# IDEA-Research/MP-Former

Hardware: AMD Instinct MI355X
Metric: training images/sec COCO-instance R50 1024x1024 (higher is better)
Workload: dtype bf16 (backbone, decoder) + f32 (pixel decoder, losses), as the reference's AMP; 1 GPU; COCO-instance R50, 100 queries, 80 classes, 1024x1024: full train step = R50 backbone + MSDeformAttn pixel decoder (6 layers) + MP masked decoder (9 layers, NUM_DN 1) + Hungarian matching + 60 losses + backward + grad all-reduce + clip + AdamW; head_only_workload=False, global_batch=2, per_gpu_batch=2, parallelism=dp1, msda_offsets=init, full=False, autograd_threads=backward on the launch thread, miopen_find_db=shipped

## Files before the change

include/mpformer_hip.h:

```cpp
#ifndef MPFORMER_HIP_H
#define MPFORMER_HIP_H

#include <stddef.h>
#include <stdint.h>

#ifdef __cplusplus
extern "C" {
#endif

enum { MPF_F32 = 0, MPF_F64 = 1, MPF_BF16 = 2, MPF_U8 = 3, MPF_BITS = 4  };

enum {
    MPF_OK = 0,
    MPF_E_DTYPE = -1,
    MPF_E_SHAPE = -2,
    MPF_E_NULL = -3,
    MPF_E_TOO_LARGE = -4
};

int mpf_abi_version(void);
const char* mpf_last_error(void);

int mpf_msda_forward(const void* value, const int64_t* spatial_shapes,
                     const int64_t* level_start_index, const void* sampling_loc,
                     const void* attn_weight, void* output,
                     int batch, int spatial_size, int num_heads, int channels,
                     int num_levels, int num_query, int num_point,
                     int dtype, void* stream);

int mpf_msda_forward_hs(const void* value, const int64_t* spatial_shapes,
                        const int64_t* level_start_index, const int64_t* host_spatial_shapes,
                        const void* sampling_loc, const void* attn_weight, void* output,
                        int batch, int spatial_size, int num_heads, int channels,
                        int num_levels, int num_query, int num_point,
                        int dtype, void* stream);

int mpf_msda_backward(const void* value, const int64_t* spatial_shapes,
                      const int64_t* level_start_index, const void* sampling_loc,
                      const void* attn_weight, const void* grad_output,
                      void* grad_value, void* grad_sampling_loc, void* grad_attn_weight,
                      int batch, int spatial_size, int num_heads, int channels,
                      int num_levels, int num_query, int num_point,
                      int dtype, void* stream);

size_t mpf_msda_dev_workspace_bytes(int batch, int spatial_size, int num_heads, int num_levels, int num_query, int num_point,
                                    int backward);
int mpf_msda_forward_dev(const void* value, const int64_t* spatial_shapes, const int64_t* level_start_index, const void* sampling_loc,
                         const void* attn_weight, void* output, int batch, int spatial_size, int num_heads, int channels,
                         int num_levels, int num_query, int num_point, int dtype, void* workspace, size_t workspace_bytes,
                         void* stream);
int mpf_msda_backward_dev(const void* value, const int64_t* spatial_shapes, const int64_t* level_start_index, const void* sampling_loc,
                          const void* attn_weight, const void* grad_output, void* grad_value, void* grad_sampling_loc,
                          void* grad_attn_weight, int batch, int spatial_size, int num_heads, int channels, int num_levels,
                          int num_query, int num_point, int dtype, void* workspace, size_t workspace_bytes, void* stream);
int mpf_msda_dev_geometry(const void* workspace, int* out, int n);

size_t mpf_msda_backward_workspace_bytes(int batch, int num_heads, int num_levels, int num_query,
                                         int num_point, const int64_t* host_spatial_shapes);
int mpf_msda_backward_ws(const void* value, const int64_t* host_spatial_shapes,
                         const void* sampling_loc, const void* attn_weight, const void* grad_output,
                         void* grad_value, void* grad_sampling_loc, void* grad_attn_weight,
                         int batch, int spatial_size, int num_heads, int channels,
                         int num_levels, int num_query, int num_point, int dtype,
                         void* workspace, size_t workspace_bytes, void* stream);

int mpf_set_option(const char* key, int value);
const char* mpf_last_kernel(void);
int mpf_msda_stats(unsigned long long* out, int n, int reset);

int mpf_point_sample(const void* src, int src_dtype, int h, int w, const int64_t* rows,
                     const float* coords, const int32_t* coord_rows, float* out, int n, int P, void* stream);

int mpf_mask_loss_forward(const void* pred, int pred_dtype, int h, int w, const int64_t* pred_rows,
                          const void* gt, int gt_dtype, int H, int W, const int32_t* gt_rows,
                          const float* coords, float* partial, int n, int P, int chunks, void* stream);

int mpf_pack_mask_bits(const uint8_t* masks, void* bits, int64_t n_pixels, void* stream);

int mpf_mask_loss_backward(const void* pred, int pred_dtype, int h, int w, const int64_t* pred_rows,
                           const uint8_t* gt, int H, int W, const int32_t* gt_rows,
                           const float* coords, const float* grad_sums, float* grad_pred,
                           const int64_t* grad_offs, int n, int P, void* stream);

int mpf_select_uncertain(const float* vals, const float* coords_in, float* coords_out,
                         int n, int M, int k, int P_out, void* stream);

int mpf_sample_select_uncertain(const void* pred, int pred_dtype, int h, int w, const int64_t* pred_offs,
                                const float* coords_in, float* coords_out, int n, int M, int k, int P_out,
                                void* stream);

int mpf_match_cost(const void* pred, int pred_dtype, int h, int w, const int64_t* pred_offs,
                   const float* coords, const int32_t* coord_rows, const float* tsamp,
                   const int32_t* t_first, const int32_t* t_count, float* cost,
                   int n_rows, int Tmax, int P, float w_mask, float w_dice, int rows_per_group, void* stream);

int mpf_attn_mask(const void* masks, int dtype, int64_t stride_n, int64_t stride_q, int h, int w,
                  const uint8_t* mp_rows, int pad, uint8_t* out, int N, int Q, int hl, int wl, void* stream);

size_t mpf_attn_workspace_bytes(int Lq, int Lk, int N, int H);
int mpf_attn_forward(const void* q, const void* k, const void* vt, const uint8_t* mask, int mask_per_image,
                     void* out, float* lse, int Lq, int Lk, int N, int H, int head_dim, float scale,
                     void* workspace, size_t workspace_bytes, void* stream);

int mpf_attn_backward(const void* q, const void* k, const void* v, const void* kT, const void* qT,
                      const void* dout, const void* doutT, const uint8_t* mask, int mask_per_image,
                      const float* lse, const float* delta, void* dq, void* dk, void* dv,
                      int Lq, int LqP, int Lk, int N, int H, int head_dim, float scale,
                      void* workspace, size_t workspace_bytes, void* stream);

int mpf_attn_transpose2(const void* a, const void* b, void* aT, void* bT, int L, int LP, int N, int E, void* stream);
int mpf_attn_transpose2_strided(const void* a, const void* b, int64_t in_row_stride, int64_t in_img_stride, void* aT, void* bT, int L,
                                int LP, int N, int E, void* stream);
int mpf_attn_forward_kv(const void* q, const void* k, int64_t k_row_stride, int64_t k_img_stride, const void* vt, const uint8_t* mask,
                        int mask_per_image, void* out, float* lse, int Lq, int Lk, int N, int H, int head_dim, float scale,
                        void* workspace, size_t workspace_bytes, void* stream);
int mpf_attn_backward_kv(const void* q, const void* k, const void* v, int64_t kv_row_stride, int64_t kv_img_stride, const void* kT,
                         const void* qT, const void* dout, const void* doutT, const uint8_t* mask, int mask_per_image,
                         const float* lse, const float* delta, void* dq, void* dk, void* dv, int64_t dkv_row_stride,
                         int64_t dkv_img_stride, int Lq, int LqP, int Lk, int N, int H, int head_dim, float scale, void* workspace,
                         size_t workspace_bytes, void* stream);
size_t mpf_attn_bwd_aux_bytes(int Lq, int Lk, int N, int H, int mask_images);
int mpf_attn_bwd_prep_aux(const void* q, const void* dout, const void* out, const float* lse, const uint8_t* mask, int mask_per_image,
                          int Lk, void* qT, void* doT, float* delta, void* aux, size_t aux_bytes, int Lq, int LqP, int N, int H,
                          void* stream);
int mpf_attn_backward_kv_aux(const void* q, const void* k, const void* v, int64_t kv_row_stride, int64_t kv_img_stride, const void* kT,
                             const void* qT, const void* dout, const void* doutT, const uint8_t* mask, int mask_per_image,
                             const float* lse, const float* delta, void* dq, void* dk, void* dv, int64_t dkv_row_stride,
                             int64_t dkv_img_stride, int Lq, int LqP, int Lk, int N, int H, int head_dim, float scale, void* workspace,
                             size_t workspace_bytes, const void* aux, void* stream);
int mpf_attn_delta(const void* dout, const void* out, float* delta, int Lq, int N, int H, void* stream);
int mpf_attn_bwd_prep(const void* q, const void* dout, const void* out, void* qT, void* doT, float* delta, int Lq, int LqP, int N,
                      int H, void* stream);

int mpf_msda_forward_raw(const void* value, const int64_t* spatial_shapes, const int64_t* level_start_index,
                         const void* raw, const void* ref_points, void* loc_out, void* attn_out, void* output,
                         int batch, int spatial_size, int num_heads, int channels, int num_levels, int num_query,
                         int num_point, int dtype, void* stream);
int mpf_msda_forward_raw_hs(const void* value, const int64_t* spatial_shapes, const int64_t* level_start_index,
                            const int64_t* host_spatial_shapes,
                            const void* raw, const void* ref_points, void* loc_out, void* attn_out, void* output,
                            int batch, int spatial_size, int num_heads, int channels, int num_levels, int num_query,
                            int num_point, int dtype, void* stream);
int mpf_msda_backward_ws_raw(const void* value, const int64_t* host_spatial_shapes,
                             const void* sampling_loc, const void* attn_weight, const void* grad_output,
                             void* grad_value, void* grad_raw,
                             int batch, int spatial_size, int num_heads, int channels,
                             int num_levels, int num_query, int num_point, int dtype,
                             void* workspace, size_t workspace_bytes, void* stream);
int mpf_msda_backward_ws_raw_o(const void* value, const int64_t* host_spatial_shapes,
// ... 122 lines not shown
size_t mpf_next_attn_mask_scratch_bytes(int N, int Q);
int mpf_next_attn_mask(const MpfNextMask* m, void* stream);
int mpf_decoder_layer_backward(const MpfDecoderLayer* layer, const MpfDecoderLayerGrad* grad, void* stream);

typedef struct MpfScaleCastItem {
    const void* src;
    void* dst;
    const float* scale;
    int64_t numel, inner, first_block;
} MpfScaleCastItem;

int mpf_grouped_scale_cast(const MpfScaleCastItem* items_device, int n_items, int64_t total_blocks, int src_dtype, int dst_dtype,
                           void* stream);

#define MPF_AMAX_SLOT_FLOATS 512
int mpf_res_ln256_forward_b(const float* x, const void* t, int t_dtype, const float* gamma, const float* beta, float* s_out, float* y32,
                            void* y16, float* mean, float* rstd, int rows, float eps, const float* padd, int padd_rows, float* y_plus,
                            float* y_bound, const float* padd_amax, float* yplus_bound, void* stream);
int mpf_res_ln256_backward_ws_amax(const float* s, const float* mean, const float* rstd, const float* gamma, const float* gy32,
                                   const void* gy16, const float* gy_plus, float* ds32, void* ds16, float* dgamma, float* dbeta, int rows,
                                   void* workspace, size_t workspace_bytes, float* ds_amax, void* stream);
typedef struct MpfAmaxItem {
    const float* src;
    float* out;
    int64_t numel, first_block;
} MpfAmaxItem;
typedef struct MpfSplitItemH2 {
    const float* src;
    void* dst;
    const float* amax;
    int64_t rows, cols, transpose, dst_ld, plane_stride, first_block;
} MpfSplitItemH2;
int mpf_amax_f32(const float* x, int64_t n, float* amax, void* stream);
int mpf_amax_f32_grouped(const MpfAmaxItem* items_device, int n_items, int64_t total_blocks, void* stream);
int mpf_h2_range_stats(const float* a, int rows, int cols, int64_t lda, const float* amax_slot, int log2_below,
                       unsigned long long* counters_device, void* stream);
int mpf_gemm3_split_grouped_h2(const MpfSplitItemH2* items_device, int n_items, int64_t total_blocks, void* stream);
typedef struct MpfNtItemH2 {
    const float* a;
    int64_t lda;
    const float* a_amax;
    const float* b;
    int64_t ldb;
    const float* b_amax;
    float* c_part;
    float* csum_a;
    int64_t Mdim, Ndim;
} MpfNtItemH2;
int mpf_gemm3_nt_h2(const float* a, int64_t lda, const float* a_amax, const float* b, int64_t ldb, const float* b_amax,
                    float* c_part, float* csum_a, float* csum_b, int R, int Mdim, int Ndim, int rows_per_split,
                    int transpose_out, void* stream);
int mpf_gemm3_nt_grouped_h2(const MpfNtItemH2* items, int n_items, int R, int rows_per_split, int64_t split_stride, void* stream);
int mpf_gemm3_conv3x3_h2(const float* x, const float* x_amax, const void* w_planes_h2, const float* w_amax, const float* bias,
                         float* y, float* out_amax, int n_img, int H, int W, int Cin, int Cout, int transposed, void* stream);
int mpf_gemm3_conv3x3_wgrad_h2(const float* dy, const float* dy_amax, const float* x, const float* x_amax, float* c_part,
                               float* csum_dy, int n_img, int H, int W, int Cin, int Cout, int rows_per_split, void* stream);
int mpf_gemm3_tn_h2(const float* a, int64_t lda, const float* a_amax, const void* b_planes_h2, const float* b_amax,
                    const float* bias, const float* c_in, int64_t ldcin, const float* c_in2, int64_t ldcin2,
                    const float* gate, int64_t ldgate, float* c, int64_t ldc, float* out_amax, int M, int N, int K,
                    int relu, void* stream);
int mpf_gemm3_tn_h2_bits(const float* a, int64_t lda, const float* a_amax, const void* b_planes_h2, const float* b_amax,
                         const float* bias, const float* c_in, int64_t ldcin, const float* c_in2, int64_t ldcin2,
                         const unsigned char* gate_bits, int64_t ldgbits, float* c, int64_t ldc, float* out_amax,
                         unsigned char* gate_bits_out, int64_t ldgbits_out, int M, int N, int K, int relu, void* stream);

typedef struct MpfNtItem {
    const float* a;
    int64_t lda;
    const float* b;
    int64_t ldb;
    float* c_part;
    float* csum_a;
    int64_t Mdim, Ndim;
} MpfNtItem;
int mpf_gemm3_nt_grouped(const MpfNtItem* items, int n_items, int R, int rows_per_split, int64_t split_stride, void* stream);

int mpf_gemm3_conv3x3(const float* x, const void* w_planes, const float* bias, float* y, int n_img, int H, int W, int Cin,
                      int Cout, int transposed, void* stream);
int mpf_gemm3_conv3x3_wgrad(const float* dy, const float* x, float* c_part, float* csum_dy, int n_img, int H, int W, int Cin, int Cout,
                            int rows_per_split, void* stream);

int mpf_gemm3_tn_ex(const void* a, int a_dtype, int64_t lda, const void* b_planes, const float* bias, const float* c_in, int64_t ldcin,
                    void* c, int c_dtype, int64_t ldc, int M, int N, int K, int relu, void* stream);
int mpf_gemm3_nt_ex(const void* a, int a_dtype, int64_t lda, const void* b, int b_dtype, int64_t ldb, float* c_part, float* csum_a,
                    int R, int Mdim, int Ndim, int rows_per_split, void* stream);

typedef struct MpfSplitItem {
    const float* src;
    void* dst;
    int64_t rows, cols, transpose, dst_ld, plane_stride, first_block;
} MpfSplitItem;

int mpf_gemm3_split_grouped(const MpfSplitItem* items_device, int n_items, int64_t total_blocks, void* stream);

typedef struct MpfOptItem {
    float* param;
    const float* grad;
    float* exp_avg;
    float* exp_avg_sq;
    int64_t numel, first_block;
    float lr, weight_decay, bc1, bc2_sqrt;
} MpfOptItem;

int mpf_clip_adamw_step(const MpfOptItem* items_device, int n_items, int64_t total_blocks, float max_norm, double beta1,
                        double beta2, double eps, float* partial, float* norm_clip, void* stream);

int mpf_transpose_f32(const float* in, int64_t in_batch_stride, float* out, int64_t out_batch_stride, int B, int R, int C,
                      void* stream);

int mpf_gemm3_nt_reduce(const float* c_part, int64_t c_numel, const float* s_part, int64_t s_numel, int nsplit,
                        float* c_out, float* s_out, void* stream);
int mpf_gemm3_nt_reduce_levels(const float* c_part, int64_t c_numel, const float* s_part, int64_t s_numel, int nsplit,
                               const int64_t* level_of_split, int n_levels, float* c_out, float* lvl_out, float* s_out, void* stream);

int mpf_tall_gemm_bf16(const void* a, int64_t lda, const void* b, int64_t ldb, const void* bias, void* c, int64_t ldc, int M, int N,
                       int K, void* stream);
size_t mpf_gemm_nt_bf16_workspace_bytes(int R, int Mdim, int Ndim, int rows_per_split);
int mpf_gemm_nt_bf16(const void* a, int64_t lda, const void* b, int64_t ldb, void* c_out, void* csum_out, int R, int Mdim,
                     int Ndim, int rows_per_split, void* workspace, size_t workspace_bytes, void* stream);

int mpf_small_gemm_bf16_blocked(const void* a, int64_t a_rs, int64_t a_ks, int a_blk, int64_t a_bs, const void* gate, const void* b,
                                int64_t b_rs, int64_t b_ks, const void* bias, const void* c_in, int64_t ldcin, void* c, int64_t ldc,
                                int c_blk, int64_t c_bs, void* rowsum_a, int I, int J, int Kc, int relu, void* stream);

int mpf_class_loss_forward(const void* logits, int dtype, int64_t sl, int64_t sn, int64_t sq, const int64_t* target,
                           int target_per_output, const float* weight, int L, int N, int Q, int C, float* lse, float* ce,
                           float* wsum, void* stream);
int mpf_class_loss_backward(const void* logits, int dtype, int64_t sl, int64_t sn, int64_t sq, const int64_t* target,
                            int target_per_output, const float* weight, int L, int N, int Q, int C, const float* lse,
                            const float* wsum, const float* grad_ce, void* dlogits, void* stream);
int mpf_mask_loss_finalize(const float* sums, const int64_t* runs, const float* norm, int n, int G, int points, float* out,
                           void* stream);
int mpf_mask_loss_finalize_backward(const float* sums, const int64_t* runs, const float* norm, int n, int G, int points,
                                    const float* grad_out, float* dsums, void* stream);

typedef struct {
    const void* a;
    const void* gate;
    const void* b;
    void* c;
    void* rowsum_a;
    int64_t a_rs, a_ks, a_bs, b_rs, b_ks, ldc;
    int a_blk, I, J, Kc;
} MpfSmallGemmItem;
int mpf_small_gemm_bf16_group(const MpfSmallGemmItem* items, int n_items, void* stream);
typedef struct MpfTransposeItem {
    const void* src;
    const void* gate;
    void* dst;
    int64_t ld;
    int R, C;
} MpfTransposeItem;
int mpf_transpose_group_bf16(const MpfTransposeItem* items, int n_items, int Rp, void* stream);

int mpf_bias_act(const void* x, const float* bias, const void* res, void* y, int64_t numel, int C, int dtype,
                 int relu, void* stream);
int mpf_relu_bwd_add(const void* ga, const void* gb, const void* y, void* out, int64_t numel, int dtype, void* stream);
int mpf_maxpool3x3s2_forward(const void* x, void* y, void* code, int N, int H, int W, int C, void* stream);
int mpf_maxpool3x3s2_backward(const void* gy, const void* code, void* gx, int N, int H, int W, int C, void* stream);

int mpf_upload_small(const void* host_src, void* device_dst, int64_t nbytes, void* stream);

int mpf_res_ln256_forward(const float* x, const void* t, int t_dtype, const float* gamma, const float* beta,
                          float* s_out, float* y32, void* y16, float* mean, float* rstd, int rows, float eps,
                          const float* padd, int padd_rows, float* y_plus, void* stream);
int mpf_res_ln256_backward(const float* s, const float* mean, const float* rstd, const float* gamma, const float* gy32,
                           const void* gy16, const float* gy_plus, float* ds32, void* ds16, float* dgamma, float* dbeta,
                           int rows, void* stream);
int mpf_res_ln256_backward_partial(const float* s, const float* mean, const float* rstd, const float* gamma, const float* gy32,
                                   const void* gy16, const float* gy_plus, float* ds32, void* ds16, int rows, void* partials,
                                   size_t partials_bytes, void* stream);
int mpf_res_ln256_backward_partial_amax(const float* s, const float* mean, const float* rstd, const float* gamma, const float* gy32,
                                        const void* gy16, const float* gy_plus, float* ds32, void* ds16, int rows, void* partials,
                                        size_t partials_bytes, float* ds_amax, void* stream);
int mpf_ln_partial_reduce(const void* partials, size_t stride_bytes, int rows, int n_ln, float* out, void* stream);
size_t mpf_res_ln256_backward_det_workspace_bytes(int rows);
int mpf_res_ln256_backward_det(const float* s, const float* mean, const float* rstd, const float* gamma, const float* gy32,
                               const void* gy16, const float* gy_plus, float* ds32, void* ds16, float* dgamma_dbeta, int rows,
                               void* workspace, size_t workspace_bytes, void* stream);
size_t mpf_res_ln256_backward_workspace_bytes(int rows);
int mpf_res_ln256_backward_ws(const float* s, const float* mean, const float* rstd, const float* gamma, const float* gy32,
                              const void* gy16, const float* gy_plus, float* ds32, void* ds16, float* dgamma, float* dbeta, int rows,
                              void* workspace, size_t workspace_bytes, void* stream);

int mpf_mask_loss_backward_dense(const void* pred, int pred_dtype, int h, int w, const int64_t* pred_rows,
                                 const void* gt, int gt_dtype, int H, int W, const int32_t* gt_rows, const float* coords,
                                 const float* grad_sums, void* grad, int grad_dtype, const int64_t* grad_offs,
                                 int n, int P, void* stream);

size_t mpf_group_stats_workspace_bytes(int rows, int64_t row_len);
int mpf_group_stats(const float* x, int rows, int64_t row_len, float eps, float* mean, float* rstd,
                    void* workspace, size_t workspace_bytes, void* stream);

int mpf_gn_cl_supported(int HW, int C, int G);
size_t mpf_gn_cl_workspace_bytes(int N, int HW, int C, int G);
int mpf_gn_cl_forward(const float* x, int64_t x_bs, const float* gamma, const float* beta, int N, int HW, int C, int G,
                      float eps, int relu, const float* top, int64_t top_bs, int W, float* y, int64_t y_bs, float* mean,
                      float* rstd, void* workspace, size_t workspace_bytes, void* stream);
int mpf_gn_cl_backward(const float* gy, int64_t gy_bs, const float* x, int64_t x_bs, const float* gamma, const float* beta,
                       const float* mean, const float* rstd, int N, int HW, int C, int G, int relu, float* dx,
                       int64_t dx_bs, float* dgamma, float* dbeta, void* workspace, size_t workspace_bytes, void* stream);
int mpf_upsample2x_cl_backward(const float* gy, int64_t gy_bs, int N, int Ht, int Wt, int C, float* dtop, int64_t dtop_bs,
                               void* stream);

size_t mpf_match_cost_fused_workspace_bytes(int G, int Q, int Tmax, int P, int tsamp_rows);
int mpf_match_cost_fused(const void* embed, const int64_t* embed_first, int64_t embed_row_stride, const void* features,
                         int64_t feat_img_stride, const int32_t* group_image, int h, int w, int channels, const float* coords,
                         const float* tsamp, int tsamp_rows, const int32_t* t_first, const int32_t* t_count, float* cost, int G,
                         int Q, int Tmax, int P, float w_mask, float w_dice, void* workspace, size_t workspace_bytes, void* stream);
int mpf_pair_planes_forward(const void* embed, const int64_t* row_off, const int32_t* pair_of_slot, const int32_t* slot_first,
                            const int32_t* slot_count, const void* features, int64_t feat_img_stride, void* out, int N, int HW,
                            int channels, void* stream);
size_t mpf_pair_planes_backward_workspace_bytes(int N, int HW, int total_slots, int max_count);
int mpf_pair_planes_backward(const void* grad_planes, const void* embed, const int64_t* row_off, const int32_t* pair_of_slot,
                             const int32_t* slot_first, const int32_t* slot_count, const void* features, int64_t feat_img_stride,
                             void* d_features, int64_t dfeat_img_stride, void* d_embed, int d_embed_dtype, int N, int HW, int channels,
                             int total_slots, int max_count, void* workspace, size_t workspace_bytes, void* stream);

int mpf_profile_enable(int on);
int mpf_profile_get(const char* name_substr, int* count, double* total_ms, double* total_bytes);
int mpf_profile_get_flops(const char* name_substr, double* total_flops);

enum {
    MPF_ENC_PV, MPF_ENC_PV_AM, MPF_ENC_PO, MPF_ENC_PO_AM, MPF_ENC_P1, MPF_ENC_P1_AM, MPF_ENC_P2, MPF_ENC_P2_AM, MPF_ENC_P288, MPF_ENC_P288_AM,
    MPF_ENC_BV, MPF_ENC_BO, MPF_ENC_BB1, MPF_ENC_BB2, MPF_ENC_B288, MPF_ENC_G1, MPF_ENC_B1, MPF_ENC_G2, MPF_ENC_B2,
    MPF_ENC_VALUE, MPF_ENC_RAW, MPF_ENC_LOC, MPF_ENC_ATTN, MPF_ENC_AO, MPF_ENC_S1, MPF_ENC_MEAN1, MPF_ENC_RSTD1, MPF_ENC_X1, MPF_ENC_H,
    MPF_ENC_HBITS, MPF_ENC_S2, MPF_ENC_MEAN2, MPF_ENC_RSTD2, MPF_ENC_X2, MPF_ENC_QN,
    MPF_ENC_AO_AM, MPF_ENC_X1_AM, MPF_ENC_H_AM, MPF_ENC_XN_AM, MPF_ENC_QN_AM,
    MPF_ENC_FIELDS
};
typedef struct MpfEncoderCall {
    int32_t N, S, M, L, P, nl, F, reserved;
    float eps, pad_;
    const int64_t* host_shapes;
    const void* shapes_dev;
    const void* lsi_dev;
    const float* ref;
    const float* pos_full;
    const float* pos_am;
    const float* x0;
    const float* x0_am;
    const float* q0;
    const float* q0_am;
    const uint64_t* layers;
} MpfEncoderCall;
int mpf_encoder_fields(void);
int mpf_encoder_forward(const MpfEncoderCall* call, void* stream);

enum {
    MPF_ENCB_X, MPF_ENCB_Q, MPF_ENCB_VALUE, MPF_ENCB_LOC, MPF_ENCB_ATTN, MPF_ENCB_AO, MPF_ENCB_S1, MPF_ENCB_MEAN1, MPF_ENCB_RSTD1, MPF_ENCB_X1,
    MPF_ENCB_H, MPF_ENCB_HBITS, MPF_ENCB_S2, MPF_ENCB_MEAN2, MPF_ENCB_RSTD2,
    MPF_ENCB_X_AM, MPF_ENCB_Q_AM, MPF_ENCB_AO_AM, MPF_ENCB_X1_AM, MPF_ENCB_H_AM,
    MPF_ENCB_G1, MPF_ENCB_G2,
    MPF_ENCB_TV, MPF_ENCB_TV_AM, MPF_ENCB_TO, MPF_ENCB_TO_AM, MPF_ENCB_T1, MPF_ENCB_T1_AM, MPF_ENCB_T2, MPF_ENCB_T2_AM, MPF_ENCB_T288, MPF_ENCB_T288_AM,
    MPF_ENCB_DS2_AM, MPF_ENCB_DH_AM, MPF_ENCB_DS1_AM, MPF_ENCB_DRAW_AM, MPF_ENCB_GV_AM,
    MPF_ENCB_WGRAD, MPF_ENCB_DW288, MPF_ENCB_LVL, MPF_ENCB_DB288,
    MPF_ENCB_FIELDS
};
typedef struct MpfEncoderBwdCall {
    int32_t N, S, M, L, P, nl, F, rps288, rps_group, reserved;
    int64_t group_stride;
    const int64_t* host_shapes;
    const float* gout;
    const int64_t* split_level;
    float *ds2, *dh, *dx1, *ds1, *dao, *gv, *draw;
    float* dq[2];
    float* g[2];
    float *cpart288, *cs288, *part_group;
    void* ln_parts;
    uint64_t ln_stride;
    void* msda_ws;
    uint64_t msda_ws_bytes;
    float* dgb_out;
    const uint64_t* layers;
} MpfEncoderBwdCall;
int mpf_encoder_bwd_fields(void);
int mpf_encoder_backward(const MpfEncoderBwdCall* call, void* stream);

int mpf_seg_softmax(const float* cls, int Q, int K1, float object_mask_threshold, float* probs, float* max_score, int* max_label,
                    int* kept, float* kept_score, void* stream);
int mpf_seg_semantic(const void* masks, int64_t stride_q, int dtype, int Q, int h, int w, int Hp, int Wp, int hi, int wi, int H, int W,
                     const float* probs, int K, float* out, void* stream);
size_t mpf_seg_instance_workspace_bytes(int T, int H, int W);
int mpf_seg_instance_scores(const void* masks, int64_t stride_q, int dtype, int Q, int h, int w, int Hp, int Wp, int hi, int wi, int H,
                            int W, const int64_t* sel_q, const float* cls_score, int T, float* scores, void* workspace,
                            size_t workspace_bytes, void* stream);
// ... 32 lines not shown
```

mp_former_amd/_lib.py:

```python
import ctypes

import torch
import os

_HERE = os.path.dirname(os.path.abspath(__file__))
LIB_PATH = os.path.join(_HERE, "libmpformer_hip.so")
LIB_PATH = os.environ.get("MPF_LIB_PATH", LIB_PATH)
ABI_VERSION = 1

MPF_F32, MPF_F64, MPF_BF16, MPF_U8, MPF_BITS = 0, 1, 2, 3, 4
DTYPE = {torch.float32: MPF_F32, torch.float64: MPF_F64, torch.bfloat16: MPF_BF16, torch.uint8: MPF_U8, torch.bool: MPF_U8}

_lib = None
_status_fns = {}

_c_int = ctypes.c_int
_c_vp = ctypes.c_void_p

SIGNATURES = {
    "mpf_abi_version": (_c_int, []),
    "mpf_last_error": (ctypes.c_char_p, []),
    "mpf_last_kernel": (ctypes.c_char_p, []),
    "mpf_set_option": (_c_int, [ctypes.c_char_p, _c_int]),
    "mpf_match_cost_fused_workspace_bytes": (ctypes.c_size_t, [_c_int] * 5),
    "mpf_match_cost_fused": (_c_int, [_c_vp, _c_vp, ctypes.c_int64, _c_vp, ctypes.c_int64, _c_vp, _c_int, _c_int, _c_int, _c_vp, _c_vp, _c_int,
                                      _c_vp, _c_vp, _c_vp, _c_int, _c_int, _c_int, _c_int, ctypes.c_float, ctypes.c_float, _c_vp,
                                      ctypes.c_size_t, _c_vp]),
    "mpf_pair_planes_forward": (_c_int, [_c_vp] * 6 + [ctypes.c_int64, _c_vp, _c_int, _c_int, _c_int, _c_vp]),
    "mpf_pair_planes_backward_workspace_bytes": (ctypes.c_size_t, [_c_int] * 4),
    "mpf_pair_planes_backward": (_c_int, [_c_vp] * 7 + [ctypes.c_int64, _c_vp, ctypes.c_int64, _c_vp, _c_int, _c_int, _c_int, _c_int, _c_int,
                                          _c_int, _c_vp, ctypes.c_size_t, _c_vp]),
    "mpf_msda_dev_workspace_bytes": (ctypes.c_size_t, [_c_int] * 7),
    "mpf_msda_forward_dev": (_c_int, [_c_vp] * 6 + [_c_int] * 8 + [_c_vp, ctypes.c_size_t, _c_vp]),
    "mpf_msda_backward_dev": (_c_int, [_c_vp] * 9 + [_c_int] * 8 + [_c_vp, ctypes.c_size_t, _c_vp]),
    "mpf_msda_dev_geometry": (_c_int, [_c_vp, ctypes.POINTER(_c_int), _c_int]),
    "mpf_msda_stats": (_c_int, [ctypes.POINTER(ctypes.c_ulonglong), _c_int, _c_int]),
    "mpf_profile_enable": (_c_int, [_c_int]),
    "mpf_profile_get_flops": (_c_int, [ctypes.c_char_p, ctypes.POINTER(ctypes.c_double)]),
    "mpf_profile_get": (_c_int, [ctypes.c_char_p, ctypes.POINTER(_c_int), ctypes.POINTER(ctypes.c_double),
                                 ctypes.POINTER(ctypes.c_double)]),
    "mpf_point_sample": (_c_int, [_c_vp, _c_int, _c_int, _c_int, _c_vp, _c_vp, _c_vp, _c_vp, _c_int, _c_int, _c_vp]),
    "mpf_mask_loss_forward": (_c_int, [_c_vp, _c_int, _c_int, _c_int, _c_vp, _c_vp, _c_int, _c_int, _c_int, _c_vp, _c_vp,
                                       _c_vp, _c_int, _c_int, _c_int, _c_vp]),
    "mpf_pack_mask_bits": (_c_int, [_c_vp, _c_vp, ctypes.c_int64, _c_vp]),
    "mpf_mask_loss_backward": (_c_int, [_c_vp, _c_int, _c_int, _c_int, _c_vp, _c_vp, _c_int, _c_int, _c_vp, _c_vp,
                                        _c_vp, _c_vp, _c_vp, _c_int, _c_int, _c_vp]),
    "mpf_select_uncertain": (_c_int, [_c_vp, _c_vp, _c_vp, _c_int, _c_int, _c_int, _c_int, _c_vp]),
    "mpf_sample_select_uncertain": (_c_int, [_c_vp, _c_int, _c_int, _c_int, _c_vp, _c_vp, _c_vp, _c_int, _c_int, _c_int, _c_int, _c_vp]),
    "mpf_match_cost": (_c_int, [_c_vp, _c_int, _c_int, _c_int, _c_vp, _c_vp, _c_vp, _c_vp, _c_vp, _c_vp, _c_vp,
                                _c_int, _c_int, _c_int, ctypes.c_float, ctypes.c_float, _c_int, _c_vp]),
    "mpf_attn_mask": (_c_int, [_c_vp, _c_int, ctypes.c_int64, ctypes.c_int64, _c_int, _c_int, _c_vp, _c_int, _c_vp,
                               _c_int, _c_int, _c_int, _c_int, _c_vp]),
    "mpf_attn_workspace_bytes": (ctypes.c_size_t, [_c_int] * 4),
    "mpf_attn_forward": (_c_int, [_c_vp, _c_vp, _c_vp, _c_vp, _c_int, _c_vp, _c_vp, _c_int, _c_int, _c_int, _c_int, _c_int,
                                  ctypes.c_float, _c_vp, ctypes.c_size_t, _c_vp]),
    "mpf_attn_backward": (_c_int, [_c_vp] * 8 + [_c_int] + [_c_vp] * 5 + [_c_int] * 6 + [ctypes.c_float, _c_vp, ctypes.c_size_t, _c_vp]),
    "mpf_attn_transpose2": (_c_int, [_c_vp] * 4 + [_c_int] * 4 + [_c_vp]),
    "mpf_attn_transpose2_strided": (_c_int, [_c_vp] * 2 + [ctypes.c_int64] * 2 + [_c_vp] * 2 + [_c_int] * 4 + [_c_vp]),
    "mpf_attn_forward_kv": (_c_int, [_c_vp, _c_vp, ctypes.c_int64, ctypes.c_int64, _c_vp, _c_vp, _c_int, _c_vp, _c_vp, _c_int, _c_int,
                                     _c_int, _c_int, _c_int, ctypes.c_float, _c_vp, ctypes.c_size_t, _c_vp]),
    "mpf_attn_backward_kv": (_c_int, [_c_vp] * 3 + [ctypes.c_int64] * 2 + [_c_vp] * 5 + [_c_int] + [_c_vp] * 5 + [ctypes.c_int64] * 2
                             + [_c_int] * 6 + [ctypes.c_float, _c_vp, ctypes.c_size_t, _c_vp]),
    "mpf_attn_backward_kv_aux": (_c_int, [_c_vp] * 3 + [ctypes.c_int64] * 2 + [_c_vp] * 5 + [_c_int] + [_c_vp] * 5 + [ctypes.c_int64] * 2
                                 + [_c_int] * 6 + [ctypes.c_float, _c_vp, ctypes.c_size_t, _c_vp, _c_vp]),
    "mpf_attn_bwd_aux_bytes": (ctypes.c_size_t, [_c_int] * 5),
    "mpf_attn_bwd_prep_aux": (_c_int, [_c_vp] * 5 + [_c_int] * 2 + [_c_vp] * 4 + [ctypes.c_size_t] + [_c_int] * 4 + [_c_vp]),
    "mpf_attn_delta": (_c_int, [_c_vp] * 3 + [_c_int] * 3 + [_c_vp]),
    "mpf_attn_bwd_prep": (_c_int, [_c_vp] * 6 + [_c_int] * 4 + [_c_vp]),
    "mpf_gemm3_split": (_c_int, [_c_vp, _c_int, _c_int, _c_int, _c_vp, _c_vp]),
    "mpf_gemm3_tn": (_c_int, [_c_vp, ctypes.c_int64, _c_vp, _c_int, _c_vp, _c_vp, _c_vp, ctypes.c_int64, _c_vp, ctypes.c_int64,
                           _c_vp, ctypes.c_int64, _c_vp, ctypes.c_int64, _c_int, _c_int, _c_int, _c_int, _c_vp]),
    "mpf_gemm3_nt": (_c_int, [_c_vp, ctypes.c_int64, _c_vp, ctypes.c_int64, _c_vp, ctypes.c_int64, _c_int, _c_vp, _c_vp, _c_vp,
                           _c_int, _c_int, _c_int, _c_int, _c_int, _c_vp]),
    "mpf_amax_f32": (_c_int, [_c_vp, ctypes.c_int64, _c_vp, _c_vp]),
    "mpf_amax_f32_grouped": (_c_int, [_c_vp, _c_int, ctypes.c_int64, _c_vp]),
    "mpf_h2_range_stats": (_c_int, [_c_vp, _c_int, _c_int, ctypes.c_int64, _c_vp, _c_int, _c_vp, _c_vp]),
    "mpf_gemm3_split_grouped_h2": (_c_int, [_c_vp, _c_int, ctypes.c_int64, _c_vp]),
    "mpf_gemm3_tn_h2": (_c_int, [_c_vp, ctypes.c_int64, _c_vp, _c_vp, _c_vp, _c_vp, _c_vp, ctypes.c_int64, _c_vp, ctypes.c_int64,
                              _c_vp, ctypes.c_int64, _c_vp, ctypes.c_int64, _c_vp, _c_int, _c_int, _c_int, _c_int, _c_vp]),
    "mpf_gemm3_tn_h2_bits": (_c_int, [_c_vp, ctypes.c_int64, _c_vp, _c_vp, _c_vp, _c_vp, _c_vp, ctypes.c_int64, _c_vp, ctypes.c_int64,
                                   _c_vp, ctypes.c_int64, _c_vp, ctypes.c_int64, _c_vp, _c_vp, ctypes.c_int64,
                                   _c_int, _c_int, _c_int, _c_int, _c_vp]),
    "mpf_gemm3_nt_h2": (_c_int, [_c_vp, ctypes.c_int64, _c_vp, _c_vp, ctypes.c_int64, _c_vp, _c_vp, _c_vp, _c_vp,
                              _c_int, _c_int, _c_int, _c_int, _c_int, _c_vp]),
    "mpf_gemm3_nt_grouped_h2": (_c_int, [_c_vp, _c_int, _c_int, _c_int, ctypes.c_int64, _c_vp]),
    "mpf_gemm3_conv3x3_h2": (_c_int, [_c_vp] * 7 + [_c_int] * 6 + [_c_vp]),
    "mpf_gemm3_conv3x3_wgrad_h2": (_c_int, [_c_vp, _c_vp, _c_vp, _c_vp, _c_vp, _c_vp, _c_int, _c_int, _c_int, _c_int, _c_int, _c_int, _c_vp]),
    "mpf_gemm3_nt_grouped": (_c_int, [_c_vp, _c_int, _c_int, _c_int, ctypes.c_int64, _c_vp]),
    "mpf_small_gemm_bf16": (_c_int, [_c_vp, ctypes.c_int64, ctypes.c_int64, _c_vp, _c_vp, ctypes.c_int64, ctypes.c_int64, _c_vp, _c_vp,
                                     ctypes.c_int64, _c_vp, ctypes.c_int64, _c_vp, _c_int, _c_int, _c_int, _c_int, _c_vp]),
    "mpf_encoder_fields": (_c_int, []),
    "mpf_encoder_forward": (_c_int, [_c_vp, _c_vp]),
    "mpf_encoder_bwd_fields": (_c_int, []),
    "mpf_encoder_backward": (_c_int, [_c_vp, _c_vp]),
    "mpf_decoder_layer_struct_bytes": (ctypes.c_uint64, [_c_int]),
    "mpf_decoder_layer_scratch_bytes": (ctypes.c_uint64, [_c_int] * 6),
    "mpf_decoder_layer_forward": (_c_int, [_c_vp, _c_vp]),
    "mpf_next_attn_mask_scratch_bytes": (ctypes.c_size_t, [_c_int, _c_int]),
    "mpf_next_attn_mask": (_c_int, [_c_vp, _c_vp]),
    "mpf_lin256_res_ln_forward": (_c_int, [_c_vp] * 11 + [_c_int, ctypes.c_float, _c_vp]),
    "mpf_ln256_mlp3_forward": (_c_int, [_c_vp] * 10 + [_c_int, ctypes.c_float, _c_vp]),
    "mpf_decoder_layer_backward": (_c_int, [_c_vp, _c_vp, _c_vp]),
    "mpf_pool_features": (_c_int, [_c_vp, _c_int, _c_vp] + [_c_int] * 6 + [_c_vp]),
    "mpf_pool_features_cl": (_c_int, [_c_vp, ctypes.c_int64, _c_int, _c_vp, _c_int, _c_int, _c_int, _c_int, _c_int, _c_int, _c_vp]),
    "mpf_mask_head_bits": (_c_int, [_c_vp, ctypes.c_int64, ctypes.c_int64, _c_vp, _c_vp, _c_int, _c_vp, _c_vp] + [_c_int] * 3 + [_c_vp]),
    "mpf_lsa_assign": (_c_int, [_c_vp, _c_vp, _c_int, _c_int, ctypes.c_int64] + [_c_vp] * 7),
    "mpf_lsa_assign_status": (_c_int, [_c_vp, _c_vp, _c_int, _c_int, ctypes.c_int64] + [_c_vp] * 8),
    "mpf_mask_block_empty": (_c_int, [_c_vp, _c_vp] + [_c_int] * 5 + [_c_vp]),
    "mpf_mp_open_counts": (_c_int, [_c_vp, _c_int, _c_int, _c_vp, _c_vp]),
    "mpf_mp_noise_rows": (_c_int, [_c_vp] * 3 + [_c_int] * 4 + [ctypes.c_double, ctypes.c_uint64, ctypes.c_uint64, _c_vp, _c_vp]),
    "mpf_gemm_nt_bf16_workspace_bytes": (ctypes.c_size_t, [_c_int] * 4),
    "mpf_gemm_nt_bf16": (_c_int, [_c_vp, ctypes.c_int64, _c_vp, ctypes.c_int64, _c_vp, _c_vp, _c_int, _c_int, _c_int, _c_int, _c_vp,
                                  ctypes.c_size_t, _c_vp]),
    "mpf_gemm3_nt_reduce": (_c_int, [_c_vp, ctypes.c_int64, _c_vp, ctypes.c_int64, _c_int, _c_vp, _c_vp, _c_vp]),
    "mpf_grouped_scale_cast": (_c_int, [_c_vp, _c_int, ctypes.c_int64, _c_int, _c_int, _c_vp]),
    "mpf_gemm3_split_grouped": (_c_int, [_c_vp, _c_int, ctypes.c_int64, _c_vp]),
    "mpf_decoder_inputs_forward": (_c_int, [_c_vp, ctypes.c_int64, ctypes.c_int64, _c_vp, _c_vp, _c_vp, _c_vp, _c_int, _c_int, _c_int, _c_int,
                                            _c_vp]),
    "mpf_decoder_inputs_backward": (_c_int, [_c_vp, _c_vp, _c_int, _c_vp, ctypes.c_int64, ctypes.c_int64, _c_int, _c_int, _c_int, _c_vp]),
    "mpf_clip_adamw_step": (_c_int, [_c_vp, _c_int, ctypes.c_int64, ctypes.c_float, ctypes.c_double, ctypes.c_double, ctypes.c_double,
                                     _c_vp, _c_vp, _c_vp]),
    "mpf_transpose_f32": (_c_int, [_c_vp, ctypes.c_int64, _c_vp, ctypes.c_int64, _c_int, _c_int, _c_int, _c_vp]),
    "mpf_small_gemm_bf16_blocked": (_c_int, [_c_vp, ctypes.c_int64, ctypes.c_int64, _c_int, ctypes.c_int64, _c_vp, _c_vp, ctypes.c_int64,
                                             ctypes.c_int64, _c_vp, _c_vp, ctypes.c_int64, _c_vp, ctypes.c_int64, _c_int, ctypes.c_int64,
                                             _c_vp, _c_int, _c_int, _c_int, _c_int, _c_vp]),
    "mpf_small_gemm_bf16_group": (_c_int, [_c_vp, _c_int, _c_vp]),
    "mpf_transpose_group_bf16": (_c_int, [_c_vp, _c_int, _c_int, _c_vp]),
    "mpf_class_loss_forward": (_c_int, [_c_vp, _c_int, ctypes.c_int64, ctypes.c_int64, ctypes.c_int64, _c_vp, _c_int, _c_vp, _c_int, _c_int,
                                        _c_int, _c_int, _c_vp, _c_vp, _c_vp, _c_vp]),
    "mpf_class_loss_backward": (_c_int, [_c_vp, _c_int, ctypes.c_int64, ctypes.c_int64, ctypes.c_int64, _c_vp, _c_int, _c_vp, _c_int, _c_int,
                                         _c_int, _c_int, _c_vp, _c_vp, _c_vp, _c_vp, _c_vp]),
    "mpf_mask_loss_finalize": (_c_int, [_c_vp, _c_vp, _c_vp, _c_int, _c_int, _c_int, _c_vp, _c_vp]),
    "mpf_mask_loss_finalize_backward": (_c_int, [_c_vp, _c_vp, _c_vp, _c_int, _c_int, _c_int, _c_vp, _c_vp, _c_vp]),
    "mpf_bias_act": (_c_int, [_c_vp, _c_vp, _c_vp, _c_vp, ctypes.c_int64, _c_int, _c_int, _c_int, _c_vp]),
    "mpf_relu_bwd_add": (_c_int, [_c_vp, _c_vp, _c_vp, _c_vp, ctypes.c_int64, _c_int, _c_vp]),
    "mpf_maxpool3x3s2_forward": (_c_int, [_c_vp] * 3 + [_c_int] * 4 + [_c_vp]),
    "mpf_maxpool3x3s2_backward": (_c_int, [_c_vp] * 3 + [_c_int] * 4 + [_c_vp]),
    "mpf_upload_small": (_c_int, [_c_vp, _c_vp, ctypes.c_int64, _c_vp]),
    "mpf_tall_gemm_bf16": (_c_int, [_c_vp, ctypes.c_int64, _c_vp, ctypes.c_int64, _c_vp, _c_vp, ctypes.c_int64, _c_int, _c_int, _c_int, _c_vp]),
    "mpf_res_ln256_forward": (_c_int, [_c_vp, _c_vp, _c_int, _c_vp, _c_vp, _c_vp, _c_vp, _c_vp, _c_vp, _c_vp, _c_int, ctypes.c_float,
                                       _c_vp, _c_int, _c_vp, _c_vp]),
    "mpf_res_ln256_forward_b": (_c_int, [_c_vp, _c_vp, _c_int, _c_vp, _c_vp, _c_vp, _c_vp, _c_vp, _c_vp, _c_vp, _c_int, ctypes.c_float,
                                         _c_vp, _c_int, _c_vp, _c_vp, _c_vp, _c_vp, _c_vp]),
    "mpf_res_ln256_backward_ws_amax": (_c_int, [_c_vp] * 11 + [_c_int, _c_vp, ctypes.c_size_t, _c_vp, _c_vp]),
    "mpf_res_ln256_backward": (_c_int, [_c_vp] * 11 + [_c_int, _c_vp]),
    "mpf_mask_loss_backward_dense": (_c_int, [_c_vp, _c_int, _c_int, _c_int, _c_vp, _c_vp, _c_int, _c_int, _c_int, _c_vp, _c_vp, _c_vp,
                                              _c_vp, _c_int, _c_vp, _c_int, _c_int, _c_vp]),
    "mpf_gn_cl_supported": (_c_int, [_c_int, _c_int, _c_int]),
    "mpf_gn_cl_workspace_bytes": (ctypes.c_size_t, [_c_int, _c_int, _c_int, _c_int]),
    "mpf_gn_cl_forward": (_c_int, [_c_vp, ctypes.c_int64, _c_vp, _c_vp, _c_int, _c_int, _c_int, _c_int, ctypes.c_float, _c_int,
                                   _c_vp, ctypes.c_int64, _c_int, _c_vp, ctypes.c_int64, _c_vp, _c_vp, _c_vp, ctypes.c_size_t, _c_vp]),
    "mpf_gn_cl_backward": (_c_int, [_c_vp, ctypes.c_int64, _c_vp, ctypes.c_int64, _c_vp, _c_vp, _c_vp, _c_vp, _c_int, _c_int, _c_int,
                                    _c_int, _c_int, _c_vp, ctypes.c_int64, _c_vp, _c_vp, _c_vp, ctypes.c_size_t, _c_vp]),
    "mpf_upsample2x_cl_backward": (_c_int, [_c_vp, ctypes.c_int64, _c_int, _c_int, _c_int, _c_int, _c_vp, ctypes.c_int64, _c_vp]),
    "mpf_gemm3_conv3x3": (_c_int, [_c_vp, _c_vp, _c_vp, _c_vp, _c_int, _c_int, _c_int, _c_int, _c_int, _c_int, _c_vp]),
    "mpf_gemm3_conv3x3_wgrad": (_c_int, [_c_vp, _c_vp, _c_vp, _c_vp, _c_int, _c_int, _c_int, _c_int, _c_int, _c_int, _c_vp]),
    "mpf_gemm3_nt_reduce_levels": (_c_int, [_c_vp, ctypes.c_int64, _c_vp, ctypes.c_int64, _c_int, _c_vp, _c_int, _c_vp, _c_vp, _c_vp, _c_vp]),
    "mpf_gemm3_tn_ex": (_c_int, [_c_vp, _c_int, ctypes.c_int64, _c_vp, _c_vp, _c_vp, ctypes.c_int64, _c_vp, _c_int, ctypes.c_int64,
                                 _c_int, _c_int, _c_int, _c_int, _c_vp]),
    "mpf_gemm3_nt_ex": (_c_int, [_c_vp, _c_int, ctypes.c_int64, _c_vp, _c_int, ctypes.c_int64, _c_vp, _c_vp, _c_int, _c_int, _c_int, _c_int, _c_vp]),
    "mpf_res_ln256_backward_workspace_bytes": (ctypes.c_size_t, [_c_int]),
    "mpf_res_ln256_backward_partial": (_c_int, [_c_vp] * 9 + [_c_int, _c_vp, ctypes.c_size_t, _c_vp]),
    "mpf_res_ln256_backward_partial_amax": (_c_int, [_c_vp] * 9 + [_c_int, _c_vp, ctypes.c_size_t, _c_vp, _c_vp]),
    "mpf_ln_partial_reduce": (_c_int, [_c_vp, ctypes.c_size_t, _c_int, _c_int, _c_vp, _c_vp]),
    "mpf_res_ln256_backward_det_workspace_bytes": (ctypes.c_size_t, [_c_int]),
    "mpf_res_ln256_backward_det": (_c_int, [_c_vp] * 10 + [_c_int, _c_vp, ctypes.c_size_t, _c_vp]),
    "mpf_res_ln256_backward_ws": (_c_int, [_c_vp] * 11 + [_c_int, _c_vp, ctypes.c_size_t, _c_vp]),
    "mpf_group_stats_workspace_bytes": (ctypes.c_size_t, [_c_int, ctypes.c_int64]),
    "mpf_group_stats": (_c_int, [_c_vp, _c_int, ctypes.c_int64, ctypes.c_float, _c_vp, _c_vp, _c_vp, ctypes.c_size_t, _c_vp]),
    "mpf_msda_forward": (_c_int, [_c_vp] * 6 + [_c_int] * 8 + [_c_vp]),
    "mpf_msda_backward": (_c_int, [_c_vp] * 9 + [_c_int] * 8 + [_c_vp]),
    "mpf_msda_forward_hs": (_c_int, [_c_vp] * 7 + [_c_int] * 8 + [_c_vp]),
    "mpf_msda_forward_raw_hs": (_c_int, [_c_vp] * 9 + [_c_int] * 8 + [_c_vp]),
    "mpf_msda_forward_raw": (_c_int, [_c_vp] * 8 + [_c_int] * 8 + [_c_vp]),
    "mpf_msda_backward_ws_raw": (_c_int, [_c_vp] * 7 + [_c_int] * 8 + [_c_vp, ctypes.c_size_t, _c_vp]),
    "mpf_msda_backward_ws_raw_o": (_c_int, [_c_vp] * 8 + [_c_int] * 8 + [_c_vp, ctypes.c_size_t, _c_vp, _c_vp, _c_vp]),
    "mpf_msda_backward_workspace_bytes": (ctypes.c_size_t, [_c_int] * 5 + [_c_vp]),
    "mpf_msda_backward_ws": (_c_int, [_c_vp] * 8 + [_c_int] * 8 + [_c_vp, ctypes.c_size_t, _c_vp]),
    "mpf_seg_softmax": (_c_int, [_c_vp, _c_int, _c_int, ctypes.c_float] + [_c_vp] * 6),
    "mpf_seg_semantic": (_c_int, [_c_vp, ctypes.c_int64] + [_c_int] * 10 + [_c_vp, _c_int, _c_vp, _c_vp]),
    "mpf_seg_instance_workspace_bytes": (ctypes.c_size_t, [_c_int] * 3),
    "mpf_seg_instance_scores": (_c_int, [_c_vp, ctypes.c_int64] + [_c_int] * 10 + [_c_vp, _c_vp, _c_int, _c_vp, _c_vp, ctypes.c_size_t,
                                                                                   _c_vp]),
    "mpf_seg_instance_masks": (_c_int, [_c_vp, ctypes.c_int64] + [_c_int] * 10 + [_c_vp, _c_int, _c_vp, _c_vp]),
    "mpf_seg_panoptic_areas": (_c_int, [_c_vp, ctypes.c_int64] + [_c_int] * 10 + [_c_vp] * 5),
    "mpf_seg_panoptic_paint": (_c_int, [_c_vp, _c_int, _c_int, _c_vp, _c_vp, _c_vp]),
    "mpf_seg_semantic_labels": (_c_int, [_c_vp, ctypes.c_int64] + [_c_int] * 10 + [_c_vp, _c_int, _c_vp, _c_vp]),
    "mpf_seg_labels_resize": (_c_int, [_c_vp] + [_c_int] * 5 + [_c_vp, _c_vp]),
    "mpf_seg_confusion_add": (_c_int, [_c_vp, _c_vp, ctypes.c_int64, _c_int, _c_int, _c_vp, _c_vp]),
    "mpf_seg_instance_rle_workspace_bytes": (ctypes.c_size_t, [_c_int] * 3),
    "mpf_seg_instance_rle_count": (_c_int, [_c_vp, ctypes.c_int64] + [_c_int] * 10 + [_c_vp, _c_int, _c_vp, _c_vp, ctypes.c_size_t, _c_vp]),
    "mpf_seg_instance_rle_write": (_c_int, [_c_vp, ctypes.c_size_t, _c_int, _c_int, _c_int, _c_vp, ctypes.c_int64, _c_vp, _c_vp, _c_vp]),
    "mpf_seg_tta_accumulate": (_c_int, [_c_vp, ctypes.c_int64] + [_c_int] * 10 + [_c_vp, _c_int, _c_int, _c_vp, _c_vp]),
    "mpf_seg_tta_resize_add": (_c_int, [_c_vp] + [_c_int] * 6 + [_c_vp, _c_vp]),
    "mpf_seg_tta_finish": (_c_int, [_c_vp] + [_c_int] * 4 + [_c_vp, _c_vp]),
    "mpf_seg_pq_workspace_bytes": (ctypes.c_size_t, [_c_int] * 2),
    "mpf_seg_pq_pairs": (_c_int, [_c_vp, _c_vp, _c_int, ctypes.c_int64, _c_vp, _c_int, _c_int, _c_vp, _c_int, _c_int, _c_int, _c_vp,
                                  ctypes.c_size_t, _c_vp]),
    "mpf_seg_pq_match": (_c_int, [_c_vp, ctypes.c_size_t, _c_int, _c_int, _c_int, _c_vp, _c_vp, _c_vp, _c_int] + [_c_vp] * 6),
}


class NativeLibraryError(RuntimeError):
    pass


def lib():
    global _lib
    if _lib is None:
        if not os.path.exists(LIB_PATH):
            raise NativeLibraryError(
                f"{LIB_PATH} not found: build it with `python -c 'import __graft_entry__ as g; g.build()'` "
                "or `make -C mp_former_amd/csrc`.  mp_former_amd has no CPU / eager fallback.")
        l = ctypes.CDLL(LIB_PATH)
        for name, (res, args) in SIGNATURES.items():
            try:
                fn = getattr(l, name)
            except AttributeError as e:
                raise NativeLibraryError(f"{LIB_PATH} does not export {name}") from e
            fn.restype = res
            fn.argtypes = args
            if res is _c_int:
                _status_fns[name] = fn
        v = l.mpf_abi_version()
        if v != ABI_VERSION:
            raise NativeLibraryError(f"ABI mismatch: library {v}, binding {ABI_VERSION}")
        _lib = l
        for kv in filter(None, os.environ.get("MPF_OPTIONS", "").split(",")):
            k, _, v = kv.partition("=")
            set_option(k.strip(), int(v))
    return _lib


def check(code, what):
    if code != 0:
        msg = lib().mpf_last_error().decode()
        raise RuntimeError(f"{what} failed with code {code}: {msg}")


def _status_fn(name):
    lib()
    fn = _status_fns.get(name)
    if fn is None:
        raise TypeError(f"{name} does not return a status: call() is for the int-returning entry points, sizes go through lib()")
    return fn


def call(name, device, *args):
    fn = _status_fns.get(name) or _status_fn(name)
    idx = device.index
    if idx is None or idx == torch.cuda.current_device():
        code = fn(*args)
    else:
        with torch.cuda.device(device):
            code = fn(*args)
    if code != 0:
        check(code, name)


def ptr(t):
    return None if t is None else t.data_ptr()


_option_gen = 0


def option_generation():
    return _option_gen


def set_option(key, value):
    global _option_gen
    check(lib().mpf_set_option(key.encode(), int(value)), f"mpf_set_option({key})")
    _option_gen += 1


def msda_stats(reset=True):
    out = (ctypes.c_ulonglong * 9)()
    check(lib().mpf_msda_stats(out, 9, 1 if reset else 0), "mpf_msda_stats")
    keys = ("fwd_lds", "fwd_gather", "push_lds", "push_gather", "push_direct", "push_hash", "spill_entries", "pull_split", "pull_single")
    return dict(zip(keys, (int(v) for v in out)))


def last_kernel():
    return lib().mpf_last_kernel().decode()


def profile_enable(on=True):
    check(lib().mpf_profile_enable(1 if on else 0), "mpf_profile_enable")


def profile_get_flops(name_substr):
    fl = ctypes.c_double(0)
    check(lib().mpf_profile_get_flops(name_substr.encode(), ctypes.byref(fl)), "mpf_profile_get_flops")
    return fl.value


def profile_get(name_substr):
    n, ms, by = _c_int(0), ctypes.c_double(0), ctypes.c_double(0)
    check(lib().mpf_profile_get(name_substr.encode(), ctypes.byref(n), ctypes.byref(ms), ctypes.byref(by)),
          "mpf_profile_get")
    return n.value, ms.value, by.value


_scratch = {}


def scratch(owner, device, stream, nbytes, zeroed=False):
    key = (owner, device, stream)
    w = _scratch.get(key)
    if w is None or w.numel() < nbytes:
        n = int(nbytes * 1.25) + 1024
        w = _scratch[key] = (torch.zeros if zeroed else torch.empty)(n, dtype=torch.uint8, device=device)
    return w


def stream_ptr(device):
    idx = device.index
    return torch._C._cuda_getCurrentRawStream(torch.cuda.current_device() if idx is None else idx)


class _NullGuard:
    def __enter__(self):
        return None

    def __exit__(self, *exc):
        return False


_NULL_GUARD = _NullGuard()


def device_guard(device):
    idx = device.index
    if idx is None or idx == torch.cuda.current_device():
        return _NULL_GUARD
    return torch.cuda.device(device)
```

mp_former_amd/conv3x3.py:

```python

import torch
from torch.autograd import Function

from . import _lib
from .gemm3 import amax, split_weights_grouped, split_weights_grouped_h2
from .groupnorm import is_cl_plane


def enabled():
    return True


def supported(x, weight):
    if not (enabled() and is_cl_plane(x) and weight.dtype == torch.float32 and weight.dim() == 4):
        return False
    N, C, H, W = x.shape
    Cout, Cin, kh, kw = weight.shape
    return (kh == 3 and kw == 3 and Cin == C and C % 32 == 0 and Cout % 32 == 0 and x.stride(0) == H * W * C
            and N * H * W * max(C, Cout) < 2 ** 31 and H >= 2 and W >= 2)


def _planes(N, C, H, W, device):
    return torch.empty((N, H, W, C), dtype=torch.float32, device=device).permute(0, 3, 1, 2)


class _Conv3x3Fn(Function):
    @staticmethod
    def forward(ctx, x, weight, bias):
        N, Cin, H, W = x.shape
        Cout = weight.shape[0]
        w2 = weight.permute(0, 2, 3, 1).reshape(Cout, 9 * Cin)
        w2t = weight.permute(1, 2, 3, 0).reshape(Cin, 9 * Cout)
        y = _planes(N, Cout, H, W, x.device)
        st = _lib.stream_ptr(x.device)
        h2 = Cout % 256 == 0 and Cin % 256 == 0
        if h2:
            (pf, pf_am), (pb, pb_am) = split_weights_grouped_h2([([w2.contiguous()], False), ([w2t.contiguous()], False)])
            x_am = amax(x.permute(0, 2, 3, 1))
            _lib.call("mpf_gemm3_conv3x3_h2", x.device, x.data_ptr(), x_am.data_ptr(), pf.data_ptr(), pf_am.data_ptr(), _lib.ptr(bias),
                      y.data_ptr(), None, N, H, W, Cin, Cout, 0, st)
            ctx.save_for_backward(x, weight, pb, pb_am, x_am)
        else:
            pf, pb = split_weights_grouped([([w2.contiguous()], False), ([w2t.contiguous()], False)])
            _lib.call("mpf_gemm3_conv3x3", x.device, x.data_ptr(), pf.data_ptr(), _lib.ptr(bias), y.data_ptr(), N, H, W, Cin, Cout, 0, st)
            ctx.save_for_backward(x, weight, pb)
        ctx.has_bias, ctx.h2 = bias is not None, h2
        return y

    @staticmethod
    def backward(ctx, gy):
        if ctx.h2:
            x, weight, pb, pb_am, x_am = ctx.saved_tensors
        else:
            x, weight, pb = ctx.saved_tensors
        N, Cin, H, W = x.shape
        Cout = weight.shape[0]
        if not (is_cl_plane(gy) and gy.stride(0) == H * W * Cout):
            gy = gy.permute(0, 2, 3, 1).contiguous().permute(0, 3, 1, 2)
        dx = dw = db = None
        st = _lib.stream_ptr(x.device)
        gy_am = amax(gy.permute(0, 2, 3, 1)) if ctx.h2 else None
        if ctx.needs_input_grad[0]:
            dx = _planes(N, Cin, H, W, x.device)
            if ctx.h2:
                _lib.call("mpf_gemm3_conv3x3_h2", x.device, gy.data_ptr(), gy_am.data_ptr(), pb.data_ptr(), pb_am.data_ptr(), None,
                          dx.data_ptr(), None, N, H, W, Cout, Cin, 1, st)
            else:
                _lib.call("mpf_gemm3_conv3x3", x.device, gy.data_ptr(), pb.data_ptr(), None, dx.data_ptr(), N, H, W, Cout, Cin, 1, st)
        if ctx.needs_input_grad[1] or (ctx.has_bias and ctx.needs_input_grad[2]):
            if W % 8 == 0 and Cin % 128 == 0:
                dw, db = _wgrad_native(gy, x, N, H, W, Cin, Cout, ctx.has_bias, (gy_am, x_am) if ctx.h2 else None)
            else:
                _, dw, db = torch.ops.aten.convolution_backward(
                    gy, x, weight, [Cout] if ctx.has_bias else None, [1, 1], [1, 1], [1, 1], False, [0, 0], 1,
                    [False, bool(ctx.needs_input_grad[1]), bool(ctx.has_bias and ctx.needs_input_grad[2])])
        return dx, dw, db


def _wgrad_native(gy, x, N, H, W, Cin, Cout, has_bias, amax_ab=None):
    from .gemm3 import nt_reduce
    R = N * H * W
    tiles = ((Cout + 127) // 128) * (9 * Cin // 128)
    slots = 2 * torch.cuda.get_device_properties(x.device).multi_processor_count
    ns = max(1, (3 * slots) // tiles)
    if amax_ab is not None and Cout % 256 == 0 and Cin % 256 == 0:
        ns = max(1, (slots // 2) // ((Cout // 256) * (9 * Cin // 256)))
    rps = max(128, ((-(-R // ns)) + 31) // 32 * 32)
    ns = -(-R // rps)
    c = torch.empty((ns, Cout, 9 * Cin), dtype=torch.float32, device=x.device)
    ca = torch.empty((ns, Cout), dtype=torch.float32, device=x.device) if has_bias else None
    if amax_ab is not None:
        _lib.call("mpf_gemm3_conv3x3_wgrad_h2", x.device, gy.data_ptr(), amax_ab[0].data_ptr(), x.data_ptr(), amax_ab[1].data_ptr(),
                  c.data_ptr(), _lib.ptr(ca), N, H, W, Cin, Cout, rps, _lib.stream_ptr(x.device))
    else:
        _lib.call("mpf_gemm3_conv3x3_wgrad", x.device, gy.data_ptr(), x.data_ptr(), c.data_ptr(), _lib.ptr(ca), N, H, W, Cin, Cout, rps,
                  _lib.stream_ptr(x.device))
    dw2, db = nt_reduce(c, ca)
    return dw2.view(Cout, 3, 3, Cin).permute(0, 3, 1, 2), db


def conv3x3(x, weight, bias=None):
    return _Conv3x3Fn.apply(x, weight, bias)


def _planes_any(x):
    if not (x.dim() == 4 and x.is_cuda and x.dtype in (torch.float32, torch.bfloat16)):
        return False
    N, C, H, W = x.shape
    return (x.stride(1) == 1 and x.stride(3) == C and x.stride(2) == W * C and x.stride(0) == H * W * C
            and x.data_ptr() % 16 == 0 and (C * x.element_size()) % 16 == 0)


def supported_1x1(x, weight):
    if not (_planes_any(x) and weight.dtype == torch.float32 and weight.dim() == 4):
        return False
    N, C, H, W = x.shape
    Cout, Cin, kh, kw = weight.shape
    return kh == 1 and kw == 1 and Cin == C and C % 32 == 0 and Cout % 32 == 0


class _Conv1x1Fn(Function):

    @staticmethod
    def forward(ctx, x, weight, bias, out_dtype):
        from .gemm3 import gemm3, gemm3_ex
        N, Cin, H, W = x.shape
        Cout = weight.shape[0]
        w2 = weight.view(Cout, Cin)
        pf, pb = split_weights_grouped([([w2], False), ([w2], True)])
        x2 = x.permute(0, 2, 3, 1).reshape(N * H * W, Cin)
        if x.dtype == torch.float32 and out_dtype == torch.float32:
            y2 = gemm3(x2, pf, bias)
        else:
            y2 = gemm3_ex(x2, pf, bias, out_dtype=out_dtype)
        ctx.save_for_backward(x2, pb)
        ctx.dims, ctx.has_bias = (N, Cin, Cout, H, W), bias is not None
        return y2.view(N, H, W, Cout).permute(0, 3, 1, 2)

    @staticmethod
    def backward(ctx, gy):
        from .gemm3 import balanced_rps, gemm3, gemm3_ex, gemm3_nt, gemm3_nt_ex, nt_reduce
        x2, pb = ctx.saved_tensors
        N, Cin, Cout, H, W = ctx.dims
        g2 = gy.permute(0, 2, 3, 1).reshape(N * H * W, Cout)
        if g2.stride(1) != 1 or g2.stride(0) != Cout:
            g2 = g2.contiguous()
        if g2.dtype == torch.bfloat16 and x2.dtype == torch.bfloat16:
            g2 = g2.float()
        dx = dw = db = None
        if ctx.needs_input_grad[0]:
            if g2.dtype == torch.float32 and x2.dtype == torch.float32:
                dx2 = gemm3(g2, pb)
            else:
                dx2 = gemm3_ex(g2, pb, out_dtype=x2.dtype)
            dx = dx2.view(N, H, W, Cin).permute(0, 3, 1, 2)
        if ctx.needs_input_grad[1] or (ctx.has_bias and ctx.needs_input_grad[2]):
            rps = balanced_rps(g2.shape[0], Cout, Cin, g2.device)
            mixed = g2.dtype != x2.dtype
            if mixed and Cin % 128 == 0:
                c, ca = gemm3_nt_ex(g2, x2, rps, want_csum_a=True)
            else:
                c, ca, _ = gemm3_nt(g2.float() if mixed else g2, x2.float() if mixed else x2, rps, want_csum_a=True)
            dw, db = nt_reduce(c, ca)
            dw = dw.view(Cout, Cin, 1, 1)
            if not ctx.has_bias:
                db = None
        return dx, dw, db, None


def conv1x1(x, weight, bias=None, out_dtype=torch.float32):
    return _Conv1x1Fn.apply(x, weight, bias, out_dtype)
```

mp_former_amd/csrc/common.hip:

```cpp
#include "mpf_common.h"

#include <stdio.h>

#include <atomic>
#include <mutex>
#include <string>
#include <vector>

namespace {
thread_local char t_err[256] = "";
std::atomic<const char*> g_kernel{""};
}

namespace mpf {
int fail(int code, const char* msg)
{
    snprintf(t_err, sizeof(t_err), "%s", msg);
    return code;
}

int check(hipError_t err, const char* where)
{
    if (err == hipSuccess) return 0;
    snprintf(t_err, sizeof(t_err), "%s: %s (%d)", where, hipGetErrorString(err), (int)err);
// ... 37 lines not shown
{
    std::lock_guard<std::mutex> lk(mpf::g_prof_mu);
    for (auto& r : mpf::g_prof) { (void)hipEventDestroy(r.e0); (void)hipEventDestroy(r.e1); }
    mpf::g_prof.clear();
    mpf::g_prof_on.store(on ? 1 : 0);
    return 0;
}

extern "C" int mpf_profile_get(const char* name_substr, int* count, double* total_ms, double* total_bytes)
{
    if (!name_substr || !count || !total_ms || !total_bytes) return MPF_E_NULL;
    std::lock_guard<std::mutex> lk(mpf::g_prof_mu);
    int n = 0; double ms = 0, by = 0;
    for (auto& r : mpf::g_prof) {
        if (!strstr(r.name, name_substr)) continue;
        if (hipEventSynchronize(r.e1) != hipSuccess) continue;
        float t = 0.f;
        if (hipEventElapsedTime(&t, r.e0, r.e1) != hipSuccess) continue;
        ms += t; by += r.bytes; ++n;
    }
    *count = n; *total_ms = ms; *total_bytes = by;
    return 0;
}

extern "C" int mpf_profile_get_flops(const char* name_substr, double* total_flops)
{
    if (!name_substr || !total_flops) return MPF_E_NULL;
    std::lock_guard<std::mutex> lk(mpf::g_prof_mu);
    double fl = 0;
    for (auto& r : mpf::g_prof)
        if (strstr(r.name, name_substr)) fl += r.flops;
    *total_flops = fl;
    return 0;
}

namespace {
constexpr int kUpPayload = 3968;
struct UpPayload { uint32_t w[kUpPayload / 4]; };
__global__ __launch_bounds__(256) void upload_small_kernel(UpPayload p, uint32_t* __restrict__ dst, int nwords)
{
    for (int i = threadIdx.x; i < nwords; i += 256) dst[i] = p.w[i];
}
}

extern "C" int mpf_upload_small(const void* host_src, void* device_dst, int64_t nbytes, void* stream)
{
    if (nbytes == 0) return 0;
    if (!host_src || !device_dst) return mpf::fail(MPF_E_NULL, "upload_small: NULL buffer");
    if (nbytes < 0 || (nbytes & 3) || ((uintptr_t)device_dst & 3)) return mpf::fail(MPF_E_SHAPE, "upload_small: size / destination must be multiples of 4 bytes");
    const unsigned char* src = static_cast<const unsigned char*>(host_src);
    unsigned char* dst = static_cast<unsigned char*>(device_dst);
    for (int64_t off = 0; off < nbytes; off += kUpPayload) {
        const int n = (int)((nbytes - off) < kUpPayload ? (nbytes - off) : kUpPayload);
        UpPayload p;
        memcpy(p.w, src + off, (size_t)n);
        hipLaunchKernelGGL(upload_small_kernel, dim3(1), dim3(256), 0, (hipStream_t)stream, p, reinterpret_cast<uint32_t*>(dst + off), n / 4);
    }
    return mpf::check(hipGetLastError(), "mpf_upload_small");
}

extern "C" int mpf_abi_version(void) { return 1; }
extern "C" const char* mpf_last_error(void) { return t_err; }
extern "C" const char* mpf_last_kernel(void) { return g_kernel.load(std::memory_order_relaxed); }

extern "C" int mpf_set_option(const char* key, int value)
{
    if (!key) return MPF_E_NULL;
    int r = mpf::set_msda_option(key, value);
    if (r <= 0) return r;
    r = mpf::set_binned_option(key, value);
    if (r <= 0) return r;
    r = mpf::set_gemm3_option(key, value);
    if (r <= 0) return r;
    r = mpf::set_decoder_option(key, value);
    if (r <= 0) return r;
    r = mpf::set_block_option(key, value);
    if (r <= 0) return r;
    r = mpf::set_attn_option(key, value);
    if (r <= 0) return r;
    r = mpf::set_small_gemm_option(key, value);
    if (r <= 0) return r;
    return mpf::fail(MPF_E_SHAPE, "mpf_set_option: unknown key");
}
```

mp_former_amd/csrc/gemm3.hip:

```cpp
#include <hip/hip_runtime.h>

#include <algorithm>
#include <atomic>
#include <stdint.h>

#include "mpf_common.h"
#include "amax.h"
#ifndef G3_PRIO
#define G3_PRIO 1
#endif

namespace {

typedef __attribute__((ext_vector_type(8))) __bf16 bf16x8;
typedef __attribute__((ext_vector_type(4))) float f32x4;

constexpr int kBM = 128;
constexpr int kBK = 32;
constexpr int kThreads = 256;
constexpr int kAKc = kBM * 16;

struct G3 {
    const float* a;
    const float* a2;
    const unsigned short* bp;
    const float* bias;
    const float* cin;
    const float* cin2;
    const float* gate;
    float* c;
    int64_t lda, ldc, ldcin, ldcin2, ldgate, plane;
    int M, N, K, a2_rows, relu, tiles_n, ntiles;
    int bias_cm, cin_cm, cin2_cm, gate_cm;
    unsigned short* c16;
    int cv_H, cv_W, cv_cin, cv_sign;
    int tm0, ntiles2, tiles_n2;
    const float* a_amax;
    const float* b_amax;
    float* out_amax;
    const unsigned char* gbits;
    unsigned char* gbits_out;
    int64_t ldgbits, ldgbits_out;
    int gbits_cm;
    int t3_bm;
};

int g_ablate = 0;
int g_mixed = 1;
int g_two_pass = 256;
int g_two_pass_rows = 0;
int g_nt2 = 1;
int g_tn3 = 1;
int g_tn3_176 = 1;
int g_ws = 512;


__device__ __forceinline__ unsigned pack_hi16(unsigned a, unsigned b)
{
    return __builtin_amdgcn_perm(b, a, 0x07060302u);
}

__device__ __forceinline__ void split8(const float4 u, const float4 v, uint4* h, uint4* m, uint4* l)
{
    const float x[8] = {u.x, u.y, u.z, u.w, v.x, v.y, v.z, v.w};
    unsigned hb[8], mb[8], lb[8];
#pragma unroll
    for (int i = 0; i < 8; ++i) {
        const unsigned xb = __float_as_uint(x[i]);
        hb[i] = xb;
        const float r1 = x[i] - __uint_as_float(xb & 0xFFFF0000u);
        const unsigned rb = __float_as_uint(r1);
        mb[i] = rb;
        const float r2 = r1 - __uint_as_float(rb & 0xFFFF0000u);
        lb[i] = __float_as_uint(r2) + 0x8000u;
    }
    *h = make_uint4(pack_hi16(hb[0], hb[1]), pack_hi16(hb[2], hb[3]), pack_hi16(hb[4], hb[5]), pack_hi16(hb[6], hb[7]));
    *m = make_uint4(pack_hi16(mb[0], mb[1]), pack_hi16(mb[2], mb[3]), pack_hi16(mb[4], mb[5]), pack_hi16(mb[6], mb[7]));
    *l = make_uint4(pack_hi16(lb[0], lb[1]), pack_hi16(lb[2], lb[3]), pack_hi16(lb[4], lb[5]), pack_hi16(lb[6], lb[7]));
}

typedef __attribute__((ext_vector_type(8))) _Float16 f16x8;
typedef __attribute__((ext_vector_type(2))) _Float16 f16x2;
typedef __attribute__((ext_vector_type(2))) float f32x2;

__device__ __forceinline__ void split8h(const float4 u, const float4 v, const float scale, uint4* h, uint4* l)
{
    const float x[8] = {u.x, u.y, u.z, u.w, v.x, v.y, v.z, v.w};
    unsigned hb[4], lb[4];
#pragma unroll
    for (int i = 0; i < 4; ++i) {
        const f32x2 s = {x[2 * i] * scale, x[2 * i + 1] * scale};
        const f16x2 hh = __builtin_convertvector(s, f16x2);
        const f32x2 back = __builtin_convertvector(hh, f32x2);
        const f32x2 r = {s[0] - back[0], s[1] - back[1]};
        const f16x2 ll = __builtin_convertvector(r, f16x2);
        union { f16x2 f; unsigned u; } ch, cl;
        ch.f = hh; cl.f = ll;
        hb[i] = ch.u; lb[i] = cl.u;
    }
    *h = make_uint4(hb[0], hb[1], hb[2], hb[3]);
    *l = make_uint4(lb[0], lb[1], lb[2], lb[3]);
}

__device__ __forceinline__ void h2_scale(const unsigned amax_bits, float* scale, float* inv)
{
    int e = (int)((amax_bits >> 23) & 0xffu);
    e = max(e, 30);
    *scale = __uint_as_float((unsigned)(268 - e) << 23);
    *inv = __uint_as_float((unsigned)(e - 14) << 23);
}

__device__ __forceinline__ f16x8 as_fragh(const uint4 v)
{
    union { uint4 u; f16x8 f; } c;
    c.u = v;
    return c.f;
}

__device__ __forceinline__ float4 add4(float4 x, float4 y) { return make_float4(x.x + y.x, x.y + y.y, x.z + y.z, x.w + y.w); }

__device__ __forceinline__ bf16x8 as_frag(const uint4 v)
{
    union { uint4 u; bf16x8 f; } c;
    c.u = v;
    return c.f;
}

typedef __attribute__((ext_vector_type(16))) float f32x16;

template <int NJ, bool W32 = false>
struct Acc {
    f32x4 v[4][NJ];

    __device__ __forceinline__ void zero()
    {
#pragma unroll
// ... 1164 lines not shown
        out[o] = (unsigned short)(xb >> 16);
        out[it.plane_stride + o] = (unsigned short)(rb >> 16);
        out[2 * it.plane_stride + o] = (unsigned short)(lb >> 16);
    }
}

__global__ __launch_bounds__(256) void amax_grouped_kernel(const MpfAmaxItem* __restrict__ items, int n_items)
{
    int lo = 0, hi = n_items - 1;
    const int64_t blk = blockIdx.x;
    while (lo < hi) {
        const int mid = (lo + hi + 1) >> 1;
        if (items[mid].first_block <= blk) lo = mid; else hi = mid - 1;
    }
    const MpfAmaxItem it = items[lo];
    const int64_t base = (blk - it.first_block) * 4096;
    float m = 0.f;
    if (((uintptr_t)it.src & 15) == 0 && base + 4096 <= it.numel) {
        const float4* __restrict__ s4 = reinterpret_cast<const float4*>(it.src + base);
        float4 v[4];
#pragma unroll
        for (int k = 0; k < 4; ++k) v[k] = s4[k * 256 + threadIdx.x];
#pragma unroll
        for (int k = 0; k < 4; ++k) m = fmaxf(fmaxf(m, fmaxf(fabsf(v[k].x), fabsf(v[k].y))), fmaxf(fabsf(v[k].z), fabsf(v[k].w)));
    } else {
        for (int64_t i = base + threadIdx.x; i < min(base + 4096, it.numel); i += 256) m = fmaxf(m, fabsf(it.src[i]));
    }
    __shared__ float red[4];
    amax_commit(it.out, m, red);
}

__global__ __launch_bounds__(256) void amax_kernel(const float* __restrict__ x, int64_t n4, int64_t n, float* __restrict__ out)
{
    const float4* __restrict__ x4 = reinterpret_cast<const float4*>(x);
    float m = 0.f;
    const int64_t stride = (int64_t)gridDim.x * 256;
    int64_t i = (int64_t)blockIdx.x * 256 + threadIdx.x;
    for (; i + 3 * stride < n4; i += 4 * stride) {
        float4 v[4];
#pragma unroll
        for (int k = 0; k < 4; ++k) v[k] = x4[i + k * stride];
#pragma unroll
        for (int k = 0; k < 4; ++k) m = fmaxf(fmaxf(m, fmaxf(fabsf(v[k].x), fabsf(v[k].y))), fmaxf(fabsf(v[k].z), fabsf(v[k].w)));
    }
    for (; i < n4; i += stride) {
        const float4 v = x4[i];
        m = fmaxf(fmaxf(m, fmaxf(fabsf(v.x), fabsf(v.y))), fmaxf(fabsf(v.z), fabsf(v.w)));
    }
    for (int64_t j = 4 * n4 + (int64_t)blockIdx.x * 256 + threadIdx.x; j < n; j += stride) m = fmaxf(m, fabsf(x[j]));
    __shared__ float red[4];
    amax_commit(out, m, red);
}

__global__ __launch_bounds__(256) void gemm3_split_grouped_h2_kernel(const MpfSplitItemH2* __restrict__ items, int n_items)
{
    int lo = 0, hi = n_items - 1;
    const int64_t blk = blockIdx.x;
    while (lo < hi) {
        const int mid = (lo + hi + 1) >> 1;
        if (items[mid].first_block <= blk) lo = mid; else hi = mid - 1;
    }
    const MpfSplitItemH2 it = items[lo];
    const float* __restrict__ w = it.src;
    _Float16* __restrict__ out = static_cast<_Float16*>(it.dst);
    float scale, inv;
    h2_scale(amax_read(it.amax), &scale, &inv);
    const int R = (int)it.rows, C = (int)it.cols;
    const int64_t total = (int64_t)R * C, base = (blk - it.first_block) * 1024;
#pragma unroll
    for (int k = 0; k < 4; ++k) {
        const int64_t i = base + k * 256 + threadIdx.x;
        if (i >= total) continue;
        int r, c;
        int64_t o;
        if (it.transpose) { c = (int)(i / R); r = (int)(i - (int64_t)c * R); o = (int64_t)c * it.dst_ld + r; }
        else { r = (int)(i / C); c = (int)(i - (int64_t)r * C); o = (int64_t)r * it.dst_ld + c; }
        const float x = w[(int64_t)r * C + c] * scale;
        const _Float16 h = (_Float16)x;
        out[o] = h;
        out[it.plane_stride + o] = (_Float16)(x - (float)h);
    }
}

}

extern "C" int mpf_amax_f32(const float* x, int64_t n, float* amax, void* stream)
{
    if (!x || !amax) return mpf::fail(MPF_E_NULL, "amax_f32: NULL buffer");
    if (n <= 0) return 0;
    if ((uintptr_t)x & 15) return mpf::fail(MPF_E_SHAPE, "amax_f32: x must be 16-byte aligned");
    const int64_t n4 = n / 4;
    const int blocks = (int)std::min<int64_t>(1024, std::max<int64_t>(1, (n4 + 1023) / 1024));
    mpf::prof_begin((hipStream_t)stream);
    mpf::set_kernel("amax_kernel");
    hipLaunchKernelGGL(amax_kernel, dim3(blocks), dim3(256), 0, (hipStream_t)stream, x, n4, n, amax);
    mpf::prof_end("amax_kernel", (hipStream_t)stream, 4.0 * (double)n);
    return mpf::check(hipGetLastError(), "mpf_amax_f32");
}

__global__ __launch_bounds__(256) void h2_range_stats_kernel(const float* __restrict__ a, int rows, int cols, int64_t lda,
                                                             const float* __restrict__ amax_slot, int log2_below,
                                                             unsigned long long* __restrict__ counters)
{
    const int lane = threadIdx.x & 63, wave = threadIdx.x >> 6;
    const float ref = __uint_as_float(amax_read(amax_slot));
    const float thr = ldexpf(ref, -log2_below);
    unsigned nz = 0, below = 0;
    for (int r = blockIdx.x * 4 + wave; r < rows; r += gridDim.x * 4) {
        const float4* __restrict__ row = reinterpret_cast<const float4*>(a + (int64_t)r * lda);
        float m = 0.f;
        for (int c = lane; c < cols / 4; c += 64) {
            const float4 v = row[c];
            m = fmaxf(fmaxf(m, fmaxf(fabsf(v.x), fabsf(v.y))), fmaxf(fabsf(v.z), fabsf(v.w)));
        }
#pragma unroll
        for (int o = 32; o >= 1; o >>= 1) m = fmaxf(m, __shfl_xor(m, o));
        nz += m > 0.f;
        below += (m > 0.f && m < thr);
    }
    __shared__ unsigned red[8];
    if (lane == 0) { red[wave * 2] = nz; red[wave * 2 + 1] = below; }
    __syncthreads();
    if (threadIdx.x < 2) {
        const unsigned v = red[threadIdx.x] + red[2 + threadIdx.x] + red[4 + threadIdx.x] + red[6 + threadIdx.x];
        if (v) atomicAdd(counters + threadIdx.x, (unsigned long long)v);
    }
}

extern "C" int mpf_h2_range_stats(const float* a, int rows, int cols, int64_t lda, const float* amax_slot, int log2_below,
                                  unsigned long long* counters_device, void* stream)
{
    if (!a || !amax_slot || !counters_device) return mpf::fail(MPF_E_NULL, "h2_range_stats: NULL buffer");
    if (rows <= 0 || cols <= 0 || cols % 4 || lda < cols || lda % 4 || ((uintptr_t)a & 15) || log2_below < 0 || log2_below > 120)
        return mpf::fail(MPF_E_SHAPE, "h2_range_stats: cols and lda must be multiples of 4, a 16-byte aligned, 0 <= log2_below <= 120");
    const int blocks = std::min(2048, (rows + 3) / 4);
    mpf::set_kernel("h2_range_stats_kernel");
    hipLaunchKernelGGL(h2_range_stats_kernel, dim3(blocks), dim3(256), 0, (hipStream_t)stream, a, rows, cols, lda, amax_slot, log2_below,
                       counters_device);
    return mpf::check(hipGetLastError(), "mpf_h2_range_stats");
}

extern "C" int mpf_amax_f32_grouped(const MpfAmaxItem* items_device, int n_items, int64_t total_blocks, void* stream)
{
    if (n_items == 0 || total_blocks == 0) return 0;
    if (!items_device) return mpf::fail(MPF_E_NULL, "amax_f32_grouped: NULL table");
    if (n_items < 0 || total_blocks < 0 || total_blocks > 0x7fffffffLL) return mpf::fail(MPF_E_SHAPE, "amax_f32_grouped: bad sizes");
    mpf::set_kernel("amax_grouped_kernel");
    hipLaunchKernelGGL(amax_grouped_kernel, dim3((unsigned)total_blocks), dim3(256), 0, (hipStream_t)stream, items_device, n_items);
    return mpf::check(hipGetLastError(), "mpf_amax_f32_grouped");
}

extern "C" int mpf_gemm3_split_grouped_h2(const MpfSplitItemH2* items_device, int n_items, int64_t total_blocks, void* stream)
{
    if (n_items == 0 || total_blocks == 0) return 0;
    if (!items_device) return mpf::fail(MPF_E_NULL, "gemm3_split_grouped_h2: NULL table");
    if (n_items < 0 || total_blocks < 0 || total_blocks > 0x7fffffffLL) return mpf::fail(MPF_E_SHAPE, "gemm3_split_grouped_h2: bad sizes");
    mpf::set_kernel("gemm3_split_grouped_h2_kernel");
    hipLaunchKernelGGL(gemm3_split_grouped_h2_kernel, dim3((unsigned)total_blocks), dim3(256), 0, (hipStream_t)stream, items_device,
                       n_items);
    return mpf::check(hipGetLastError(), "mpf_gemm3_split_grouped_h2");
}

int mpf::set_gemm3_option(const char* key, int v)
{
    if (!strcmp(key, "gemm3_mixed_tiles")) { g_mixed = v; return 0; }
    if (!strcmp(key, "gemm3_two_pass")) { g_two_pass = v; return 0; }
    if (!strcmp(key, "gemm3_two_pass_rows")) { g_two_pass_rows = v; return 0; }
    if (!strcmp(key, "gemm3_ws")) { g_ws = v; return 0; }
    if (!strcmp(key, "gemm3_tn3")) { g_tn3 = v; return 0; }
    if (!strcmp(key, "gemm3_tn3_176")) { g_tn3_176 = v; return 0; }
    if (!strcmp(key, "gemm3_nt2")) { g_nt2 = v; return 0; }
    if (strcmp(key, "gemm3_ablate") != 0) return 1;
    g_ablate = v;
    return 0;
}

extern "C" int mpf_gemm3_split(const float* w, int rows, int cols, int transpose, void* planes, void* stream)
{
    hipStream_t st = (hipStream_t)stream;
    if (!w || !planes) return mpf::fail(MPF_E_NULL, "gemm3_split: NULL buffer");
    if (rows <= 0 || cols <= 0) return mpf::fail(MPF_E_SHAPE, "gemm3_split: bad sizes");
    const int64_t total = (int64_t)rows * cols;
    const int blocks = (int)((total + 255) / 256 < 2048 ? (total + 255) / 256 : 2048);
    mpf::set_kernel("gemm3_split_kernel");
    hipLaunchKernelGGL(gemm3_split_kernel, dim3(blocks), dim3(256), 0, st, w, (unsigned short*)planes, rows, cols, transpose);
    return mpf::check(hipGetLastError(), "mpf_gemm3_split");
}

extern "C" int mpf_gemm3_split_grouped(const MpfSplitItem* items_device, int n_items, int64_t total_blocks, void* stream)
{
    if (n_items == 0 || total_blocks == 0) return 0;
    if (!items_device) return mpf::fail(MPF_E_NULL, "gemm3_split_grouped: NULL table");
    if (n_items < 0 || total_blocks < 0 || total_blocks > 0x7fffffffLL) return mpf::fail(MPF_E_SHAPE, "gemm3_split_grouped: bad sizes");
    mpf::set_kernel("gemm3_split_grouped_kernel");
    hipLaunchKernelGGL(gemm3_split_grouped_kernel, dim3((unsigned)total_blocks), dim3(256), 0, (hipStream_t)stream, items_device,
                       n_items);
    return mpf::check(hipGetLastError(), "mpf_gemm3_split_grouped");
}

static bool g3_launch_two_pass(G3& p, hipStream_t st)
{
    if (g_two_pass <= 0 || p.N % 256 != 0 || p.N < g_two_pass) return false;
    static int slots2 = 0;
    if (!slots2) {
        int dev = 0, cus = 0;
        slots2 = (hipGetDevice(&dev) == hipSuccess && hipDeviceGetAttribute(&cus, hipDeviceAttributeMultiprocessorCount, dev) == hipSuccess && cus > 0) ? 2 * cus : 512;
    }
    p.tiles_n = p.N / 256;
    const int t128 = ((p.M + 127) / 128) * p.tiles_n, t96 = ((p.M + 95) / 96) * p.tiles_n;
    const double c128 = (double)((t128 + slots2 - 1) / slots2) * 128.0, c96 = (double)((t96 + slots2 - 1) / slots2) * 96.0;
    const bool use96r = g_two_pass_rows == 96 || (g_two_pass_rows == 0 && c96 < c128);
    p.ntiles = use96r ? t96 : t128;
    p.tm0 = 0; p.ntiles2 = 0; p.tiles_n2 = 0;
    mpf::prof_begin(st);
    mpf::set_kernel(use96r ? "gemm3_tn_kernel<96x256>" : "gemm3_tn_kernel<128x256>");
    if (p.a_amax) {
        mpf::set_kernel(use96r ? "gemm3_tn_kernel<h2 96x256>" : "gemm3_tn_kernel<h2 128x256>");
        if (use96r) hipLaunchKernelGGL((gemm3_tn2_kernel<96, false, true>), dim3(((p.ntiles + 7) / 8) * 8), dim3(kThreads), 0, st, p);
        else hipLaunchKernelGGL((gemm3_tn2_kernel<128, false, true>), dim3(((p.ntiles + 7) / 8) * 8), dim3(kThreads), 0, st, p);
        return true;
    }
    if (use96r) hipLaunchKernelGGL(gemm3_tn2_kernel<96>, dim3(((p.ntiles + 7) / 8) * 8), dim3(kThreads), 0, st, p);
    else hipLaunchKernelGGL(gemm3_tn2_kernel<128>, dim3(((p.ntiles + 7) / 8) * 8), dim3(kThreads), 0, st, p);
    return true;
}

static int g3_tn_impl(const float* a, int64_t lda, const float* a2, int a2_rows, const void* b_planes,
                      const float* bias, const float* c_in, int64_t ldcin, const float* c_in2, int64_t ldcin2,
                      const float* gate, int64_t ldgate, float* c, int64_t ldc, int M, int N, int K,
                      int relu, void* stream, const float* a_amax, const float* b_amax, float* out_amax,
                      const unsigned char* gbits = nullptr, int64_t ldgbits = 0, unsigned char* gbits_out = nullptr,
                      int64_t ldgbits_out = 0);

static int g3_launch_ws(G3& p, hipStream_t st)
{
    const int ncg = p.N / 256;
    const int cus = mpf::cu_count();
    int per_xcd = cus / 8 / ncg * ncg;
    if (per_xcd < ncg) per_xcd = ncg;
    int workers = per_xcd / ncg * 8;
    const int tiles16 = (p.M + 15) / 16;
    if (workers > tiles16) workers = ((tiles16 + 7) / 8) * 8;
    const int rpw = ((p.M + workers - 1) / workers + 15) / 16 * 16;
    const int grid = workers * ncg;
    const int key = (p.cin_cm ? 8 : 0) | (p.gbits_cm ? 4 : 0) | (p.relu ? 2 : 0) | (p.gbits_out ? 1 : 0);
    const void* fn = nullptr;
    int slot = 0;
#define WS_CASE(K_, I_, E_, G_, R_, B_) case K_: fn = (const void*)gemm3_ws_kernel<E_, G_, R_, B_>; slot = I_; break;
    switch (key) {
        WS_CASE(0, 0, 0, false, false, false) WS_CASE(8, 1, 1, false, false, false) WS_CASE(2, 2, 0, false, true, false)
        WS_CASE(10, 3, 1, false, true, false) WS_CASE(3, 4, 0, false, true, true) WS_CASE(4, 5, 0, true, false, false)
        WS_CASE(12, 6, 1, true, false, false)
        default: return -1000;
    }
#undef WS_CASE
    static mpf::LdsAttr attr[7];
    if (int e = mpf::ensure_dynamic_lds(fn, kWsLds, attr[slot])) return e;
    mpf::prof_begin(st);
    mpf::set_kernel("gemm3_tn_kernel<h2 ws>");
    {
        void* args[] = {(void*)&p, (void*)&rpw, (void*)&ncg};
        if (hipError_t e = hipLaunchKernel(fn, dim3(grid), dim3(kWsThreads), args, kWsLds, st); e != hipSuccess) return mpf::check(e, "gemm3_ws_kernel");
    }
    mpf::prof_end(mpf_last_kernel(), st, 4.0 * ((double)p.M * p.K + (double)p.M * p.N) + 4.0 * (double)p.N * p.K, 2.0 * p.M * (double)p.N * p.K);
    return mpf::check(hipGetLastError(), "mpf_gemm3_tn_h2(ws)");
}

extern "C" int mpf_gemm3_tn(const float* a, int64_t lda, const float* a2, int a2_rows, const void* b_planes,
                            const float* bias, const float* c_in, int64_t ldcin, const float* c_in2, int64_t ldcin2,
                            const float* gate, int64_t ldgate, float* c, int64_t ldc, int M, int N, int K,
                            int relu, void* stream)
{
    return g3_tn_impl(a, lda, a2, a2_rows, b_planes, bias, c_in, ldcin, c_in2, ldcin2, gate, ldgate, c, ldc, M, N, K, relu, stream,
                      nullptr, nullptr, nullptr);
}

extern "C" int mpf_gemm3_tn_h2(const float* a, int64_t lda, const float* a_amax, const void* b_planes_h2, const float* b_amax,
                               const float* bias, const float* c_in, int64_t ldcin, const float* c_in2, int64_t ldcin2,
                               const float* gate, int64_t ldgate, float* c, int64_t ldc, float* out_amax, int M, int N, int K,
                               int relu, void* stream)
{
    if (!a_amax || !b_amax) return mpf::fail(MPF_E_NULL, "gemm3_tn_h2: NULL amax");
    return g3_tn_impl(a, lda, nullptr, 0, b_planes_h2, bias, c_in, ldcin, c_in2, ldcin2, gate, ldgate, c, ldc, M, N, K, relu, stream,
                      a_amax, b_amax, out_amax);
}

extern "C" int mpf_gemm3_tn_h2_bits(const float* a, int64_t lda, const float* a_amax, const void* b_planes_h2, const float* b_amax,
                                    const float* bias, const float* c_in, int64_t ldcin, const float* c_in2, int64_t ldcin2,
                                    const unsigned char* gate_bits, int64_t ldgbits, float* c, int64_t ldc, float* out_amax,
                                    unsigned char* gate_bits_out, int64_t ldgbits_out, int M, int N, int K, int relu, void* stream)
{
    if (!a_amax || !b_amax) return mpf::fail(MPF_E_NULL, "gemm3_tn_h2_bits: NULL amax");
    if (N % 128 != 0 || (gate_bits && (ldgbits < N / 8 || ldgbits % 8 != 0 || ((uintptr_t)gate_bits & 7))) ||
        (gate_bits_out && (ldgbits_out < N / 8 || ldgbits_out % 8 != 0 || ((uintptr_t)gate_bits_out & 7))))
        return mpf::fail(MPF_E_SHAPE, "gemm3_tn_h2_bits: N must be a multiple of 128; mask rows of >= N / 8 bytes, 8-byte aligned");
    return g3_tn_impl(a, lda, nullptr, 0, b_planes_h2, bias, c_in, ldcin, c_in2, ldcin2, nullptr, 0, c, ldc, M, N, K, relu, stream,
                      a_amax, b_amax, out_amax, gate_bits, ldgbits, gate_bits_out, ldgbits_out);
}

static int g3_tn_impl(const float* a, int64_t lda, const float* a2, int a2_rows, const void* b_planes,
                      const float* bias, const float* c_in, int64_t ldcin, const float* c_in2, int64_t ldcin2,
                      const float* gate, int64_t ldgate, float* c, int64_t ldc, int M, int N, int K,
                      int relu, void* stream, const float* a_amax, const float* b_amax, float* out_amax,
                      const unsigned char* gbits, int64_t ldgbits, unsigned char* gbits_out, int64_t ldgbits_out)
{
    hipStream_t st = (hipStream_t)stream;
    if (!a || !b_planes || !c) return mpf::fail(MPF_E_NULL, "gemm3_tn: NULL buffer");
    if (M <= 0 || N <= 0 || K <= 0) return mpf::fail(MPF_E_SHAPE, "gemm3_tn: bad sizes");
    if (K % kBK != 0 || N % 4 != 0 || lda % 4 != 0 || ldc % 4 != 0 || (c_in && ldcin % 4 != 0) || (c_in2 && ldcin2 % 4 != 0) ||
        (gate && ldgate % 4 != 0))
        return mpf::fail(MPF_E_SHAPE, "gemm3_tn: K must be a multiple of 32; N, lda, ldc multiples of 4");
    if (a2 && a2_rows <= 0) return mpf::fail(MPF_E_SHAPE, "gemm3_tn: a2_rows must be positive");
    G3 p;
    p.a_amax = nullptr; p.b_amax = nullptr; p.out_amax = nullptr;
    p.a = a; p.a2 = a2; p.bp = (const unsigned short*)b_planes; p.bias = bias; p.cin = c_in; p.c = c;
    p.cin2 = c_in2; p.gate = gate; p.ldcin2 = ldcin2; p.ldgate = ldgate;
    p.lda = lda; p.ldc = ldc; p.ldcin = ldcin; p.plane = (int64_t)N * K;
    p.M = M; p.N = N; p.K = K; p.a2_rows = a2_rows; p.relu = relu; p.c16 = nullptr;
    p.a_amax = a_amax; p.b_amax = b_amax; p.out_amax = out_amax;
    {
        const float* consts = nullptr;
        if (int rc = g3_consts(&consts, "gemm3_tn: constants")) return rc;
        p.bias_cm = bias ? 1 : 0; p.cin_cm = c_in ? 1 : 0; p.cin2_cm = c_in2 ? 1 : 0; p.gate_cm = gate ? 1 : 0;
        if (!bias) p.bias = consts;
        if (!c_in) { p.cin = consts; p.ldcin = 0; }
        if (!c_in2) { p.cin2 = consts; p.ldcin2 = 0; }
        if (!gate) { p.gate = consts + 4; p.ldgate = 0; }
        g3_no_bits(p, consts);
        if (gbits) { p.gbits = gbits; p.ldgbits = ldgbits; p.gbits_cm = 1; }
        p.gbits_out = gbits_out; p.ldgbits_out = ldgbits_out;
    }
    const int tiles_m = (M + kBM - 1) / kBM;
    const int waste128 = ((N + 127) / 128) * 128 - N, waste96 = ((N + 95) / 96) * 96 - N;
    const bool use96 = waste96 < waste128;
    p.tiles_n = use96 ? (N + 95) / 96 : (N + 127) / 128;
    p.ntiles = tiles_m * p.tiles_n;
    p.tm0 = 0; p.ntiles2 = 0; p.tiles_n2 = 0;
    if (a_amax && !a2 && !gate && !c_in2 && g_ws > 0 && N >= g_ws && K == kWsK && N % 256 == 0 && ((uintptr_t)a & 15) == 0) {
        const int r = g3_launch_ws(p, st);
        if (r != -1000) return r;
    }
    bool tn3 = a_amax && !a2 && g_tn3 && N % 256 == 0 && M >= 2048 && ((uintptr_t)a & 15) == 0 && lda % 4 == 0;
    int t3_bm = kT3BM;
    if (tn3) {
        const int cus = mpf::cu_count(), nt3 = ((M + kT3BM - 1) / kT3BM) * (N / 256), rem = nt3 % cus;
        tn3 = g_tn3 == 2 || (nt3 >= cus * 3 / 4 && (rem == 0 || 4 * rem >= 3 * cus || nt3 >= 4 * cus));
        const int nt176 = ((M + 175) / 176) * (N / 256);
        if (g_tn3_176 && (nt176 + cus - 1) / cus <= (nt3 + cus - 1) / cus) t3_bm = 176;
    }
    if (tn3) {
        static mpf::LdsAttr attr;
        if (int e = mpf::ensure_dynamic_lds((const void*)gemm3_tn3_kernel, kT3Lds, attr)) return e;
        p.tiles_n = N / 256;
        p.t3_bm = t3_bm;
        p.ntiles = ((M + t3_bm - 1) / t3_bm) * p.tiles_n;
        mpf::prof_begin(st);
        mpf::set_kernel(t3_bm == kT3BM ? "gemm3_tn_kernel<h2 192x256>" : "gemm3_tn_kernel<h2 192x256:176>");
        {
            void* args[] = {(void*)&p};
            if (hipError_t e = hipLaunchKernel((const void*)gemm3_tn3_kernel, dim3(((p.ntiles + 7) / 8) * 8), dim3(kT3T), args, kT3Lds, st); e != hipSuccess)
                return mpf::check(e, "gemm3_tn3_kernel");
        }
        mpf::prof_end(mpf_last_kernel(), st, 4.0 * ((double)M * K + (double)M * N) + 4.0 * (double)N * K, 2.0 * M * (double)N * K);
        return mpf::check(hipGetLastError(), "mpf_gemm3_tn_h2(192x256)");
    }
    if (!a2 && g3_launch_two_pass(p, st)) {
        mpf::prof_end(mpf_last_kernel(), st, 4.0 * ((double)M * K + (double)M * N) + (a_amax ? 4.0 : 6.0) * (double)N * K, 2.0 * M * (double)N * K);
        return mpf::check(hipGetLastError(), "mpf_gemm3_tn");
    }
    if (a_amax) {
        const int grid_h = ((p.ntiles + 7) / 8) * 8;
        mpf::prof_begin(st);
        if (use96) {
            mpf::set_kernel("gemm3_tn_kernel<h2 96>");
            hipLaunchKernelGGL((gemm3_tn_kernel<96, false, true>), dim3(grid_h), dim3(kThreads), 0, st, p);
        } else {
            mpf::set_kernel("gemm3_tn_kernel<h2 128>");
            hipLaunchKernelGGL((gemm3_tn_kernel<128, false, true>), dim3(grid_h), dim3(kThreads), 0, st, p);
        }
        mpf::prof_end(mpf_last_kernel(), st, 4.0 * ((double)M * K + (double)M * N) + 4.0 * (double)N * K, 2.0 * M * (double)N * K);
        return mpf::check(hipGetLastError(), "mpf_gemm3_tn_h2");
    }
    if (!use96 && N % 64 == 0 && g_mixed) {
        static int slots = 0;
        if (!slots) {
            int dev = 0, cus = 0;
            if (hipGetDevice(&dev) == hipSuccess && hipDeviceGetAttribute(&cus, hipDeviceAttributeMultiprocessorCount, dev) == hipSuccess && cus > 0)
                slots = 2 * cus;
            else
                slots = 512;
        }
        const int rounds = p.ntiles / slots, rem = p.ntiles - rounds * slots;
        if (rounds >= 1 && rem > 0 && 2 * rem <= slots && slots % p.tiles_n == 0) {
            const int main_blocks = rounds * (slots / p.tiles_n);
            p.tm0 = main_blocks;
            p.tiles_n2 = N / 64;
            p.ntiles2 = (tiles_m - main_blocks) * p.tiles_n2;
            p.ntiles = main_blocks * p.tiles_n;
            const int grid_mixed = ((p.ntiles + 7) / 8) * 8 + ((p.ntiles2 + 7) / 8) * 8;
            mpf::prof_begin(st);
            mpf::set_kernel("gemm3_tn_kernel<128+64>");
            if (a2) hipLaunchKernelGGL(gemm3_tn_mixed_kernel<true>, dim3(grid_mixed), dim3(kThreads), 0, st, p);
            else hipLaunchKernelGGL(gemm3_tn_mixed_kernel<false>, dim3(grid_mixed), dim3(kThreads), 0, st, p);
            mpf::prof_end(mpf_last_kernel(), st, 4.0 * ((double)M * K + (double)M * N) + 6.0 * (double)N * K, 2.0 * M * (double)N * K);
            return mpf::check(hipGetLastError(), "mpf_gemm3_tn");
        }
    }
    const int grid = ((p.ntiles + 7) / 8) * 8;
    mpf::prof_begin(st);
    if (use96) {
        mpf::set_kernel("gemm3_tn_kernel<96>");
        if (a2) hipLaunchKernelGGL((gemm3_tn_kernel<96, true>), dim3(grid), dim3(kThreads), 0, st, p);
        else hipLaunchKernelGGL((gemm3_tn_kernel<96, false>), dim3(grid), dim3(kThreads), 0, st, p);
    } else {
        mpf::set_kernel("gemm3_tn_kernel<128>");
        if (a2) hipLaunchKernelGGL((gemm3_tn_kernel<128, true>), dim3(grid), dim3(kThreads), 0, st, p);
        else hipLaunchKernelGGL((gemm3_tn_kernel<128, false>), dim3(grid), dim3(kThreads), 0, st, p);
    }
    mpf::prof_end(mpf_last_kernel(), st, 4.0 * ((double)M * K + (double)M * N) + 6.0 * (double)N * K, 2.0 * M * (double)N * K);
    return mpf::check(hipGetLastError(), "mpf_gemm3_tn");
}

extern "C" int mpf_gemm3_tn_ex(const void* a, int a_dtype, int64_t lda, const void* b_planes, const float* bias, const float* c_in,
                               int64_t ldcin, void* c, int c_dtype, int64_t ldc, int M, int N, int K, int relu, void* stream)
{
    hipStream_t st = (hipStream_t)stream;
    if (!a || !b_planes || !c) return mpf::fail(MPF_E_NULL, "gemm3_tn_ex: NULL buffer");
    if ((a_dtype != MPF_F32 && a_dtype != MPF_BF16) || (c_dtype != MPF_F32 && c_dtype != MPF_BF16))
        return mpf::fail(MPF_E_DTYPE, "gemm3_tn_ex: a / c must be MPF_F32 or MPF_BF16");
    const int aal = a_dtype == MPF_BF16 ? 8 : 4;
    if (M <= 0 || N <= 0 || K <= 0 || K % kBK != 0 || N % 4 != 0 || lda % aal != 0 || ldc % 4 != 0 || (c_in && ldcin % 4 != 0) ||
        ((uintptr_t)a & 15))
        return mpf::fail(MPF_E_SHAPE, "gemm3_tn_ex: K must be a multiple of 32, N / ldc of 4, 16-byte aligned A rows");
    if (a_dtype == MPF_F32 && c_dtype == MPF_F32)
        return mpf_gemm3_tn((const float*)a, lda, nullptr, 0, b_planes, bias, c_in, ldcin, nullptr, 0, nullptr, 0, (float*)c, ldc, M, N, K, relu, stream);
    const float* consts = nullptr;
    if (int rc = g3_consts(&consts, "gemm3_tn_ex: constants")) return rc;
    G3 p;
    p.a_amax = nullptr; p.b_amax = nullptr; p.out_amax = nullptr;
    p.a = (const float*)a; p.a2 = nullptr; p.bp = (const unsigned short*)b_planes;
    p.bias = bias ? bias : consts; p.bias_cm = bias ? 1 : 0;
    p.cin = c_in ? c_in : consts; p.ldcin = c_in ? ldcin : 0; p.cin_cm = c_in ? 1 : 0;
    p.cin2 = consts; p.ldcin2 = 0; p.cin2_cm = 0; p.gate = consts + 4; p.ldgate = 0; p.gate_cm = 0;
    g3_no_bits(p, consts);
    p.c = c_dtype == MPF_F32 ? (float*)c : nullptr; p.c16 = c_dtype == MPF_BF16 ? (unsigned short*)c : nullptr;
    p.lda = lda; p.ldc = ldc; p.plane = (int64_t)N * K;
    p.M = M; p.N = N; p.K = K; p.a2_rows = 0; p.relu = relu;
    p.cv_H = p.cv_W = p.cv_cin = 0; p.cv_sign = 1;
    p.tm0 = 0; p.ntiles2 = 0; p.tiles_n2 = 0;
    const int tiles_m = (M + kBM - 1) / kBM;
    const int waste128 = ((N + 127) / 128) * 128 - N, waste96 = ((N + 95) / 96) * 96 - N;
    const bool use96 = waste96 < waste128;
    p.tiles_n = use96 ? (N + 95) / 96 : (N + 127) / 128;
    p.ntiles = tiles_m * p.tiles_n;
    if (a_dtype == MPF_F32 && g3_launch_two_pass(p, st)) {
        mpf::prof_end(mpf_last_kernel(), st, 4.0 * (double)M * K + 2.0 * (double)M * N + 6.0 * (double)N * K, 2.0 * M * (double)N * K);
        return mpf::check(hipGetLastError(), "mpf_gemm3_tn_ex");
    }
    const dim3 grid(((p.ntiles + 7) / 8) * 8);
    mpf::prof_begin(st);
    if (a_dtype == MPF_BF16) {
        mpf::set_kernel("gemm3_tn_kernel<a16>");
        if (use96) hipLaunchKernelGGL(gemm3_tn_abf_kernel<96>, grid, dim3(kThreads), 0, st, p);
        else hipLaunchKernelGGL(gemm3_tn_abf_kernel<128>, grid, dim3(kThreads), 0, st, p);
    } else {
        mpf::set_kernel("gemm3_tn_kernel<c16>");
        if (use96) hipLaunchKernelGGL((gemm3_tn_kernel<96, false>), grid, dim3(kThreads), 0, st, p);
        else hipLaunchKernelGGL((gemm3_tn_kernel<128, false>), grid, dim3(kThreads), 0, st, p);
    }
    mpf::prof_end(mpf_last_kernel(), st, (a_dtype == MPF_BF16 ? 2.0 : 4.0) * (double)M * K + (c_dtype == MPF_BF16 ? 2.0 : 4.0) * (double)M * N + 6.0 * (double)N * K,
                  2.0 * M * (double)N * K);
    return mpf::check(hipGetLastError(), "mpf_gemm3_tn_ex");
}

static int g3_conv_impl(const float* x, const void* w_planes, const float* bias, float* y, int n_img, int H, int W, int Cin,
                        int Cout, int transposed, void* stream, const float* x_amax, const float* w_amax, float* out_amax);

extern "C" int mpf_gemm3_conv3x3(const float* x, const void* w_planes, const float* bias, float* y, int n_img, int H, int W, int Cin,
                                 int Cout, int transposed, void* stream)
{
    return g3_conv_impl(x, w_planes, bias, y, n_img, H, W, Cin, Cout, transposed, stream, nullptr, nullptr, nullptr);
}

extern "C" int mpf_gemm3_conv3x3_h2(const float* x, const float* x_amax, const void* w_planes_h2, const float* w_amax, const float* bias,
                                    float* y, float* out_amax, int n_img, int H, int W, int Cin, int Cout, int transposed, void* stream)
{
    if (!x_amax || !w_amax) return mpf::fail(MPF_E_NULL, "gemm3_conv3x3_h2: NULL amax");
    if (Cout % 256 != 0) return mpf::fail(MPF_E_SHAPE, "gemm3_conv3x3_h2: Cout must be a multiple of 256");
    return g3_conv_impl(x, w_planes_h2, bias, y, n_img, H, W, Cin, Cout, transposed, stream, x_amax, w_amax, out_amax);
}

static int g3_conv_impl(const float* x, const void* w_planes, const float* bias, float* y, int n_img, int H, int W, int Cin,
                        int Cout, int transposed, void* stream, const float* x_amax, const float* w_amax, float* out_amax)
{
    hipStream_t st = (hipStream_t)stream;
    if (!x || !w_planes || !y) return mpf::fail(MPF_E_NULL, "gemm3_conv3x3: NULL buffer");
    if (n_img <= 0 || H <= 0 || W <= 0 || Cin <= 0 || Cout <= 0 || Cin % 32 != 0 || Cout % 4 != 0)
        return mpf::fail(MPF_E_SHAPE, "gemm3_conv3x3: Cin must be a multiple of 32, Cout of 4");
    const int64_t M64 = (int64_t)n_img * H * W;
    if (M64 >= (1ll << 31) / 4 || M64 * Cin >= (1ll << 40)) return mpf::fail(MPF_E_TOO_LARGE, "gemm3_conv3x3: image too large");
    G3 p;
    p.a_amax = nullptr; p.b_amax = nullptr; p.out_amax = nullptr;
    const float* consts = nullptr;
    if (int rc = g3_consts(&consts, "gemm3_conv3x3: constants")) return rc;
    p.a = x; p.a2 = nullptr; p.bp = (const unsigned short*)w_planes; p.c = y;
    p.bias = bias ? bias : consts; p.bias_cm = bias ? 1 : 0;
    p.cin = consts; p.ldcin = 0; p.cin_cm = 0; p.cin2 = consts; p.ldcin2 = 0; p.cin2_cm = 0; p.gate = consts + 4; p.ldgate = 0; p.gate_cm = 0;
    g3_no_bits(p, consts);
    p.M = (int)M64; p.N = Cout; p.K = 9 * Cin; p.lda = Cin; p.ldc = Cout; p.plane = (int64_t)Cout * p.K;
    p.a2_rows = 0; p.relu = 0; p.c16 = nullptr;
    p.cv_H = H; p.cv_W = W; p.cv_cin = Cin; p.cv_sign = transposed ? -1 : 1;
    p.tiles_n = (Cout + 127) / 128;
    p.ntiles = ((p.M + kBM - 1) / kBM) * p.tiles_n;
    p.tm0 = 0; p.ntiles2 = 0; p.tiles_n2 = 0;
    mpf::prof_begin(st);
    mpf::set_kernel("gemm3_conv_kernel");
    p.a_amax = x_amax; p.b_amax = w_amax; p.out_amax = out_amax;
    if (x_amax) mpf::set_kernel("gemm3_conv_kernel<h2>");
    if (x_amax) {
        p.tiles_n = Cout / 256;
        p.ntiles = ((p.M + kBM - 1) / kBM) * p.tiles_n;
        hipLaunchKernelGGL((gemm3_tn2_kernel<128, true, true>), dim3(((p.ntiles + 7) / 8) * 8), dim3(kThreads), 0, st, p);
    } else if (g_two_pass > 0 && Cout % 256 == 0) {
        p.tiles_n = Cout / 256;
        p.ntiles = ((p.M + kBM - 1) / kBM) * p.tiles_n;
        hipLaunchKernelGGL((gemm3_tn2_kernel<128, true>), dim3(((p.ntiles + 7) / 8) * 8), dim3(kThreads), 0, st, p);
    } else
    hipLaunchKernelGGL(gemm3_conv_kernel, dim3(((p.ntiles + 7) / 8) * 8), dim3(kThreads), 0, st, p);
    mpf::prof_end(mpf_last_kernel(), st, 4.0 * ((double)p.M * Cin + (double)p.M * Cout) + (x_amax ? 4.0 : 6.0) * (double)Cout * p.K,
                  2.0 * p.M * (double)Cout * p.K);
    return mpf::check(hipGetLastError(), "mpf_gemm3_conv3x3");
}

static int g3_nt_impl(const float* a, int64_t lda, const float* b, int64_t ldb, const float* b2, int64_t ldb2, int b2_rows,
                      float* c_part, float* csum_a, float* csum_b, int R, int Mdim, int Ndim, int rows_per_split,
                      int transpose_out, void* stream, const float* a_amax, const float* b_amax);

extern "C" int mpf_gemm3_nt(const float* a, int64_t lda, const float* b, int64_t ldb, const float* b2, int64_t ldb2, int b2_rows,
                            float* c_part, float* csum_a, float* csum_b, int R, int Mdim, int Ndim, int rows_per_split,
                            int transpose_out, void* stream)
{
    return g3_nt_impl(a, lda, b, ldb, b2, ldb2, b2_rows, c_part, csum_a, csum_b, R, Mdim, Ndim, rows_per_split, transpose_out, stream,
                      nullptr, nullptr);
}

extern "C" int mpf_gemm3_nt_h2(const float* a, int64_t lda, const float* a_amax, const float* b, int64_t ldb, const float* b_amax,
                               float* c_part, float* csum_a, float* csum_b, int R, int Mdim, int Ndim, int rows_per_split,
                               int transpose_out, void* stream)
{
    if (!a_amax || !b_amax) return mpf::fail(MPF_E_NULL, "gemm3_nt_h2: NULL amax");
    return g3_nt_impl(a, lda, b, ldb, nullptr, 0, 0, c_part, csum_a, csum_b, R, Mdim, Ndim, rows_per_split, transpose_out, stream,
                      a_amax, b_amax);
}

static int g3_nt_impl(const float* a, int64_t lda, const float* b, int64_t ldb, const float* b2, int64_t ldb2, int b2_rows,
// ... 409 lines not shown
```

mp_former_amd/csrc/groupnorm_cl.hip:

```cpp
#include <hip/hip_runtime.h>
#include <math.h>
#include <stdint.h>

#include "mpf_common.h"

namespace {

constexpr int kT = 256;
constexpr int kStatPix = 128;
constexpr int kApplyPix = 64;
constexpr int kSub = 8;

struct Plane {
    int HW, C, G, chunks;
    int tpc;
    int pr;
};

__device__ __forceinline__ void chan_merge(float& n, float& mu, float& m2, float nb, float mb, float qb)
{
    if (nb == 0.f) return;
    const float nn = n + nb, d = mb - mu;
    mu += d * (nb / nn);
    m2 += qb + d * d * (n * nb / nn);
    n = nn;
}

__global__ __launch_bounds__(kT) void gn_cl_stats_kernel(const float* __restrict__ x, int64_t x_bs, float* __restrict__ part,
                                                         const Plane P)
{
    __shared__ float s_st[kT * 3];
    const int n = blockIdx.y, ch = blockIdx.x;
    const int c4 = threadIdx.x % P.tpc, prow = threadIdx.x / P.tpc;
    const int p0 = ch * kStatPix, p1 = min(P.HW, p0 + kStatPix);
    const float* xb = x + (int64_t)n * x_bs + c4 * 4;
    float cn = 0.f, mu = 0.f, m2 = 0.f;
    for (int base = p0 + prow; base < p1; base += P.pr * kSub) {
        float4 v[kSub];
        int cnt = 0;
#pragma unroll
        for (int j = 0; j < kSub; ++j) {
            const int p = base + j * P.pr;
            v[j] = make_float4(0.f, 0.f, 0.f, 0.f);
            if (p < p1) { v[j] = *reinterpret_cast<const float4*>(xb + (int64_t)p * P.C); ++cnt; }
        }
        float s = 0.f;
#pragma unroll
        for (int j = 0; j < kSub; ++j) s += (v[j].x + v[j].y) + (v[j].z + v[j].w);
        const float nb = 4.f * cnt, mb = s / nb;
        float q = 0.f;
#pragma unroll
        for (int j = 0; j < kSub; ++j)
            if (j < cnt) {
                const float a = v[j].x - mb, b = v[j].y - mb, c = v[j].z - mb, d = v[j].w - mb;
                q += (a * a + b * b) + (c * c + d * d);
            }
        chan_merge(cn, mu, m2, nb, mb, q);
    }
    s_st[threadIdx.x * 3] = cn; s_st[threadIdx.x * 3 + 1] = mu; s_st[threadIdx.x * 3 + 2] = m2;
    __syncthreads();
    if (threadIdx.x < P.G) {
        const int g = threadIdx.x, tpg = P.tpc / P.G;
        float an = 0.f, am = 0.f, aq = 0.f;
        for (int r = 0; r < P.pr; ++r)
            for (int k = 0; k < tpg; ++k) {
                const int t = r * P.tpc + g * tpg + k;
                chan_merge(an, am, aq, s_st[t * 3], s_st[t * 3 + 1], s_st[t * 3 + 2]);
            }
        float* o = part + (((int64_t)n * P.G + g) * P.chunks + ch) * 3;
        o[0] = an; o[1] = am; o[2] = aq;
    }
}

__global__ __launch_bounds__(kT) void gn_cl_merge_kernel(const float* __restrict__ part, float* __restrict__ mean,
                                                         float* __restrict__ rstd, int rows, int chunks, float eps)
{
    const int row = blockIdx.x * (kT / 64) + (threadIdx.x >> 6), lane = threadIdx.x & 63;
    if (row >= rows) return;
    double n = 0.0, mu = 0.0, m2 = 0.0;
    for (int c = lane; c < chunks; c += 64) {
        const float* o = part + ((int64_t)row * chunks + c) * 3;
        const double nb = o[0], mb = o[1], qb = o[2];
        if (nb == 0.0) continue;
        const double d = mb - mu, nn = n + nb;
        mu += d * nb / nn;
        m2 += qb + d * d * n * nb / nn;
        n = nn;
    }
#pragma unroll
    for (int o = 1; o < 64; o <<= 1) {
        const double nb = __shfl_xor(n, o, 64), mb = __shfl_xor(mu, o, 64), qb = __shfl_xor(m2, o, 64);
        const double nn = n + nb;
        if (nn > 0.0) {
            const double d = mb - mu;
            const double mu_new = (n * mu + nb * mb) / nn;
            m2 = m2 + qb + d * d * n * nb / nn;
            mu = mu_new;
            n = nn;
        }
    }
    if (lane == 0) {
        mean[row] = (float)mu;
        rstd[row] = (float)(1.0 / sqrt(m2 / n + (double)eps));
    }
}

__device__ __forceinline__ void up2_taps(int o, int in, int& i0, int& i1, float& w0, float& w1)
{
    const float src = fmaxf(0.5f * (o + 0.5f) - 0.5f, 0.f);
    i0 = (int)src;
    i1 = i0 + (i0 < in - 1 ? 1 : 0);
    w1 = src - (float)i0;
    w0 = 1.f - w1;
}

struct ApplyArgs {
    const float* x; int64_t x_bs;
    const float* gamma; const float* beta; const float* mean; const float* rstd;
    const float* top; int64_t top_bs; int W;
    float* y; int64_t y_bs;
};

template <bool RELU, bool TOP>
__global__ __launch_bounds__(kT) void gn_cl_apply_kernel(const ApplyArgs A, const Plane P)
{
    const int n = blockIdx.y;
    const int c4 = threadIdx.x % P.tpc, prow = threadIdx.x / P.tpc;
    const int c = c4 * 4, g = c / (P.C / P.G);
    const float rs = A.rstd[n * P.G + g], mu = A.mean[n * P.G + g];
    const float4 gm = *reinterpret_cast<const float4*>(A.gamma + c), bt = *reinterpret_cast<const float4*>(A.beta + c);
    const float4 a = make_float4(rs * gm.x, rs * gm.y, rs * gm.z, rs * gm.w);
    const float4 b = make_float4(bt.x - mu * a.x, bt.y - mu * a.y, bt.z - mu * a.z, bt.w - mu * a.w);
    const float* xb = A.x + (int64_t)n * A.x_bs + c;
    float* yb = A.y + (int64_t)n * A.y_bs + c;
    const float* tb = TOP ? A.top + (int64_t)n * A.top_bs + c : nullptr;
    const int p0 = blockIdx.x * kApplyPix, p1 = min(P.HW, p0 + kApplyPix);
    const int Wt = A.W >> 1, Ht = (P.HW / A.W) >> 1;
#pragma unroll 4
    for (int p = p0 + prow; p < p1; p += P.pr) {
        const float4 v = *reinterpret_cast<const float4*>(xb + (int64_t)p * P.C);
        float4 r = make_float4(fmaf(v.x, a.x, b.x), fmaf(v.y, a.y, b.y), fmaf(v.z, a.z, b.z), fmaf(v.w, a.w, b.w));
        if (TOP) {
            const int oy = p / A.W, ox = p - oy * A.W;
            int y0, y1, x0, x1;
            float wy0, wy1, wx0, wx1;
            up2_taps(oy, Ht, y0, y1, wy0, wy1);
            up2_taps(ox, Wt, x0, x1, wx0, wx1);
            const float4 t00 = *reinterpret_cast<const float4*>(tb + ((int64_t)y0 * Wt + x0) * P.C);
            const float4 t01 = *reinterpret_cast<const float4*>(tb + ((int64_t)y0 * Wt + x1) * P.C);
            const float4 t10 = *reinterpret_cast<const float4*>(tb + ((int64_t)y1 * Wt + x0) * P.C);
            const float4 t11 = *reinterpret_cast<const float4*>(tb + ((int64_t)y1 * Wt + x1) * P.C);
            r.x += wy0 * (wx0 * t00.x + wx1 * t01.x) + wy1 * (wx0 * t10.x + wx1 * t11.x);
            r.y += wy0 * (wx0 * t00.y + wx1 * t01.y) + wy1 * (wx0 * t10.y + wx1 * t11.y);
            r.z += wy0 * (wx0 * t00.z + wx1 * t01.z) + wy1 * (wx0 * t10.z + wx1 * t11.z);
            r.w += wy0 * (wx0 * t00.w + wx1 * t01.w) + wy1 * (wx0 * t10.w + wx1 * t11.w);
        }
        if (RELU) r = make_float4(fmaxf(r.x, 0.f), fmaxf(r.y, 0.f), fmaxf(r.z, 0.f), fmaxf(r.w, 0.f));
        *reinterpret_cast<float4*>(yb + (int64_t)p * P.C) = r;
    }
}

struct BwdArgs {
    const float* gy; int64_t gy_bs;
    const float* x; int64_t x_bs;
    const float* gamma; const float* beta; const float* mean; const float* rstd;
    float* part;
    float* coef;
    float* dx; int64_t dx_bs;
    float* dgamma; float* dbeta;
    int N;
};

template <bool RELU>
__global__ __launch_bounds__(kT) void gn_cl_bwd_stats_kernel(const BwdArgs A, const Plane P)
{
    __shared__ float4 s_a[kT], s_b[kT];
    const int n = blockIdx.y, ch = blockIdx.x;
    const int c4 = threadIdx.x % P.tpc, prow = threadIdx.x / P.tpc;
    const int c = c4 * 4, g = c / (P.C / P.G);
    float4 a = make_float4(0.f, 0.f, 0.f, 0.f), b = a;
    if (RELU) {
        const float rs = A.rstd[n * P.G + g], mu = A.mean[n * P.G + g];
        const float4 gm = *reinterpret_cast<const float4*>(A.gamma + c), bt = *reinterpret_cast<const float4*>(A.beta + c);
        a = make_float4(rs * gm.x, rs * gm.y, rs * gm.z, rs * gm.w);
        b = make_float4(bt.x - mu * a.x, bt.y - mu * a.y, bt.z - mu * a.z, bt.w - mu * a.w);
    }
    const float* xb = A.x + (int64_t)n * A.x_bs + c;
    const float* gb = A.gy + (int64_t)n * A.gy_bs + c;
    const int p0 = ch * kStatPix, p1 = min(P.HW, p0 + kStatPix);
    float4 sg = make_float4(0.f, 0.f, 0.f, 0.f), sx = sg;
#pragma unroll 4
    for (int p = p0 + prow; p < p1; p += P.pr) {
        const float4 v = *reinterpret_cast<const float4*>(xb + (int64_t)p * P.C);
        float4 q = *reinterpret_cast<const float4*>(gb + (int64_t)p * P.C);
        if (RELU) {
            q.x = fmaf(v.x, a.x, b.x) > 0.f ? q.x : 0.f;
            q.y = fmaf(v.y, a.y, b.y) > 0.f ? q.y : 0.f;
            q.z = fmaf(v.z, a.z, b.z) > 0.f ? q.z : 0.f;
            q.w = fmaf(v.w, a.w, b.w) > 0.f ? q.w : 0.f;
        }
        sg.x += q.x; sg.y += q.y; sg.z += q.z; sg.w += q.w;
        sx.x = fmaf(q.x, v.x, sx.x); sx.y = fmaf(q.y, v.y, sx.y); sx.z = fmaf(q.z, v.z, sx.z); sx.w = fmaf(q.w, v.w, sx.w);
    }
    s_a[threadIdx.x] = sg; s_b[threadIdx.x] = sx;
    __syncthreads();
    if (prow == 0) {
        for (int r = 1; r < P.pr; ++r) {
            const float4 u = s_a[r * P.tpc + c4], w = s_b[r * P.tpc + c4];
            sg.x += u.x; sg.y += u.y; sg.z += u.z; sg.w += u.w;
            sx.x += w.x; sx.y += w.y; sx.z += w.z; sx.w += w.w;
        }
        float* o = A.part + ((int64_t)n * P.chunks + ch) * 2 * P.C;
        *reinterpret_cast<float4*>(o + c) = sg;
        *reinterpret_cast<float4*>(o + P.C + c) = sx;
    }
}

constexpr int kRedCh = 32;
__global__ __launch_bounds__(1024) void gn_cl_bwd_reduce_kernel(const BwdArgs A, const Plane P, float* __restrict__ dgb)
{
    __shared__ double s_1[1024], s_2[1024];
    const int n = blockIdx.y;
    const int cl = threadIdx.x % kRedCh, sl = threadIdx.x / kRedCh;
    const int c = blockIdx.x * kRedCh + cl;
    const int cpg = P.C / P.G, g = c / cpg;
    double sgy = 0.0, sgx = 0.0;
    for (int ch = sl; ch < P.chunks; ch += 1024 / kRedCh) {
        const float* o = A.part + ((int64_t)n * P.chunks + ch) * 2 * P.C;
        sgy += (double)o[c];
        sgx += (double)o[P.C + c];
    }
    s_1[threadIdx.x] = sgy; s_2[threadIdx.x] = sgx;
    __syncthreads();
    for (int h = 512; h >= kRedCh; h >>= 1) {
        if (threadIdx.x < h) { s_1[threadIdx.x] += s_1[threadIdx.x + h]; s_2[threadIdx.x] += s_2[threadIdx.x + h]; }
        __syncthreads();
    }
    if (sl != 0) return;
    sgy = s_1[cl]; sgx = s_2[cl];
    const float gm = A.gamma[c];
    const double mu = A.mean[n * P.G + g], rs = A.rstd[n * P.G + g];
    const double t2 = (sgx - mu * sgy) * rs;
    double s1 = (double)gm * sgy, s2 = (double)gm * t2;
    for (int o = 1; o < cpg; o <<= 1) { s1 += __shfl_xor(s1, o, 64); s2 += __shfl_xor(s2, o, 64); }
    const double m = (double)cpg * (double)P.HW;
    const double Bc = -rs * rs * s2 / m;
    float* o = A.coef + (int64_t)n * 3 * P.C;
    o[c] = (float)(rs * (double)gm);
    o[P.C + c] = (float)Bc;
    o[2 * P.C + c] = (float)(-rs * s1 / m - Bc * mu);
    dgb[((int64_t)n * 2) * P.C + c] = (float)t2;
    dgb[((int64_t)n * 2 + 1) * P.C + c] = (float)sgy;
}

template <bool RELU>
__global__ __launch_bounds__(kT) void gn_cl_bwd_apply_kernel(const BwdArgs A, const Plane P, const float* __restrict__ dgb)
{
    const int n = blockIdx.y;
    if (blockIdx.x == 0 && blockIdx.y == 0)
        for (int c = threadIdx.x; c < P.C; c += kT) {
            float dg = 0.f, db = 0.f;
            for (int i = 0; i < A.N; ++i) { dg += dgb[((int64_t)i * 2) * P.C + c]; db += dgb[((int64_t)i * 2 + 1) * P.C + c]; }
            if (A.dgamma) A.dgamma[c] = dg;
            if (A.dbeta) A.dbeta[c] = db;
        }
    const int c4 = threadIdx.x % P.tpc, prow = threadIdx.x / P.tpc;
    const int c = c4 * 4, g = c / (P.C / P.G);
    const float* co = A.coef + (int64_t)n * 3 * P.C + c;
    const float4 ca = *reinterpret_cast<const float4*>(co), cb = *reinterpret_cast<const float4*>(co + P.C),
                 cd = *reinterpret_cast<const float4*>(co + 2 * P.C);
    float4 a = make_float4(0.f, 0.f, 0.f, 0.f), b = a;
    if (RELU) {
        const float rs = A.rstd[n * P.G + g], mu = A.mean[n * P.G + g];
        const float4 gm = *reinterpret_cast<const float4*>(A.gamma + c), bt = *reinterpret_cast<const float4*>(A.beta + c);
        a = make_float4(rs * gm.x, rs * gm.y, rs * gm.z, rs * gm.w);
        b = make_float4(bt.x - mu * a.x, bt.y - mu * a.y, bt.z - mu * a.z, bt.w - mu * a.w);
    }
    const float* xb = A.x + (int64_t)n * A.x_bs + c;
    const float* gb = A.gy + (int64_t)n * A.gy_bs + c;
    float* db = A.dx + (int64_t)n * A.dx_bs + c;
    const int p0 = blockIdx.x * kApplyPix, p1 = min(P.HW, p0 + kApplyPix);
#pragma unroll 4
    for (int p = p0 + prow; p < p1; p += P.pr) {
        const float4 v = *reinterpret_cast<const float4*>(xb + (int64_t)p * P.C);
        float4 q = *reinterpret_cast<const float4*>(gb + (int64_t)p * P.C);
        if (RELU) {
            q.x = fmaf(v.x, a.x, b.x) > 0.f ? q.x : 0.f;
            q.y = fmaf(v.y, a.y, b.y) > 0.f ? q.y : 0.f;
            q.z = fmaf(v.z, a.z, b.z) > 0.f ? q.z : 0.f;
            q.w = fmaf(v.w, a.w, b.w) > 0.f ? q.w : 0.f;
        }
        float4 r;
        r.x = fmaf(ca.x, q.x, fmaf(cb.x, v.x, cd.x));
        r.y = fmaf(ca.y, q.y, fmaf(cb.y, v.y, cd.y));
        r.z = fmaf(ca.z, q.z, fmaf(cb.z, v.z, cd.z));
        r.w = fmaf(ca.w, q.w, fmaf(cb.w, v.w, cd.w));
        *reinterpret_cast<float4*>(db + (int64_t)p * P.C) = r;
    }
}

__device__ __forceinline__ void up2_adj(int k, int in, int o[4], float w[4])
{
    o[0] = 2 * k - 1; o[1] = 2 * k; o[2] = 2 * k + 1; o[3] = 2 * k + 2;
    w[0] = k > 0 ? 0.25f : 0.f;
    w[1] = k > 0 ? 0.75f : 1.f;
    w[2] = k < in - 1 ? 0.75f : 1.f;
    w[3] = k < in - 1 ? 0.25f : 0.f;
    if (k == 0) o[0] = 0;
    if (k == in - 1) o[3] = 2 * k + 1;
}

__global__ __launch_bounds__(kT) void upsample2x_cl_bwd_kernel(const float* __restrict__ gy, int64_t gy_bs, float* __restrict__ dt,
                                                               int64_t dt_bs, int Ht, int Wt, int C, int tpc, int pr)
{
    const int n = blockIdx.y;
    const int c4 = threadIdx.x % tpc, prow = threadIdx.x / tpc;
    const int p = blockIdx.x * pr + prow;
    if (p >= Ht * Wt) return;
    const int ky = p / Wt, kx = p - ky * Wt;
    int oy[4], ox[4];
    float wy[4], wx[4];
    up2_adj(ky, Ht, oy, wy);
    up2_adj(kx, Wt, ox, wx);
    const float* gb = gy + (int64_t)n * gy_bs + c4 * 4;
    const int W = 2 * Wt;
    float4 acc = make_float4(0.f, 0.f, 0.f, 0.f);
#pragma unroll
    for (int i = 0; i < 4; ++i) {
        float4 row = make_float4(0.f, 0.f, 0.f, 0.f);
#pragma unroll
        for (int j = 0; j < 4; ++j) {
            const float4 q = *reinterpret_cast<const float4*>(gb + ((int64_t)oy[i] * W + ox[j]) * C);
            row.x = fmaf(wx[j], q.x, row.x); row.y = fmaf(wx[j], q.y, row.y);
            row.z = fmaf(wx[j], q.z, row.z); row.w = fmaf(wx[j], q.w, row.w);
        }
        acc.x = fmaf(wy[i], row.x, acc.x); acc.y = fmaf(wy[i], row.y, acc.y);
        acc.z = fmaf(wy[i], row.z, acc.z); acc.w = fmaf(wy[i], row.w, acc.w);
    }
    *reinterpret_cast<float4*>(dt + (int64_t)n * dt_bs + (int64_t)p * C + c4 * 4) = acc;
}

bool make_plane(int HW, int C, int G, Plane& P)
{
    if (HW <= 0 || C <= 0 || G <= 0 || C % G != 0 || C % 4 != 0 || C > 1024) return false;
    const int cpg = C / G, tpc = C / 4;
    if (cpg % 4 != 0 || kT % tpc != 0 || G > kT || C % 32 != 0 || cpg > 32 || (cpg & (cpg - 1)) != 0) return false;
    P.HW = HW; P.C = C; P.G = G; P.tpc = tpc; P.pr = kT / tpc;
    P.chunks = (HW + kStatPix - 1) / kStatPix;
    return true;
}

size_t fwd_ws(int N, const Plane& P) { return (size_t)N * P.G * P.chunks * 3 * sizeof(float); }
size_t bwd_ws(int N, const Plane& P) { return ((size_t)N * P.chunks * 2 * P.C + (size_t)N * 5 * P.C) * sizeof(float); }

}

extern "C" int mpf_gn_cl_supported(int HW, int C, int G)
{
    Plane P;
    return make_plane(HW, C, G, P) ? 1 : 0;
}

extern "C" size_t mpf_gn_cl_workspace_bytes(int N, int HW, int C, int G)
{
    Plane P;
    if (N <= 0 || !make_plane(HW, C, G, P)) return 0;
    const size_t a = fwd_ws(N, P), b = bwd_ws(N, P);
    return a > b ? a : b;
}

extern "C" int mpf_gn_cl_forward(const float* x, int64_t x_bs, const float* gamma, const float* beta, int N, int HW, int C, int G,
                                 float eps, int relu, const float* top, int64_t top_bs, int W, float* y, int64_t y_bs, float* mean,
                                 float* rstd, void* workspace, size_t workspace_bytes, void* stream)
{
    hipStream_t st = (hipStream_t)stream;
    if (!x || !gamma || !beta || !y || !mean || !rstd || !workspace) return mpf::fail(MPF_E_NULL, "gn_cl_forward: NULL buffer");
    Plane P;
    if (N <= 0 || !make_plane(HW, C, G, P))
        return mpf::fail(MPF_E_SHAPE, "gn_cl_forward: needs C % 32 == 0, C/G a power of two in 4..32, 256 % (C/4) == 0");
    if (x_bs % 4 != 0 || y_bs % 4 != 0 || top_bs % 4 != 0) return mpf::fail(MPF_E_SHAPE, "gn_cl_forward: batch strides must be multiples of 4");
    if (top && (W <= 0 || W % 2 != 0 || HW % W != 0 || (HW / W) % 2 != 0))
        return mpf::fail(MPF_E_SHAPE, "gn_cl_forward: the fused top-down sum needs an exact 2x upsampling (even H and W)");
    if (top && relu) return mpf::fail(MPF_E_SHAPE, "gn_cl_forward: relu and top are exclusive");
    if (workspace_bytes < fwd_ws(N, P)) return mpf::fail(MPF_E_SHAPE, "gn_cl_forward: workspace too small");
    float* part = (float*)workspace;
    mpf::prof_begin(st);
    mpf::set_kernel("gn_cl_stats_kernel");
    hipLaunchKernelGGL(gn_cl_stats_kernel, dim3(P.chunks, N), dim3(kT), 0, st, x, x_bs, part, P);
    mpf::prof_end("gn_cl_stats_kernel", st, 4.0 * (double)N * HW * C);
    hipLaunchKernelGGL(gn_cl_merge_kernel, dim3((N * G + kT / 64 - 1) / (kT / 64)), dim3(kT), 0, st, (const float*)part, mean, rstd, N * G, P.chunks, eps);
    ApplyArgs A{x, x_bs, gamma, beta, mean, rstd, top, top_bs, W, y, y_bs};
    const dim3 grid((HW + kApplyPix - 1) / kApplyPix, N);
    mpf::prof_begin(st);
    mpf::set_kernel("gn_cl_apply_kernel");
    if (top) hipLaunchKernelGGL((gn_cl_apply_kernel<false, true>), grid, dim3(kT), 0, st, A, P);
    else if (relu) hipLaunchKernelGGL((gn_cl_apply_kernel<true, false>), grid, dim3(kT), 0, st, A, P);
    else hipLaunchKernelGGL((gn_cl_apply_kernel<false, false>), grid, dim3(kT), 0, st, A, P);
    mpf::prof_end("gn_cl_apply_kernel", st, (top ? 9.0 : 8.0) * (double)N * HW * C);
    return mpf::check(hipGetLastError(), "mpf_gn_cl_forward");
}

extern "C" int mpf_gn_cl_backward(const float* gy, int64_t gy_bs, const float* x, int64_t x_bs, const float* gamma, const float* beta,
                                  const float* mean, const float* rstd, int N, int HW, int C, int G, int relu, float* dx,
                                  int64_t dx_bs, float* dgamma, float* dbeta, void* workspace, size_t workspace_bytes, void* stream)
{
    hipStream_t st = (hipStream_t)stream;
    if (!gy || !x || !gamma || !beta || !mean || !rstd || !dx || !workspace) return mpf::fail(MPF_E_NULL, "gn_cl_backward: NULL buffer");
    Plane P;
    if (N <= 0 || !make_plane(HW, C, G, P))
        return mpf::fail(MPF_E_SHAPE, "gn_cl_backward: needs C % 32 == 0, C/G a power of two in 4..32, 256 % (C/4) == 0");
    if (x_bs % 4 != 0 || gy_bs % 4 != 0 || dx_bs % 4 != 0) return mpf::fail(MPF_E_SHAPE, "gn_cl_backward: batch strides must be multiples of 4");
    if (workspace_bytes < bwd_ws(N, P)) return mpf::fail(MPF_E_SHAPE, "gn_cl_backward: workspace too small");
    float* part = (float*)workspace;
    BwdArgs A{gy, gy_bs, x, x_bs, gamma, beta, mean, rstd, part, part + (size_t)N * P.chunks * 2 * C, dx, dx_bs, dgamma, dbeta, N};
    mpf::prof_begin(st);
    mpf::set_kernel("gn_cl_bwd_stats_kernel");
    if (relu) hipLaunchKernelGGL(gn_cl_bwd_stats_kernel<true>, dim3(P.chunks, N), dim3(kT), 0, st, A, P);
    else hipLaunchKernelGGL(gn_cl_bwd_stats_kernel<false>, dim3(P.chunks, N), dim3(kT), 0, st, A, P);
    mpf::prof_end("gn_cl_bwd_stats_kernel", st, 8.0 * (double)N * HW * C);
    float* dgb = A.coef + (size_t)N * 3 * C;
    hipLaunchKernelGGL(gn_cl_bwd_reduce_kernel, dim3(C / kRedCh, N), dim3(1024), 0, st, A, P, dgb);
    const dim3 grid((HW + kApplyPix - 1) / kApplyPix, N);
    mpf::prof_begin(st);
    mpf::set_kernel("gn_cl_bwd_apply_kernel");
    if (relu) hipLaunchKernelGGL(gn_cl_bwd_apply_kernel<true>, grid, dim3(kT), 0, st, A, P, (const float*)dgb);
    else hipLaunchKernelGGL(gn_cl_bwd_apply_kernel<false>, grid, dim3(kT), 0, st, A, P, (const float*)dgb);
    mpf::prof_end("gn_cl_bwd_apply_kernel", st, 12.0 * (double)N * HW * C);
    return mpf::check(hipGetLastError(), "mpf_gn_cl_backward");
}

extern "C" int mpf_upsample2x_cl_backward(const float* gy, int64_t gy_bs, int N, int Ht, int Wt, int C, float* dtop, int64_t dtop_bs,
                                          void* stream)
{
    hipStream_t st = (hipStream_t)stream;
    if (!gy || !dtop) return mpf::fail(MPF_E_NULL, "upsample2x_cl_backward: NULL buffer");
    if (N <= 0 || Ht <= 0 || Wt <= 0 || C <= 0 || C % 4 != 0 || C > 1024 || kT % (C / 4) != 0 || gy_bs % 4 != 0 || dtop_bs % 4 != 0)
        return mpf::fail(MPF_E_SHAPE, "upsample2x_cl_backward: needs C % 4 == 0 and 256 % (C/4) == 0");
    const int tpc = C / 4, pr = kT / tpc;
    mpf::prof_begin(st);
    mpf::set_kernel("upsample2x_cl_bwd_kernel");
    hipLaunchKernelGGL(upsample2x_cl_bwd_kernel, dim3((Ht * Wt + pr - 1) / pr, N), dim3(kT), 0, st, gy, gy_bs, dtop, dtop_bs, Ht, Wt, C,
                       tpc, pr);
    mpf::prof_end("upsample2x_cl_bwd_kernel", st, 20.0 * (double)N * Ht * Wt * C);
    return mpf::check(hipGetLastError(), "mpf_upsample2x_cl_backward");
}
```

mp_former_amd/csrc/mpf_common.h:

```cpp
#pragma once
#include <hip/hip_runtime.h>
#include <string.h>

#include <atomic>

#include "../../include/mpformer_hip.h"

namespace mpf {
int fail(int code, const char* msg);
int check(hipError_t err, const char* where);
void set_kernel(const char* name);
void prof_begin(hipStream_t st);
void prof_end(const char* name, hipStream_t st, double algorithmic_bytes, double flops = 0.0);
constexpr int kMaxDevices = 32;
struct LdsAttr { std::atomic<int> bytes[kMaxDevices] = {}; };
inline int ensure_dynamic_lds(const void* fn, size_t bytes, LdsAttr& slots)
{
    int dev = 0;
    if (hipGetDevice(&dev) != hipSuccess || dev < 0 || dev >= kMaxDevices) dev = -1;
    if (dev >= 0 && slots.bytes[dev].load(std::memory_order_relaxed) >= (int)bytes) return 0;
    if (int e = check(hipFuncSetAttribute(fn, hipFuncAttributeMaxDynamicSharedMemorySize, (int)bytes), "hipFuncSetAttribute")) return e;
    if (dev >= 0) slots.bytes[dev].store((int)bytes, std::memory_order_relaxed);
    return 0;
}
inline int cu_count()
{
    static std::atomic<int> cache[kMaxDevices];
    int dev = 0, cus = 0;
    if (hipGetDevice(&dev) != hipSuccess || dev < 0 || dev >= kMaxDevices) return 256;
    cus = cache[dev].load(std::memory_order_relaxed);
    if (cus > 0) return cus;
    if (hipDeviceGetAttribute(&cus, hipDeviceAttributeMultiprocessorCount, dev) != hipSuccess || cus <= 0) cus = 256;
    cache[dev].store(cus, std::memory_order_relaxed);
    return cus;
}
int set_msda_option(const char* key, int v);
int set_binned_option(const char* key, int v);
int set_gemm3_option(const char* key, int v);
int set_block_option(const char* key, int v);
int set_decoder_option(const char* key, int v);
int set_attn_option(const char* key, int v);
int set_small_gemm_option(const char* key, int v);
int msda_block_forward(const void* value, const int64_t* host_shapes, const void* loc, const void* attn, void* out, int N, int S, int M,
                       int D, int L, int Lq, int P, int dtype, hipStream_t st, const void* raw = nullptr, const void* ref = nullptr);
size_t msda_block_workspace_bytes(const int64_t* host_shapes, int N, int M, int L, int Lq, int P);
int msda_block_backward(const void* value, const int64_t* host_shapes, const void* loc, const void* attn, const void* go, void* gv,
                        void* gl, void* ga, void* graw, int N, int S, int M, int D, int L, int Lq, int P, int dtype, void* workspace,
                        size_t workspace_bytes, hipStream_t st, const void* fwd_out = nullptr, float* graw_amax = nullptr,
                        float* gv_amax = nullptr, bool* amax_recorded = nullptr);
}
```

mp_former_amd/gemm3.py:

```python
import functools

import torch

from . import _lib


def split_weight(w, transpose=False):
    assert w.is_cuda and w.dtype == torch.float32 and w.dim() == 2 and w.is_contiguous()
    r, c = w.shape
    out = torch.empty((3, c, r) if transpose else (3, r, c), dtype=torch.bfloat16, device=w.device)
    _lib.call("mpf_gemm3_split", w.device, w.data_ptr(), r, c, 1 if transpose else 0, out.data_ptr(), _lib.stream_ptr(w.device))
    return out


def split_weights_grouped(groups):
    import numpy as np
    from ._h2d import upload
    dev = groups[0][0][0].device
    sizes, tot = [], 0
    for srcs, _ in groups:
        n = sum(t.numel() for t in srcs)
        sizes.append((tot, n))
        tot += 3 * n
    buf = torch.empty(tot, dtype=torch.bfloat16, device=dev)
    base = buf.data_ptr()
    rows_tab, blk, outs = [], 0, []
    for (srcs, tr), (off, n) in zip(groups, sizes):
        K = srcs[0].shape[1]
        R = sum(t.shape[0] for t in srcs)
        r0 = 0
        for t in srcs:
            assert t.dtype == torch.float32 and t.is_contiguous() and t.shape[1] == K
            dst = base + 2 * (off + (r0 if tr else r0 * K))
            rows_tab.append((t.data_ptr(), dst, t.shape[0], K, 1 if tr else 0, R if tr else K, n, blk))
            blk += (t.numel() + 1023) // 1024
            r0 += t.shape[0]
        outs.append(buf[off:off + 3 * n].view((3, K, R) if tr else (3, R, K)))
    items = upload(np.asarray(rows_tab, dtype=np.int64).reshape(-1), dev)
    _lib.call("mpf_gemm3_split_grouped", dev, items.data_ptr(), len(rows_tab), blk, _lib.stream_ptr(dev))
    return outs


AMAX_SLOT = 512


def amax_slots(n, device):
    return torch.zeros((n, AMAX_SLOT), dtype=torch.float32, device=device)


def amax_value(slot):
    return slot.view(-1)[::32][:16].max()


def amax(t, out=None):
    assert t.is_cuda and t.dtype == torch.float32 and t.is_contiguous()
    if out is None:
        out = torch.zeros(AMAX_SLOT, dtype=torch.float32, device=t.device)
    _lib.call("mpf_amax_f32", t.device, t.data_ptr(), t.numel(), out.data_ptr(), _lib.stream_ptr(t.device))
    return out


def split_weights_grouped_h2(groups):
    import numpy as np
    from ._h2d import upload
    dev = groups[0][0][0].device
    sizes, tot = [], 0
    for srcs, _ in groups:
        n = sum(t.numel() for t in srcs)
        sizes.append((tot, n))
        tot += 2 * n
    buf = torch.empty(tot, dtype=torch.float16, device=dev)
    slots = amax_slots(len(groups), dev)
    base, sbase = buf.data_ptr(), slots.data_ptr()
    am_tab, sp_tab, ablk, sblk, outs = [], [], 0, 0, []
    seen = {}
    for gi, ((srcs, tr), (off, n)) in enumerate(zip(groups, sizes)):
        K = srcs[0].shape[1]
        R = sum(t.shape[0] for t in srcs)
        key = tuple(t.data_ptr() for t in srcs)
        slot = sbase + 4 * AMAX_SLOT * gi
        if key in seen:
            slot_src = seen[key]
        else:
            seen[key] = gi
            slot_src = gi
            for t in srcs:
                am_tab.append((t.data_ptr(), slot, t.numel(), ablk))
                ablk += (t.numel() + 4095) // 4096
        slot = sbase + 4 * AMAX_SLOT * slot_src
        r0 = 0
        for t in srcs:
            assert t.dtype == torch.float32 and t.is_contiguous() and t.shape[1] == K
            dst = base + 2 * (off + (r0 if tr else r0 * K))
            sp_tab.append((t.data_ptr(), dst, slot, t.shape[0], K, 1 if tr else 0, R if tr else K, n, sblk))
            sblk += (t.numel() + 1023) // 1024
            r0 += t.shape[0]
        outs.append((buf[off:off + 2 * n].view((2, K, R) if tr else (2, R, K)), slots[slot_src]))
    both = upload(np.asarray([x for row in am_tab for x in row] + [x for row in sp_tab for x in row], dtype=np.int64), dev)
    _lib.call("mpf_amax_f32_grouped", dev, both.data_ptr(), len(am_tab), ablk, _lib.stream_ptr(dev))
    _lib.call("mpf_gemm3_split_grouped_h2", dev, both.data_ptr() + 8 * 4 * len(am_tab), len(sp_tab), sblk, _lib.stream_ptr(dev))
    return outs


def gemm3_h2(a, a_amax, planes, w_amax, bias=None, cin=None, cin2=None, gate=None, relu=False, out_amax=None):
    assert a.is_cuda and a.dtype == torch.float32 and a.dim() == 2 and a.stride(1) == 1
    assert planes.dtype == torch.float16 and planes.is_contiguous() and planes.shape[0] == 2
    M, K = a.shape
    N = planes.shape[1]
    assert planes.shape[2] == K
    c = torch.empty((M, N), dtype=torch.float32, device=a.device)
    _lib.call("mpf_gemm3_tn_h2", a.device,
              a.data_ptr(), a.stride(0), a_amax.data_ptr(), planes.data_ptr(), w_amax.data_ptr(), _lib.ptr(bias),
              _lib.ptr(cin), _rows(cin, N) if cin is not None else 0, _lib.ptr(cin2), _rows(cin2, N) if cin2 is not None else 0,
              _lib.ptr(gate), _rows(gate, N) if gate is not None else 0, c.data_ptr(), c.stride(0), _lib.ptr(out_amax), M, N, K,
              1 if relu else 0, _lib.stream_ptr(a.device))
    return c


def gemm3_h2_bits(a, a_amax, planes, w_amax, bias=None, cin=None, cin2=None, gate_bits=None, relu=False, out_amax=None,
                  want_bits=False):
    assert a.is_cuda and a.dtype == torch.float32 and a.dim() == 2 and a.stride(1) == 1
    assert planes.dtype == torch.float16 and planes.is_contiguous() and planes.shape[0] == 2
    M, K = a.shape
    N = planes.shape[1]
    assert planes.shape[2] == K and N % 128 == 0
    if gate_bits is not None:
        assert gate_bits.dtype == torch.uint8 and gate_bits.shape == (M, N // 8) and gate_bits.is_contiguous()
    c = torch.empty((M, N), dtype=torch.float32, device=a.device)
    bits = torch.empty((M, N // 8), dtype=torch.uint8, device=a.device) if want_bits else None
    _lib.call("mpf_gemm3_tn_h2_bits", a.device,
              a.data_ptr(), a.stride(0), a_amax.data_ptr(), planes.data_ptr(), w_amax.data_ptr(), _lib.ptr(bias),
              _lib.ptr(cin), _rows(cin, N) if cin is not None else 0, _lib.ptr(cin2), _rows(cin2, N) if cin2 is not None else 0,
              _lib.ptr(gate_bits), N // 8, c.data_ptr(), c.stride(0), _lib.ptr(out_amax), _lib.ptr(bits), N // 8, M, N, K,
              1 if relu else 0, _lib.stream_ptr(a.device))
# ... 59 lines not shown
    cb = torch.empty((ns, N), dtype=torch.float32, device=a.device) if want_csum_b else None
    if b2 is not None:
        assert b2.dtype == torch.float32 and b2.dim() == 2 and b2.stride(1) == 1 and b2.shape[1] == N
    if amax_ab is not None:
        assert b2 is None
        _lib.call("mpf_gemm3_nt_h2", a.device,
                  a.data_ptr(), a.stride(0), amax_ab[0].data_ptr(), b.data_ptr(), b.stride(0), amax_ab[1].data_ptr(), c.data_ptr(),
                  _lib.ptr(ca), _lib.ptr(cb), R, M, N, rows_per_split, 1 if transpose_out else 0, _lib.stream_ptr(a.device))
    else:
        _lib.call("mpf_gemm3_nt", a.device,
                  a.data_ptr(), a.stride(0), b.data_ptr(), b.stride(0), _lib.ptr(b2), b2.stride(0) if b2 is not None else 0,
                  b2.shape[0] if b2 is not None else 0, c.data_ptr(), _lib.ptr(ca), _lib.ptr(cb), R, M, N, rows_per_split,
                  1 if transpose_out else 0, _lib.stream_ptr(a.device))
    return c, ca, cb


def gemm3_nt_grouped(pairs, rows_per_split, amax_pairs=None):
    import numpy as np
    R = pairs[0][0].shape[0]
    dev = pairs[0][0].device
    ns = (R + rows_per_split - 1) // rows_per_split
    offs, tot = [], 0
    for g, x in pairs:
        assert g.is_cuda and g.dtype == torch.float32 and x.dtype == torch.float32 and g.dim() == 2 and x.dim() == 2
        assert g.stride(1) == 1 and x.stride(1) == 1 and g.shape[0] == R and x.shape[0] == R and x.shape[1] % 4 == 0
        offs.append(tot)
        tot += (g.shape[1] * x.shape[1] + g.shape[1] + 3) // 4 * 4
    padded = any((g.shape[1] * x.shape[1] + g.shape[1]) % 4 for g, x in pairs)
    part = (torch.zeros if padded else torch.empty)((ns, tot), dtype=torch.float32, device=dev)
    base = part.data_ptr()
    items = np.empty((len(pairs), 8 if amax_pairs is None else 10), dtype=np.int64)
    for i, ((g, x), o) in enumerate(zip(pairs, offs)):
        M, N = g.shape[1], x.shape[1]
        if amax_pairs is None:
            items[i] = (g.data_ptr(), g.stride(0), x.data_ptr(), x.stride(0), base + 4 * o, base + 4 * (o + M * N), M, N)
        else:
            items[i] = (g.data_ptr(), g.stride(0), amax_pairs[i][0].data_ptr(), x.data_ptr(), x.stride(0), amax_pairs[i][1].data_ptr(),
                        base + 4 * o, base + 4 * (o + M * N), M, N)
    _lib.call("mpf_gemm3_nt_grouped" if amax_pairs is None else "mpf_gemm3_nt_grouped_h2", dev,
              items.ctypes.data, len(pairs), R, rows_per_split, tot, _lib.stream_ptr(dev))
    out, _ = nt_reduce(part)
    res = []
    for (g, x), o in zip(pairs, offs):
        M, N = g.shape[1], x.shape[1]
        res.append((out[o:o + M * N].view(M, N), out[o + M * N:o + M * N + M]))
    return res


def nt_reduce(c_part, s_part=None):
    ns = c_part.shape[0]
    c = torch.empty(c_part.shape[1:], dtype=torch.float32, device=c_part.device)
    s = torch.empty(s_part.shape[1:], dtype=torch.float32, device=c_part.device) if s_part is not None else None
    if c.numel() % 4 or (s is not None and s.numel() % 4):
        return c_part.sum(0), (s_part.sum(0) if s_part is not None else None)
    _lib.call("mpf_gemm3_nt_reduce", c_part.device, c_part.data_ptr(), c.numel(), _lib.ptr(s_part), s.numel() if s is not None else 0, ns,
              c.data_ptr(), _lib.ptr(s), _lib.stream_ptr(c_part.device))
    return c, s


def nt_reduce_levels(c_part, s_part, level_of_split, n_levels):
    ns = c_part.shape[0]
    c = torch.empty(c_part.shape[1:], dtype=torch.float32, device=c_part.device)
    n = s_part.shape[1]
    lvl = torch.empty((n_levels, n), dtype=torch.float32, device=c_part.device)
    s = torch.empty((n,), dtype=torch.float32, device=c_part.device)
    assert level_of_split.dtype == torch.int64 and level_of_split.numel() == ns and c.numel() % 4 == 0 and n % 4 == 0 and n_levels <= 4
    _lib.call("mpf_gemm3_nt_reduce_levels", c_part.device, c_part.data_ptr(), c.numel(), s_part.data_ptr(), n, ns,
              level_of_split.data_ptr(), n_levels, c.data_ptr(), lvl.data_ptr(), s.data_ptr(), _lib.stream_ptr(c_part.device))
    return c, lvl, s


def gemm3_ex(a, planes, bias=None, cin=None, relu=False, out_dtype=torch.float32):
    assert a.is_cuda and a.dim() == 2 and a.stride(1) == 1 and a.dtype in (torch.float32, torch.bfloat16)
    M, K = a.shape
    N = planes.shape[1]
    assert planes.shape[2] == K and planes.dtype == torch.bfloat16 and planes.is_contiguous()
    c = torch.empty((M, N), dtype=out_dtype, device=a.device)
    _lib.call("mpf_gemm3_tn_ex", a.device, a.data_ptr(), _lib.DTYPE[a.dtype], a.stride(0), planes.data_ptr(), _lib.ptr(bias), _lib.ptr(cin),
              _rows(cin, N) if cin is not None else 0, c.data_ptr(), _lib.DTYPE[out_dtype], N, M, N, K,
              1 if relu else 0, _lib.stream_ptr(a.device))
    return c


def gemm3_nt_ex(a, b, rows_per_split, want_csum_a=False):
    assert a.is_cuda and a.dim() == 2 and b.dim() == 2 and a.stride(1) == 1 and b.stride(1) == 1 and a.shape[0] == b.shape[0]
    R, M = a.shape
    N = b.shape[1]
    ns = (R + rows_per_split - 1) // rows_per_split
    c = torch.empty((ns, M, N), dtype=torch.float32, device=a.device)
    ca = torch.empty((ns, M), dtype=torch.float32, device=a.device) if want_csum_a else None
    _lib.call("mpf_gemm3_nt_ex", a.device, a.data_ptr(), _lib.DTYPE[a.dtype], a.stride(0), b.data_ptr(), _lib.DTYPE[b.dtype], b.stride(0),
              c.data_ptr(), _lib.ptr(ca), R, M, N, rows_per_split, _lib.stream_ptr(a.device))
    return c, ca
```

mp_former_amd/groupnorm.py:

```python

import torch
from torch import nn
from torch.autograd import Function

from . import _lib

def _transpose(src, B, R, C, in_bs=None):
    out = torch.empty(B * R * C, dtype=torch.float32, device=src.device)
    _lib.call("mpf_transpose_f32", src.device, src.data_ptr(), R * C if in_bs is None else in_bs, out.data_ptr(), R * C, B, R, C,
              _lib.stream_ptr(src.device))
    return out


class _ToNCHW(Function):

    @staticmethod
    def forward(ctx, x):
        N, C, H, W = x.shape
        ctx.dims = (N, C, H, W)
        return _transpose(x, N, H * W, C, x.stride(0)).view(N, C, H, W)

    @staticmethod
    def backward(ctx, g):
        N, C, H, W = ctx.dims
        g = g.contiguous()
        return _transpose(g, N, C, H * W).view(N, H, W, C).permute(0, 3, 1, 2)


def to_nchw(x):
    if (x.dim() == 4 and x.dtype == torch.float32 and x.is_cuda and x.stride(1) == 1 and x.stride(3) == x.shape[1]
            and x.stride(2) == x.shape[3] * x.shape[1] and x.stride(0) % 4 == 0
            and not x.is_contiguous() and x.shape[1] % 4 == 0 and (x.shape[2] * x.shape[3]) % 4 == 0 and x.data_ptr() % 16 == 0):
        return _ToNCHW.apply(x)
    return x.contiguous()


class _GroupNormFn(Function):
    @staticmethod
    def forward(ctx, x, weight, bias, groups, eps):
        N, C = x.shape[:2]
        hw = x.numel() // (N * C)
        rows, row_len = N * groups, (C // groups) * hw
        mean = torch.empty(rows, dtype=torch.float32, device=x.device)
        rstd = torch.empty(rows, dtype=torch.float32, device=x.device)
        lib = _lib.lib()
        stream = _lib.stream_ptr(x.device)
        ws = _lib.scratch("gn", x.device, stream, lib.mpf_group_stats_workspace_bytes(rows, row_len))
        _lib.call("mpf_group_stats", x.device, x.data_ptr(), rows, row_len, float(eps), mean.data_ptr(), rstd.data_ptr(), ws.data_ptr(),
                  ws.numel(), stream)
        a = (rstd.view(N, groups, 1) * weight.view(1, groups, C // groups)).view(N, C)
        b = (bias.view(1, groups, C // groups) - mean.view(N, groups, 1) * a.view(N, groups, C // groups)).view(N, C)
        shape = (N, C) + (1,) * (x.dim() - 2)
        y = torch.addcmul(b.view(shape), x, a.view(shape))
        ctx.save_for_backward(x, weight, mean, rstd)
        ctx.groups, ctx.hw = groups, hw
        return y

    @staticmethod
    def backward(ctx, gy):
        x, weight, mean, rstd = ctx.saved_tensors
        N, C = x.shape[:2]
        gx, gw, gb = torch.ops.aten.native_group_norm_backward(
            gy.contiguous(), x, mean.view(N, ctx.groups), rstd.view(N, ctx.groups), weight, N, C, ctx.hw, ctx.groups,
            [ctx.needs_input_grad[0], ctx.needs_input_grad[1], ctx.needs_input_grad[2]])
        return gx, gw, gb, None, None


def is_cl_plane(x):
    return (x.dim() == 4 and x.dtype == torch.float32 and x.is_cuda and x.stride(1) == 1 and x.stride(3) == x.shape[1]
            and x.stride(2) == x.shape[3] * x.shape[1] and x.stride(0) % 4 == 0 and x.data_ptr() % 16 == 0)


def _cl_empty(N, C, H, W, device):
    return torch.empty((N, H, W, C), dtype=torch.float32, device=device).permute(0, 3, 1, 2)


class _GroupNormCLFn(Function):

    @staticmethod
    def forward(ctx, x, weight, bias, groups, eps, relu, top):
        N, C, H, W = x.shape
        lib = _lib.lib()
        mean = torch.empty(N * groups, dtype=torch.float32, device=x.device)
        rstd = torch.empty(N * groups, dtype=torch.float32, device=x.device)
        y = _cl_empty(N, C, H, W, x.device)
        stream = _lib.stream_ptr(x.device)
        ws = _lib.scratch("gn", x.device, stream, lib.mpf_gn_cl_workspace_bytes(N, H * W, C, groups))
        _lib.call("mpf_gn_cl_forward", x.device, x.data_ptr(), x.stride(0), weight.data_ptr(), bias.data_ptr(), N, H * W, C, groups,
                  float(eps), 1 if relu else 0, _lib.ptr(top), top.stride(0) if top is not None else 0, W, y.data_ptr(), y.stride(0),
                  mean.data_ptr(), rstd.data_ptr(), ws.data_ptr(), ws.numel(), stream)
        ctx.save_for_backward(x, weight, bias, mean, rstd)
        ctx.groups, ctx.relu, ctx.has_top = groups, bool(relu), top is not None
        return y

    @staticmethod
    def backward(ctx, gy):
        x, weight, bias, mean, rstd = ctx.saved_tensors
        N, C, H, W = x.shape
        if not is_cl_plane(gy):
            gy = gy.contiguous(memory_format=torch.channels_last)
            if not is_cl_plane(gy):
                gy = gy.permute(0, 2, 3, 1).contiguous().permute(0, 3, 1, 2)
        lib = _lib.lib()
        dx = _cl_empty(N, C, H, W, x.device)
        dg = torch.empty(C, dtype=torch.float32, device=x.device)
        db = torch.empty(C, dtype=torch.float32, device=x.device)
        stream = _lib.stream_ptr(x.device)
        ws = _lib.scratch("gn", x.device, stream, lib.mpf_gn_cl_workspace_bytes(N, H * W, C, ctx.groups))
        dtop = None
        _lib.call("mpf_gn_cl_backward", x.device, gy.data_ptr(), gy.stride(0), x.data_ptr(), x.stride(0), weight.data_ptr(), bias.data_ptr(),
                  mean.data_ptr(), rstd.data_ptr(), N, H * W, C, ctx.groups, 1 if ctx.relu else 0,
                  dx.data_ptr(), dx.stride(0), dg.data_ptr(), db.data_ptr(), ws.data_ptr(), ws.numel(), stream)
        if ctx.has_top and ctx.needs_input_grad[6]:
            dtop = _cl_empty(N, C, H // 2, W // 2, x.device)
            _lib.call("mpf_upsample2x_cl_backward", x.device, gy.data_ptr(), gy.stride(0), N, H // 2, W // 2, C, dtop.data_ptr(),
                      dtop.stride(0), stream)
        return dx, dg, db, None, None, None, dtop


class _GroupNormFlattenFn(Function):

    @staticmethod
    def forward(ctx, groups, eps, *args):
        xs, ws, bs = args[0::3], args[1::3], args[2::3]
        N, C = xs[0].shape[:2]
        sizes = [int(x.shape[2]) * int(x.shape[3]) for x in xs]
        S = sum(sizes)
        dev = xs[0].device
        lib = _lib.lib()
        out = torch.empty((N, S, C), dtype=torch.float32, device=dev)
        stats = []
        stream = _lib.stream_ptr(dev)
        off = 0
        for x, w, b, hw in zip(xs, ws, bs, sizes):
            mean = torch.empty(N * groups, dtype=torch.float32, device=dev)
            rstd = torch.empty(N * groups, dtype=torch.float32, device=dev)
            wsb = _lib.scratch("gn", dev, stream, lib.mpf_gn_cl_workspace_bytes(N, hw, C, groups))
            _lib.call("mpf_gn_cl_forward", dev, x.data_ptr(), x.stride(0), w.data_ptr(), b.data_ptr(), N, hw, C, groups, float(eps), 0,
                      None, 0, int(x.shape[3]), out.data_ptr() + off * C * 4, S * C, mean.data_ptr(),
                      rstd.data_ptr(), wsb.data_ptr(), wsb.numel(), stream)
            stats += [mean, rstd]
            off += hw
        ctx.save_for_backward(*xs, *ws, *bs, *stats)
        ctx.groups, ctx.sizes, ctx.nl = groups, sizes, len(xs)
        return out

    @staticmethod
    def backward(ctx, g):
        nl = ctx.nl
        sv = ctx.saved_tensors
        xs, ws, bs, stats = sv[:nl], sv[nl:2 * nl], sv[2 * nl:3 * nl], sv[3 * nl:]
        g = g.contiguous()
        N, S, C = g.shape
        dev = g.device
        lib = _lib.lib()
        stream = _lib.stream_ptr(dev)
        grads = []
        off = 0
        for l, (x, w, b, hw) in enumerate(zip(xs, ws, bs, ctx.sizes)):
            H, W = int(x.shape[2]), int(x.shape[3])
            dx = _cl_empty(N, C, H, W, dev)
            dg = torch.empty(C, dtype=torch.float32, device=dev)
            db = torch.empty(C, dtype=torch.float32, device=dev)
            wsb = _lib.scratch("gn", dev, stream, lib.mpf_gn_cl_workspace_bytes(N, hw, C, ctx.groups))
            _lib.call("mpf_gn_cl_backward", dev, g.data_ptr() + off * C * 4, S * C, x.data_ptr(), x.stride(0), w.data_ptr(), b.data_ptr(),
                      stats[2 * l].data_ptr(), stats[2 * l + 1].data_ptr(), N, hw, C, ctx.groups, 0,
                      dx.data_ptr(), dx.stride(0), dg.data_ptr(), db.data_ptr(), wsb.data_ptr(), wsb.numel(), stream)
            grads += [dx, dg, db]
            off += hw
        return (None, None) + tuple(grads)


def group_norm_flatten(norms, xs):
    g0 = norms[0]
    for n, x in zip(norms, xs):
        if not (isinstance(n, GroupNorm) and n.cl_ok(x) and n.num_groups == g0.num_groups and n.eps == g0.eps
                and x.shape[:2] == xs[0].shape[:2]):
            return None
    args = []
    for n, x in zip(norms, xs):
        args += [x, n.weight, n.bias]
    return _GroupNormFlattenFn.apply(g0.num_groups, g0.eps, *args)


def cl_enabled():
    return True


class GroupNorm(nn.GroupNorm):
    def cl_ok(self, x, top=None):
        if not (cl_enabled() and self.affine and is_cl_plane(x) and self.weight.dtype == torch.float32):
            return False
        N, C, H, W = x.shape
        if not _lib.lib().mpf_gn_cl_supported(H * W, C, self.num_groups):
            return False
        if top is not None:
            return (is_cl_plane(top) and top.shape[0] == N and top.shape[1] == C and top.shape[2] * 2 == H
                    and top.shape[3] * 2 == W)
        return True

    def forward_cl(self, x, relu=False, top=None):
        return _GroupNormCLFn.apply(x, self.weight, self.bias, self.num_groups, self.eps, relu, top)

    def forward(self, x):
        C = x.shape[1]
        if self.cl_ok(x):
            return self.forward_cl(x)
        if x.is_cuda and x.dtype == torch.float32 and not x.is_contiguous():
            x = to_nchw(x)
        if (x.is_cuda and x.dtype == torch.float32 and x.is_contiguous() and self.affine and x.dim() >= 3
                and ((C // self.num_groups) * (x.numel() // (x.shape[0] * C))) % 4 == 0):
            return _GroupNormFn.apply(x, self.weight, self.bias, self.num_groups, self.eps)
        return super().forward(x)
```

Measured before the change: 86.23 images/sec.

## Publish amax from GroupNorm kernels and use fp16x2 GEMM for 1x1/3x3 convs

GroupNorm forward and backward kernels now compute the absolute maximum of their outputs and attach it to the tensor, so downstream conv3x3 and 1x1 conv GEMMs can skip a separate amax pass. A new mixed split kernel produces both bf16x3 and fp16x2 weight planes plus a weight amax in one call. 1x1 convs with fp32 inputs that carry an amax use a new scaled two-plane fp16 GEMM (tn_ex_h2) instead of the three-plane bf16 path. The cost is an extra amax reduction inside GN kernels, per-tensor Python metadata checks, and possible precision differences from the fp16 split.

```diff
diff --git a/include/mpformer_hip.h b/include/mpformer_hip.h
--- a/include/mpformer_hip.h
+++ b/include/mpformer_hip.h
@@ -65,6 +65,7 @@
                          void* workspace, size_t workspace_bytes, void* stream);
 
 int mpf_set_option(const char* key, int value);
+int mpf_get_option(const char* key, int* value);
 const char* mpf_last_kernel(void);
 int mpf_msda_stats(unsigned long long* out, int n, int reset);
 
@@ -353,6 +354,11 @@
 
 int mpf_gemm3_tn_ex(const void* a, int a_dtype, int64_t lda, const void* b_planes, const float* bias, const float* c_in, int64_t ldcin,
                     void* c, int c_dtype, int64_t ldc, int M, int N, int K, int relu, void* stream);
+int mpf_gemm3_tn_ex_h2(const float* a, int64_t lda, const float* a_amax, const void* b_planes_h2, const float* b_amax,
+                       const float* bias, const float* c_in, int64_t ldcin, void* c, int c_dtype, int64_t ldc, int M, int N, int K,
+                       int relu, void* stream);
+int mpf_gemm3_split_mixed(const float* w, int rows, int cols, void* planes_bf16, int transpose_bf16, void* planes_h2,
+                          int transpose_h2, float* w_amax, void* stream);
 int mpf_gemm3_nt_ex(const void* a, int a_dtype, int64_t lda, const void* b, int b_dtype, int64_t ldb, float* c_part, float* csum_a,
                     int R, int Mdim, int Ndim, int rows_per_split, void* stream);
 
@@ -473,6 +479,13 @@
                        int64_t dx_bs, float* dgamma, float* dbeta, void* workspace, size_t workspace_bytes, void* stream);
 int mpf_upsample2x_cl_backward(const float* gy, int64_t gy_bs, int N, int Ht, int Wt, int C, float* dtop, int64_t dtop_bs,
                                void* stream);
+int mpf_gn_cl_forward_amax(const float* x, int64_t x_bs, const float* gamma, const float* beta, int N, int HW, int C, int G,
+                           float eps, int relu, const float* top, int64_t top_bs, int W, float* y, int64_t y_bs, float* mean,
+                           float* rstd, void* workspace, size_t workspace_bytes, float* y_amax, void* stream);
+int mpf_gn_cl_backward_amax(const float* gy, int64_t gy_bs, const float* x, int64_t x_bs, const float* gamma, const float* beta,
+                            const float* mean, const float* rstd, int N, int HW, int C, int G, int relu, float* dx,
+                            int64_t dx_bs, float* dgamma, float* dbeta, void* workspace, size_t workspace_bytes, float* dx_amax,
+                            void* stream);
 
 size_t mpf_match_cost_fused_workspace_bytes(int G, int Q, int Tmax, int P, int tsamp_rows);
 int mpf_match_cost_fused(const void* embed, const int64_t* embed_first, int64_t embed_row_stride, const void* features,
diff --git a/mp_former_amd/_lib.py b/mp_former_amd/_lib.py
--- a/mp_former_amd/_lib.py
+++ b/mp_former_amd/_lib.py
@@ -22,6 +22,7 @@
     "mpf_last_error": (ctypes.c_char_p, []),
     "mpf_last_kernel": (ctypes.c_char_p, []),
     "mpf_set_option": (_c_int, [ctypes.c_char_p, _c_int]),
+    "mpf_get_option": (_c_int, [ctypes.c_char_p, ctypes.POINTER(_c_int)]),
     "mpf_match_cost_fused_workspace_bytes": (ctypes.c_size_t, [_c_int] * 5),
     "mpf_match_cost_fused": (_c_int, [_c_vp, _c_vp, ctypes.c_int64, _c_vp, ctypes.c_int64, _c_vp, _c_int, _c_int, _c_int, _c_vp, _c_vp, _c_int,
                                       _c_vp, _c_vp, _c_vp, _c_int, _c_int, _c_int, _c_int, ctypes.c_float, ctypes.c_float, _c_vp,
@@ -152,12 +153,20 @@
                                    _c_vp, ctypes.c_int64, _c_int, _c_vp, ctypes.c_int64, _c_vp, _c_vp, _c_vp, ctypes.c_size_t, _c_vp]),
     "mpf_gn_cl_backward": (_c_int, [_c_vp, ctypes.c_int64, _c_vp, ctypes.c_int64, _c_vp, _c_vp, _c_vp, _c_vp, _c_int, _c_int, _c_int,
                                     _c_int, _c_int, _c_vp, ctypes.c_int64, _c_vp, _c_vp, _c_vp, ctypes.c_size_t, _c_vp]),
+    "mpf_gn_cl_forward_amax": (_c_int, [_c_vp, ctypes.c_int64, _c_vp, _c_vp, _c_int, _c_int, _c_int, _c_int, ctypes.c_float, _c_int,
+                                        _c_vp, ctypes.c_int64, _c_int, _c_vp, ctypes.c_int64, _c_vp, _c_vp, _c_vp, ctypes.c_size_t, _c_vp,
+                                        _c_vp]),
+    "mpf_gn_cl_backward_amax": (_c_int, [_c_vp, ctypes.c_int64, _c_vp, ctypes.c_int64, _c_vp, _c_vp, _c_vp, _c_vp, _c_int, _c_int, _c_int,
+                                         _c_int, _c_int, _c_vp, ctypes.c_int64, _c_vp, _c_vp, _c_vp, ctypes.c_size_t, _c_vp, _c_vp]),
     "mpf_upsample2x_cl_backward": (_c_int, [_c_vp, ctypes.c_int64, _c_int, _c_int, _c_int, _c_int, _c_vp, ctypes.c_int64, _c_vp]),
     "mpf_gemm3_conv3x3": (_c_int, [_c_vp, _c_vp, _c_vp, _c_vp, _c_int, _c_int, _c_int, _c_int, _c_int, _c_int, _c_vp]),
     "mpf_gemm3_conv3x3_wgrad": (_c_int, [_c_vp, _c_vp, _c_vp, _c_vp, _c_int, _c_int, _c_int, _c_int, _c_int, _c_int, _c_vp]),
     "mpf_gemm3_nt_reduce_levels": (_c_int, [_c_vp, ctypes.c_int64, _c_vp, ctypes.c_int64, _c_int, _c_vp, _c_int, _c_vp, _c_vp, _c_vp, _c_vp]),
     "mpf_gemm3_tn_ex": (_c_int, [_c_vp, _c_int, ctypes.c_int64, _c_vp, _c_vp, _c_vp, ctypes.c_int64, _c_vp, _c_int, ctypes.c_int64,
                                  _c_int, _c_int, _c_int, _c_int, _c_vp]),
+    "mpf_gemm3_tn_ex_h2": (_c_int, [_c_vp, ctypes.c_int64, _c_vp, _c_vp, _c_vp, _c_vp, _c_vp, ctypes.c_int64, _c_vp, _c_int, ctypes.c_int64,
+                                    _c_int, _c_int, _c_int, _c_int, _c_vp]),
+    "mpf_gemm3_split_mixed": (_c_int, [_c_vp, _c_int, _c_int, _c_vp, _c_int, _c_vp, _c_int, _c_vp, _c_vp]),
     "mpf_gemm3_nt_ex": (_c_int, [_c_vp, _c_int, ctypes.c_int64, _c_vp, _c_int, ctypes.c_int64, _c_vp, _c_vp, _c_int, _c_int, _c_int, _c_int, _c_vp]),
     "mpf_res_ln256_backward_workspace_bytes": (ctypes.c_size_t, [_c_int]),
     "mpf_res_ln256_backward_partial": (_c_int, [_c_vp] * 9 + [_c_int, _c_vp, ctypes.c_size_t, _c_vp]),
@@ -275,6 +284,18 @@
     _option_gen += 1
 
 
+_option_cache = {}
+
+
+def get_option(key):
+    hit = _option_cache.get(key)
+    if hit is None or hit[0] != _option_gen:
+        v = _c_int(0)
+        check(lib().mpf_get_option(key.encode(), ctypes.byref(v)), f"mpf_get_option({key})")
+        hit = _option_cache[key] = (_option_gen, v.value)
+    return hit[1]
+
+
 def msda_stats(reset=True):
     out = (ctypes.c_ulonglong * 9)()
     check(lib().mpf_msda_stats(out, 9, 1 if reset else 0), "mpf_msda_stats")
diff --git a/mp_former_amd/conv3x3.py b/mp_former_amd/conv3x3.py
--- a/mp_former_amd/conv3x3.py
+++ b/mp_former_amd/conv3x3.py
@@ -3,7 +3,7 @@
 from torch.autograd import Function
 
 from . import _lib
-from .gemm3 import amax, split_weights_grouped, split_weights_grouped_h2
+from .gemm3 import amax, published_amax, split_weights_grouped, split_weights_grouped_h2
 from .groupnorm import is_cl_plane
 
 
@@ -36,7 +36,9 @@
         h2 = Cout % 256 == 0 and Cin % 256 == 0
         if h2:
             (pf, pf_am), (pb, pb_am) = split_weights_grouped_h2([([w2.contiguous()], False), ([w2t.contiguous()], False)])
-            x_am = amax(x.permute(0, 2, 3, 1))
+            x_am = published_amax(x)
+            if x_am is None:
+                x_am = amax(x.permute(0, 2, 3, 1))
             _lib.call("mpf_gemm3_conv3x3_h2", x.device, x.data_ptr(), x_am.data_ptr(), pf.data_ptr(), pf_am.data_ptr(), _lib.ptr(bias),
                       y.data_ptr(), None, N, H, W, Cin, Cout, 0, st)
             ctx.save_for_backward(x, weight, pb, pb_am, x_am)
@@ -55,11 +57,13 @@
             x, weight, pb = ctx.saved_tensors
         N, Cin, H, W = x.shape
         Cout = weight.shape[0]
+        gy_am = published_amax(gy) if ctx.h2 else None
         if not (is_cl_plane(gy) and gy.stride(0) == H * W * Cout):
             gy = gy.permute(0, 2, 3, 1).contiguous().permute(0, 3, 1, 2)
         dx = dw = db = None
         st = _lib.stream_ptr(x.device)
-        gy_am = amax(gy.permute(0, 2, 3, 1)) if ctx.h2 else None
+        if ctx.h2 and gy_am is None:
+            gy_am = amax(gy.permute(0, 2, 3, 1))
         if ctx.needs_input_grad[0]:
             dx = _planes(N, Cin, H, W, x.device)
             if ctx.h2:
@@ -123,24 +127,43 @@
 
     @staticmethod
     def forward(ctx, x, weight, bias, out_dtype):
-        from .gemm3 import gemm3, gemm3_ex
+        from .gemm3 import gemm3, gemm3_ex, gemm3_ex_h2, producers_publish_amax, split_weight_mixed
         N, Cin, H, W = x.shape
         Cout = weight.shape[0]
         w2 = weight.view(Cout, Cin)
+        x2 = x.permute(0, 2, 3, 1).reshape(N * H * W, Cin)
+        ctx.dims, ctx.has_bias, ctx.h2_bwd = (N, Cin, Cout, H, W), bias is not None, False
+        mixed = producers_publish_amax() and w2.is_contiguous()
+        x_am = published_amax(x) if mixed and x.dtype == torch.float32 else None
+        if x_am is not None:
+            pb, pf, w_am = split_weight_mixed(w2, True, False)
+            y2 = gemm3_ex_h2(x2, x_am, pf, w_am, bias, out_dtype)
+            ctx.save_for_backward(x2, pb)
+            return y2.view(N, H, W, Cout).permute(0, 3, 1, 2)
+        if mixed and x.dtype == torch.bfloat16 and out_dtype == torch.float32:
+            pf, pb, w_am = split_weight_mixed(w2, False, True)
+            y2 = gemm3_ex(x2, pf, bias, out_dtype=out_dtype)
+            ctx.save_for_backward(x2, pb, w_am, w2)
+            ctx.h2_bwd = True
+            return y2.view(N, H, W, Cout).permute(0, 3, 1, 2)
         pf, pb = split_weights_grouped([([w2], False), ([w2], True)])
-        x2 = x.permute(0, 2, 3, 1).reshape(N * H * W, Cin)
         if x.dtype == torch.float32 and out_dtype == torch.float32:
             y2 = gemm3(x2, pf, bias)
         else:
             y2 = gemm3_ex(x2, pf, bias, out_dtype=out_dtype)
         ctx.save_for_backward(x2, pb)
-        ctx.dims, ctx.has_bias = (N, Cin, Cout, H, W), bias is not None
         return y2.view(N, H, W, Cout).permute(0, 3, 1, 2)
 
     @staticmethod
     def backward(ctx, gy):
-        from .gemm3 import balanced_rps, gemm3, gemm3_ex, gemm3_nt, gemm3_nt_ex, nt_reduce
-        x2, pb = ctx.saved_tensors
+        from .gemm3 import balanced_rps, gemm3, gemm3_ex, gemm3_ex_h2, gemm3_nt, gemm3_nt_ex, nt_reduce, split_weight
+        g_am = None
+        if ctx.h2_bwd:
+            x2, pb_h2, w_am, w2 = ctx.saved_tensors
+            g_am = published_amax(gy) if gy.dtype == torch.float32 else None
+            pb = None
+        else:
+            x2, pb = ctx.saved_tensors
         N, Cin, Cout, H, W = ctx.dims
         g2 = gy.permute(0, 2, 3, 1).reshape(N * H * W, Cout)
         if g2.stride(1) != 1 or g2.stride(0) != Cout:
@@ -149,7 +172,11 @@
             g2 = g2.float()
         dx = dw = db = None
         if ctx.needs_input_grad[0]:
-            if g2.dtype == torch.float32 and x2.dtype == torch.float32:
+            if g_am is None and pb is None:
+                pb = split_weight(w2, transpose=True)
+            if g_am is not None:
+                dx2 = gemm3_ex_h2(g2, g_am, pb_h2, w_am, out_dtype=x2.dtype)
+            elif g2.dtype == torch.float32 and x2.dtype == torch.float32:
                 dx2 = gemm3(g2, pb)
             else:
                 dx2 = gemm3_ex(g2, pb, out_dtype=x2.dtype)
diff --git a/mp_former_amd/csrc/common.hip b/mp_former_amd/csrc/common.hip
--- a/mp_former_amd/csrc/common.hip
+++ b/mp_former_amd/csrc/common.hip
@@ -143,3 +143,10 @@
     if (r <= 0) return r;
     return mpf::fail(MPF_E_SHAPE, "mpf_set_option: unknown key");
 }
+
+extern "C" int mpf_get_option(const char* key, int* value)
+{
+    if (!key || !value) return mpf::fail(MPF_E_NULL, "mpf_get_option: NULL argument");
+    if (mpf::get_gemm3_option(key, value) == 0) return 0;
+    return mpf::fail(MPF_E_SHAPE, "mpf_get_option: unknown key (the gemm3_* switches only)");
+}
diff --git a/mp_former_amd/csrc/gemm3.hip b/mp_former_amd/csrc/gemm3.hip
--- a/mp_former_amd/csrc/gemm3.hip
+++ b/mp_former_amd/csrc/gemm3.hip
@@ -52,6 +52,7 @@
 int g_nt2 = 1;
 int g_tn3 = 1;
 int g_tn3_176 = 1;
+int g_tn_ex_h2 = 1;
 int g_ws = 512;
 
 
@@ -1382,6 +1383,68 @@
     }
 }
 
+__global__ __launch_bounds__(256) void gemm3_split_amax_kernel(const float* __restrict__ w, unsigned short* __restrict__ out, int R, int C,
+                                                               int transpose, float* __restrict__ amax)
+{
+    const int64_t total = (int64_t)R * C;
+    float m = 0.f;
+#pragma unroll
+    for (int k = 0; k < 4; ++k) {
+        const int64_t i = (int64_t)blockIdx.x * 1024 + k * 256 + threadIdx.x;
+        if (i >= total) continue;
+        int r, c;
+        if (transpose) { c = (int)(i / R); r = (int)(i - (int64_t)c * R); } else { r = (int)(i / C); c = (int)(i - (int64_t)r * C); }
+        const float x = w[(int64_t)r * C + c];
+        m = fmaxf(m, fabsf(x));
+        const unsigned xb = __float_as_uint(x);
+        const float r1 = x - __uint_as_float(xb & 0xFFFF0000u);
+        const unsigned rb = __float_as_uint(r1);
+        const float r2 = r1 - __uint_as_float(rb & 0xFFFF0000u);
+        const unsigned lb = __float_as_uint(r2) + 0x8000u;
+        out[i] = (unsigned short)(xb >> 16);
+        out[total + i] = (unsigned short)(rb >> 16);
+        out[2 * total + i] = (unsigned short)(lb >> 16);
+    }
+    __shared__ float red[4];
+    amax_commit(amax, m, red);
+}
+
+__global__ __launch_bounds__(256) void gemm3_split_h2_kernel(const float* __restrict__ w, _Float16* __restrict__ out, int R, int C,
+                                                             int transpose, const float* __restrict__ amax)
+{
+    float scale, inv;
+    h2_scale(amax_read(amax), &scale, &inv);
+    const int64_t total = (int64_t)R * C;
+#pragma unroll
+    for (int k = 0; k < 4; ++k) {
+        const int64_t i = (int64_t)blockIdx.x * 1024 + k * 256 + threadIdx.x;
+        if (i >= total) continue;
+        int r, c;
+        if (transpose) { c = (int)(i / R); r = (int)(i - (int64_t)c * R); } else { r = (int)(i / C); c = (int)(i - (int64_t)r * C); }
+        const float x = w[(int64_t)r * C + c] * scale;
+        const _Float16 h = (_Float16)x;
+        out[i] = h;
+        out[total + i] = (_Float16)(x - (float)h);
+    }
+}
+
+}
+
+extern "C" int mpf_gemm3_split_mixed(const float* w, int rows, int cols, void* planes_bf16, int transpose_bf16, void* planes_h2,
+                                     int transpose_h2, float* w_amax, void* stream)
+{
+    hipStream_t st = (hipStream_t)stream;
+    if (!w || !planes_bf16 || !planes_h2 || !w_amax) return mpf::fail(MPF_E_NULL, "gemm3_split_mixed: NULL buffer");
+    if (rows <= 0 || cols <= 0) return mpf::fail(MPF_E_SHAPE, "gemm3_split_mixed: bad sizes");
+    const int64_t total = (int64_t)rows * cols;
+    if ((total + 1023) / 1024 > 0x7fffffffLL) return mpf::fail(MPF_E_TOO_LARGE, "gemm3_split_mixed: too many elements");
+    const unsigned blocks = (unsigned)((total + 1023) / 1024);
+    hipLaunchKernelGGL(gemm3_split_amax_kernel, dim3(blocks), dim3(256), 0, st, w, (unsigned short*)planes_bf16, rows, cols, transpose_bf16,
+                       w_amax);
+    mpf::set_kernel("gemm3_split_h2_kernel");
+    hipLaunchKernelGGL(gemm3_split_h2_kernel, dim3(blocks), dim3(256), 0, st, w, (_Float16*)planes_h2, rows, cols, transpose_h2,
+                       (const float*)w_amax);
+    return mpf::check(hipGetLastError(), "mpf_gemm3_split_mixed");
 }
 
 extern "C" int mpf_amax_f32(const float* x, int64_t n, float* amax, void* stream)
@@ -1470,9 +1533,23 @@
     if (!strcmp(key, "gemm3_tn3")) { g_tn3 = v; return 0; }
     if (!strcmp(key, "gemm3_tn3_176")) { g_tn3_176 = v; return 0; }
     if (!strcmp(key, "gemm3_nt2")) { g_nt2 = v; return 0; }
+    if (!strcmp(key, "gemm3_tn_ex_h2")) { g_tn_ex_h2 = v; return 0; }
     if (strcmp(key, "gemm3_ablate") != 0) return 1;
     g_ablate = v;
     return 0;
+}
+
+int mpf::get_gemm3_option(const char* key, int* v)
+{
+    if (!strcmp(key, "gemm3_mixed_tiles")) { *v = g_mixed; return 0; }
+    if (!strcmp(key, "gemm3_two_pass")) { *v = g_two_pass; return 0; }
+    if (!strcmp(key, "gemm3_two_pass_rows")) { *v = g_two_pass_rows; return 0; }
+    if (!strcmp(key, "gemm3_ws")) { *v = g_ws; return 0; }
+    if (!strcmp(key, "gemm3_tn3")) { *v = g_tn3; return 0; }
+    if (!strcmp(key, "gemm3_tn3_176")) { *v = g_tn3_176; return 0; }
+    if (!strcmp(key, "gemm3_nt2")) { *v = g_nt2; return 0; }
+    if (!strcmp(key, "gemm3_tn_ex_h2")) { *v = g_tn_ex_h2; return 0; }
+    return 1;
 }
 
 extern "C" int mpf_gemm3_split(const float* w, int rows, int cols, int transpose, void* planes, void* stream)
@@ -1530,7 +1607,7 @@
                       const float* gate, int64_t ldgate, float* c, int64_t ldc, int M, int N, int K,
                       int relu, void* stream, const float* a_amax, const float* b_amax, float* out_amax,
                       const unsigned char* gbits = nullptr, int64_t ldgbits = 0, unsigned char* gbits_out = nullptr,
-                      int64_t ldgbits_out = 0);
+                      int64_t ldgbits_out = 0, int c_bf16 = 0);
 
 static int g3_launch_ws(G3& p, hipStream_t st)
 {
@@ -1602,7 +1679,7 @@
                       const float* bias, const float* c_in, int64_t ldcin, const float* c_in2, int64_t ldcin2,
                       const float* gate, int64_t ldgate, float* c, int64_t ldc, int M, int N, int K,
                       int relu, void* stream, const float* a_amax, const float* b_amax, float* out_amax,
-                      const unsigned char* gbits, int64_t ldgbits, unsigned char* gbits_out, int64_t ldgbits_out)
+                      const unsigned char* gbits, int64_t ldgbits, unsigned char* gbits_out, int64_t ldgbits_out, int c_bf16)
 {
     hipStream_t st = (hipStream_t)stream;
     if (!a || !b_planes || !c) return mpf::fail(MPF_E_NULL, "gemm3_tn: NULL buffer");
@@ -1617,6 +1694,8 @@
     p.cin2 = c_in2; p.gate = gate; p.ldcin2 = ldcin2; p.ldgate = ldgate;
     p.lda = lda; p.ldc = ldc; p.ldcin = ldcin; p.plane = (int64_t)N * K;
     p.M = M; p.N = N; p.K = K; p.a2_rows = a2_rows; p.relu = relu; p.c16 = nullptr;
+    if (c_bf16) { p.c16 = reinterpret_cast<unsigned short*>(c); p.c = nullptr; }
+    const double cb = c_bf16 ? 2.0 : 4.0;
     p.a_amax = a_amax; p.b_amax = b_amax; p.out_amax = out_amax;
     {
         const float* consts = nullptr;
@@ -1636,7 +1715,7 @@
     p.tiles_n = use96 ? (N + 95) / 96 : (N + 127) / 128;
     p.ntiles = tiles_m * p.tiles_n;
     p.tm0 = 0; p.ntiles2 = 0; p.tiles_n2 = 0;
-    if (a_amax && !a2 && !gate && !c_in2 && g_ws > 0 && N >= g_ws && K == kWsK && N % 256 == 0 && ((uintptr_t)a & 15) == 0) {
+    if (a_amax && !a2 && !gate && !c_in2 && !c_bf16 && g_ws > 0 && N >= g_ws && K == kWsK && N % 256 == 0 && ((uintptr_t)a & 15) == 0) {
         const int r = g3_launch_ws(p, st);
         if (r != -1000) return r;
     }
@@ -1661,11 +1740,11 @@
             if (hipError_t e = hipLaunchKernel((const void*)gemm3_tn3_kernel, dim3(((p.ntiles + 7) / 8) * 8), dim3(kT3T), args, kT3Lds, st); e != hipSuccess)
                 return mpf::check(e, "gemm3_tn3_kernel");
         }
-        mpf::prof_end(mpf_last_kernel(), st, 4.0 * ((double)M * K + (double)M * N) + 4.0 * (double)N * K, 2.0 * M * (double)N * K);
+        mpf::prof_end(mpf_last_kernel(), st, 4.0 * (double)M * K + cb * (double)M * N + 4.0 * (double)N * K, 2.0 * M * (double)N * K);
         return mpf::check(hipGetLastError(), "mpf_gemm3_tn_h2(192x256)");
     }
     if (!a2 && g3_launch_two_pass(p, st)) {
-        mpf::prof_end(mpf_last_kernel(), st, 4.0 * ((double)M * K + (double)M * N) + (a_amax ? 4.0 : 6.0) * (double)N * K, 2.0 * M * (double)N * K);
+        mpf::prof_end(mpf_last_kernel(), st, 4.0 * (double)M * K + cb * (double)M * N + (a_amax ? 4.0 : 6.0) * (double)N * K, 2.0 * M * (double)N * K);
         return mpf::check(hipGetLastError(), "mpf_gemm3_tn");
     }
     if (a_amax) {
@@ -1678,7 +1757,7 @@
             mpf::set_kernel("gemm3_tn_kernel<h2 128>");
             hipLaunchKernelGGL((gemm3_tn_kernel<128, false, true>), dim3(grid_h), dim3(kThreads), 0, st, p);
         }
-        mpf::prof_end(mpf_last_kernel(), st, 4.0 * ((double)M * K + (double)M * N) + 4.0 * (double)N * K, 2.0 * M * (double)N * K);
+        mpf::prof_end(mpf_last_kernel(), st, 4.0 * (double)M * K + cb * (double)M * N + 4.0 * (double)N * K, 2.0 * M * (double)N * K);
         return mpf::check(hipGetLastError(), "mpf_gemm3_tn_h2");
     }
     if (!use96 && N % 64 == 0 && g_mixed) {
@@ -1771,6 +1850,16 @@
     mpf::prof_end(mpf_last_kernel(), st, (a_dtype == MPF_BF16 ? 2.0 : 4.0) * (double)M * K + (c_dtype == MPF_BF16 ? 2.0 : 4.0) * (double)M * N + 6.0 * (double)N * K,
                   2.0 * M * (double)N * K);
     return mpf::check(hipGetLastError(), "mpf_gemm3_tn_ex");
+}
+
+extern "C" int mpf_gemm3_tn_ex_h2(const float* a, int64_t lda, const float* a_amax, const void* b_planes_h2, const float* b_amax,
+                                  const float* bias, const float* c_in, int64_t ldcin, void* c, int c_dtype, int64_t ldc, int M, int N,
+                                  int K, int relu, void* stream)
+{
+    if (!a_amax || !b_amax) return mpf::fail(MPF_E_NULL, "gemm3_tn_ex_h2: NULL amax");
+    if (c_dtype != MPF_F32 && c_dtype != MPF_BF16) return mpf::fail(MPF_E_DTYPE, "gemm3_tn_ex_h2: c must be MPF_F32 or MPF_BF16");
+    return g3_tn_impl(a, lda, nullptr, 0, b_planes_h2, bias, c_in, ldcin, nullptr, 0, nullptr, 0, (float*)c, ldc, M, N, K, relu, stream,
+                      a_amax, b_amax, nullptr, nullptr, 0, nullptr, 0, c_dtype == MPF_BF16 ? 1 : 0);
 }
 
 static int g3_conv_impl(const float* x, const void* w_planes, const float* bias, float* y, int n_img, int H, int W, int Cin,
diff --git a/mp_former_amd/csrc/groupnorm_cl.hip b/mp_former_amd/csrc/groupnorm_cl.hip
--- a/mp_former_amd/csrc/groupnorm_cl.hip
+++ b/mp_former_amd/csrc/groupnorm_cl.hip
@@ -3,6 +3,7 @@
 #include <stdint.h>
 
 #include "mpf_common.h"
+#include "amax.h"
 
 namespace {
 
@@ -119,6 +120,7 @@
     const float* gamma; const float* beta; const float* mean; const float* rstd;
     const float* top; int64_t top_bs; int W;
     float* y; int64_t y_bs;
+    float* amax;
 };
 
 template <bool RELU, bool TOP>
@@ -136,6 +138,7 @@
     const float* tb = TOP ? A.top + (int64_t)n * A.top_bs + c : nullptr;
     const int p0 = blockIdx.x * kApplyPix, p1 = min(P.HW, p0 + kApplyPix);
     const int Wt = A.W >> 1, Ht = (P.HW / A.W) >> 1;
+    float am = 0.f;
 #pragma unroll 4
     for (int p = p0 + prow; p < p1; p += P.pr) {
         const float4 v = *reinterpret_cast<const float4*>(xb + (int64_t)p * P.C);
@@ -157,6 +160,11 @@
         }
         if (RELU) r = make_float4(fmaxf(r.x, 0.f), fmaxf(r.y, 0.f), fmaxf(r.z, 0.f), fmaxf(r.w, 0.f));
         *reinterpret_cast<float4*>(yb + (int64_t)p * P.C) = r;
+        am = fmaxf(fmaxf(am, fmaxf(fabsf(r.x), fabsf(r.y))), fmaxf(fabsf(r.z), fabsf(r.w)));
+    }
+    if (A.amax) {
+        __shared__ float red[4];
+        amax_commit(A.amax, am, red);
     }
 }
 
@@ -169,6 +177,7 @@
     float* dx; int64_t dx_bs;
     float* dgamma; float* dbeta;
     int N;
+    float* amax;
 };
 
 template <bool RELU>
@@ -280,6 +289,7 @@
     const float* gb = A.gy + (int64_t)n * A.gy_bs + c;
     float* db = A.dx + (int64_t)n * A.dx_bs + c;
     const int p0 = blockIdx.x * kApplyPix, p1 = min(P.HW, p0 + kApplyPix);
+    float am = 0.f;
 #pragma unroll 4
     for (int p = p0 + prow; p < p1; p += P.pr) {
         const float4 v = *reinterpret_cast<const float4*>(xb + (int64_t)p * P.C);
@@ -296,6 +306,11 @@
         r.z = fmaf(ca.z, q.z, fmaf(cb.z, v.z, cd.z));
         r.w = fmaf(ca.w, q.w, fmaf(cb.w, v.w, cd.w));
         *reinterpret_cast<float4*>(db + (int64_t)p * P.C) = r;
+        am = fmaxf(fmaxf(am, fmaxf(fabsf(r.x), fabsf(r.y))), fmaxf(fabsf(r.z), fabsf(r.w)));
+    }
+    if (A.amax) {
+        __shared__ float red[4];
+        amax_commit(A.amax, am, red);
     }
 }
 
@@ -372,6 +387,14 @@
 extern "C" int mpf_gn_cl_forward(const float* x, int64_t x_bs, const float* gamma, const float* beta, int N, int HW, int C, int G,
                                  float eps, int relu, const float* top, int64_t top_bs, int W, float* y, int64_t y_bs, float* mean,
                                  float* rstd, void* workspace, size_t workspace_bytes, void* stream)
+{
+    return mpf_gn_cl_forward_amax(x, x_bs, gamma, beta, N, HW, C, G, eps, relu, top, top_bs, W, y, y_bs, mean, rstd, workspace,
+                                  workspace_bytes, nullptr, stream);
+}
+
+extern "C" int mpf_gn_cl_forward_amax(const float* x, int64_t x_bs, const float* gamma, const float* beta, int N, int HW, int C, int G,
+                                      float eps, int relu, const float* top, int64_t top_bs, int W, float* y, int64_t y_bs,
+                                      float* mean, float* rstd, void* workspace, size_t workspace_bytes, float* y_amax, void* stream)
 {
     hipStream_t st = (hipStream_t)stream;
     if (!x || !gamma || !beta || !y || !mean || !rstd || !workspace) return mpf::fail(MPF_E_NULL, "gn_cl_forward: NULL buffer");
@@ -389,7 +412,7 @@
     hipLaunchKernelGGL(gn_cl_stats_kernel, dim3(P.chunks, N), dim3(kT), 0, st, x, x_bs, part, P);
     mpf::prof_end("gn_cl_stats_kernel", st, 4.0 * (double)N * HW * C);
     hipLaunchKernelGGL(gn_cl_merge_kernel, dim3((N * G + kT / 64 - 1) / (kT / 64)), dim3(kT), 0, st, (const float*)part, mean, rstd, N * G, P.chunks, eps);
-    ApplyArgs A{x, x_bs, gamma, beta, mean, rstd, top, top_bs, W, y, y_bs};
+    ApplyArgs A{x, x_bs, gamma, beta, mean, rstd, top, top_bs, W, y, y_bs, y_amax};
     const dim3 grid((HW + kApplyPix - 1) / kApplyPix, N);
     mpf::prof_begin(st);
     mpf::set_kernel("gn_cl_apply_kernel");
@@ -404,6 +427,15 @@
                                   const float* mean, const float* rstd, int N, int HW, int C, int G, int relu, float* dx,
                                   int64_t dx_bs, float* dgamma, float* dbeta, void* workspace, size_t workspace_bytes, void* stream)
 {
+    return mpf_gn_cl_backward_amax(gy, gy_bs, x, x_bs, gamma, beta, mean, rstd, N, HW, C, G, relu, dx, dx_bs, dgamma, dbeta, workspace,
+                                   workspace_bytes, nullptr, stream);
+}
+
+extern "C" int mpf_gn_cl_backward_amax(const float* gy, int64_t gy_bs, const float* x, int64_t x_bs, const float* gamma,
+                                       const float* beta, const float* mean, const float* rstd, int N, int HW, int C, int G, int relu,
+                                       float* dx, int64_t dx_bs, float* dgamma, float* dbeta, void* workspace, size_t workspace_bytes,
+                                       float* dx_amax, void* stream)
+{
     hipStream_t st = (hipStream_t)stream;
     if (!gy || !x || !gamma || !beta || !mean || !rstd || !dx || !workspace) return mpf::fail(MPF_E_NULL, "gn_cl_backward: NULL buffer");
     Plane P;
@@ -412,7 +444,7 @@
     if (x_bs % 4 != 0 || gy_bs % 4 != 0 || dx_bs % 4 != 0) return mpf::fail(MPF_E_SHAPE, "gn_cl_backward: batch strides must be multiples of 4");
     if (workspace_bytes < bwd_ws(N, P)) return mpf::fail(MPF_E_SHAPE, "gn_cl_backward: workspace too small");
     float* part = (float*)workspace;
-    BwdArgs A{gy, gy_bs, x, x_bs, gamma, beta, mean, rstd, part, part + (size_t)N * P.chunks * 2 * C, dx, dx_bs, dgamma, dbeta, N};
+    BwdArgs A{gy, gy_bs, x, x_bs, gamma, beta, mean, rstd, part, part + (size_t)N * P.chunks * 2 * C, dx, dx_bs, dgamma, dbeta, N, dx_amax};
     mpf::prof_begin(st);
     mpf::set_kernel("gn_cl_bwd_stats_kernel");
     if (relu) hipLaunchKernelGGL(gn_cl_bwd_stats_kernel<true>, dim3(P.chunks, N), dim3(kT), 0, st, A, P);
diff --git a/mp_former_amd/csrc/mpf_common.h b/mp_former_amd/csrc/mpf_common.h
--- a/mp_former_amd/csrc/mpf_common.h
+++ b/mp_former_amd/csrc/mpf_common.h
@@ -37,6 +37,7 @@
 int set_msda_option(const char* key, int v);
 int set_binned_option(const char* key, int v);
 int set_gemm3_option(const char* key, int v);
+int get_gemm3_option(const char* key, int* v);
 int set_block_option(const char* key, int v);
 int set_decoder_option(const char* key, int v);
 int set_attn_option(const char* key, int v);
diff --git a/mp_former_amd/gemm3.py b/mp_former_amd/gemm3.py
--- a/mp_former_amd/gemm3.py
+++ b/mp_former_amd/gemm3.py
@@ -50,6 +50,32 @@
 
 def amax_value(slot):
     return slot.view(-1)[::32][:16].max()
+
+
+_slot_pool = {}
+
+
+def fresh_slot(device):
+    block, used = _slot_pool.get(device, (None, 32))
+    if used == 32:
+        block, used = amax_slots(32, device), 0
+    _slot_pool[device] = (block, used + 1)
+    return block[used]
+
+
+def publish_amax(t, slot):
+    t._mpf_amax = (slot, t._version, t.data_ptr(), t.numel())
+
+
+def published_amax(t):
+    rec = getattr(t, "_mpf_amax", None)
+    if rec is not None and rec[1] == t._version and rec[2] == t.data_ptr() and rec[3] == t.numel():
+        return rec[0]
+    return None
+
+
+def producers_publish_amax():
+    return _lib.get_option("gemm3_tn_ex_h2") != 0
 
 
 def amax(t, out=None):
@@ -275,6 +301,29 @@
     return c
 
 
+def split_weight_mixed(w, transpose_bf16, transpose_h2):
+    assert w.is_cuda and w.dtype == torch.float32 and w.dim() == 2 and w.is_contiguous()
+    r, c = w.shape
+    p3 = torch.empty((3, c, r) if transpose_bf16 else (3, r, c), dtype=torch.bfloat16, device=w.device)
+    p2 = torch.empty((2, c, r) if transpose_h2 else (2, r, c), dtype=torch.float16, device=w.device)
+    slot = fresh_slot(w.device)
+    _lib.call("mpf_gemm3_split_mixed", w.device, w.data_ptr(), r, c, p3.data_ptr(), 1 if transpose_bf16 else 0, p2.data_ptr(),
+              1 if transpose_h2 else 0, slot.data_ptr(), _lib.stream_ptr(w.device))
+    return p3, p2, slot
+
+
+def gemm3_ex_h2(a, a_amax, planes, w_amax, bias=None, out_dtype=torch.float32):
+    assert a.is_cuda and a.dim() == 2 and a.stride(1) == 1 and a.dtype == torch.float32
+    assert planes.dtype == torch.float16 and planes.is_contiguous() and planes.shape[0] == 2
+    M, K = a.shape
+    N = planes.shape[1]
+    assert planes.shape[2] == K
+    c = torch.empty((M, N), dtype=out_dtype, device=a.device)
+    _lib.call("mpf_gemm3_tn_ex_h2", a.device, a.data_ptr(), a.stride(0), a_amax.data_ptr(), planes.data_ptr(), w_amax.data_ptr(),
+              _lib.ptr(bias), None, 0, c.data_ptr(), _lib.DTYPE[out_dtype], N, M, N, K, 0, _lib.stream_ptr(a.device))
+    return c
+
+
 def gemm3_nt_ex(a, b, rows_per_split, want_csum_a=False):
     assert a.is_cuda and a.dim() == 2 and b.dim() == 2 and a.stride(1) == 1 and b.stride(1) == 1 and a.shape[0] == b.shape[0]
     R, M = a.shape
diff --git a/mp_former_amd/groupnorm.py b/mp_former_amd/groupnorm.py
--- a/mp_former_amd/groupnorm.py
+++ b/mp_former_amd/groupnorm.py
@@ -4,6 +4,7 @@
 from torch.autograd import Function
 
 from . import _lib
+from .gemm3 import fresh_slot, producers_publish_amax, publish_amax
 
 def _transpose(src, B, R, C, in_bs=None):
     out = torch.empty(B * R * C, dtype=torch.float32, device=src.device)
@@ -86,9 +87,12 @@
         y = _cl_empty(N, C, H, W, x.device)
         stream = _lib.stream_ptr(x.device)
         ws = _lib.scratch("gn", x.device, stream, lib.mpf_gn_cl_workspace_bytes(N, H * W, C, groups))
-        _lib.call("mpf_gn_cl_forward", x.device, x.data_ptr(), x.stride(0), weight.data_ptr(), bias.data_ptr(), N, H * W, C, groups,
+        slot = fresh_slot(x.device) if (relu or top is not None) and y.stride(0) == H * W * C and producers_publish_amax() else None
+        _lib.call("mpf_gn_cl_forward_amax", x.device, x.data_ptr(), x.stride(0), weight.data_ptr(), bias.data_ptr(), N, H * W, C, groups,
                   float(eps), 1 if relu else 0, _lib.ptr(top), top.stride(0) if top is not None else 0, W, y.data_ptr(), y.stride(0),
-                  mean.data_ptr(), rstd.data_ptr(), ws.data_ptr(), ws.numel(), stream)
+                  mean.data_ptr(), rstd.data_ptr(), ws.data_ptr(), ws.numel(), _lib.ptr(slot), stream)
+        if slot is not None:
+            publish_amax(y, slot)
         ctx.save_for_backward(x, weight, bias, mean, rstd)
         ctx.groups, ctx.relu, ctx.has_top = groups, bool(relu), top is not None
         return y
@@ -108,9 +112,12 @@
         stream = _lib.stream_ptr(x.device)
         ws = _lib.scratch("gn", x.device, stream, lib.mpf_gn_cl_workspace_bytes(N, H * W, C, ctx.groups))
         dtop = None
-        _lib.call("mpf_gn_cl_backward", x.device, gy.data_ptr(), gy.stride(0), x.data_ptr(), x.stride(0), weight.data_ptr(), bias.data_ptr(),
-                  mean.data_ptr(), rstd.data_ptr(), N, H * W, C, ctx.groups, 1 if ctx.relu else 0,
-                  dx.data_ptr(), dx.stride(0), dg.data_ptr(), db.data_ptr(), ws.data_ptr(), ws.numel(), stream)
+        slot = fresh_slot(x.device) if producers_publish_amax() else None
+        _lib.call("mpf_gn_cl_backward_amax", x.device, gy.data_ptr(), gy.stride(0), x.data_ptr(), x.stride(0), weight.data_ptr(),
+                  bias.data_ptr(), mean.data_ptr(), rstd.data_ptr(), N, H * W, C, ctx.groups, 1 if ctx.relu else 0,
+                  dx.data_ptr(), dx.stride(0), dg.data_ptr(), db.data_ptr(), ws.data_ptr(), ws.numel(), _lib.ptr(slot), stream)
+        if slot is not None:
+            publish_amax(dx, slot)
         if ctx.has_top and ctx.needs_input_grad[6]:
             dtop = _cl_empty(N, C, H // 2, W // 2, x.device)
             _lib.call("mpf_upsample2x_cl_backward", x.device, gy.data_ptr(), gy.stride(0), N, H // 2, W // 2, C, dtop.data_ptr(),
@@ -163,9 +170,12 @@
             dg = torch.empty(C, dtype=torch.float32, device=dev)
             db = torch.empty(C, dtype=torch.float32, device=dev)
             wsb = _lib.scratch("gn", dev, stream, lib.mpf_gn_cl_workspace_bytes(N, hw, C, ctx.groups))
-            _lib.call("mpf_gn_cl_backward", dev, g.data_ptr() + off * C * 4, S * C, x.data_ptr(), x.stride(0), w.data_ptr(), b.data_ptr(),
+            slot = fresh_slot(dev) if producers_publish_amax() else None
+            _lib.call("mpf_gn_cl_backward_amax", dev, g.data_ptr() + off * C * 4, S * C, x.data_ptr(), x.stride(0), w.data_ptr(), b.data_ptr(),
                       stats[2 * l].data_ptr(), stats[2 * l + 1].data_ptr(), N, hw, C, ctx.groups, 0,
-                      dx.data_ptr(), dx.stride(0), dg.data_ptr(), db.data_ptr(), wsb.data_ptr(), wsb.numel(), stream)
+                      dx.data_ptr(), dx.stride(0), dg.data_ptr(), db.data_ptr(), wsb.data_ptr(), wsb.numel(), _lib.ptr(slot), stream)
+            if slot is not None:
+                publish_amax(dx, slot)
             grads += [dx, dg, db]
             off += hw
         return (None, None) + tuple(grads)
```

Result: no change. 87.01 images/sec, median of 6 (+0.9%).
